# element36-io/hyperfridge-r0

Hardware: AMD Instinct MI355X
Metric: segments/sec (po2=20) proving camt53 guest, 1/2/4/8 MI355X (higher is better)
Workload: dtype u32

## Files before the change

### __graft_entry__.py

```python
import hashlib
import os
import subprocess
import sys

ROOT = os.path.dirname(os.path.abspath(__file__))
HIPCC = os.environ.get("HIPCC", "/opt/rocm/bin/hipcc")
CIRCUITS = ("tiny", "small", "bench", "recursion", "trace", "image")
PRECOMPILED = ("small", "bench", "recursion", "trace", "image")


def _run(cmd, **kw):
    subprocess.check_call(cmd, cwd=ROOT, **kw)


def _stale(target, sources):
    if not os.path.exists(target):
        return True
    t = os.path.getmtime(target)
    return any(os.path.getmtime(s) > t for s in sources)


def circuit_blob_path(name):
    return os.path.join(ROOT, "circuits", name + ".r0c")


def code_object_path(name):
    return os.path.join(ROOT, "circuits", name + ".evalcheck.hsaco")


def check_code_object_path(name):
    return os.path.join(ROOT, "circuits", name + ".checkwitness.hsaco")


def term_names_path(name):
    return os.path.join(ROOT, "circuits", name + ".terms.txt")


NAMED = ("trace", "image")


def build():
    jobs = str(min(8, os.cpu_count() or 1))
    _run(["make", "-s", "-j", jobs, "-C", os.path.join("hyperfridge-r0_amd", "csrc")])
    _run(["make", "-s", "-C", "oracle"])
    gen = os.path.join(ROOT, "tools", "gen_circuit.py")
    for name in CIRCUITS:
        if _stale(circuit_blob_path(name), [gen, os.path.join(ROOT, "tools", "trace_circuit.py"), os.path.join(ROOT, "tools", "sponge_component.py"), os.path.join(ROOT, "tools", "image_circuit.py")]):
            _run([sys.executable, gen, name, circuit_blob_path(name)])
    for name in NAMED:
        if _stale(term_names_path(name), [circuit_blob_path(name)]):
            _run([sys.executable, gen, "--names", name, term_names_path(name)])
    sys.path.insert(0, ROOT)
    import numpy as np

    import hyperfridge_r0_amd as r0
    r0.lib()
    guest = os.path.join(ROOT, "circuits", "guest_camt53.elf")
    if _stale(guest, [os.path.join(ROOT, "tools", n) for n in ("guest_camt53.py", "guest_rsa.py", "rvasm.py")]):
        _run([sys.executable, os.path.join(ROOT, "tools", "guest_camt53.py"), guest], stdout=subprocess.DEVNULL)
    pending = []
    for name in PRECOMPILED:
        blob = np.fromfile(circuit_blob_path(name), dtype=np.uint32)
        for emit, target, suffix in ((r0.emit_eval_check_source, code_object_path(name), ".evalcheck.hip"),
                                     (r0.emit_check_witness_source, check_code_object_path(name), ".checkwitness.hip")):
            src = emit(blob)
            src_path = os.path.join(ROOT, "circuits", name + suffix)
            digest = hashlib.sha256(src.encode()).hexdigest()
            stamp = target + ".sha256"
            if os.path.exists(target) and os.path.exists(stamp) and open(stamp).read() == digest:
                continue
            with open(src_path, "w") as f:
                f.write(src)
            cmd = [HIPCC, "--genco", "--offload-arch=gfx950", "-O3", "-o", target, src_path]
            pending.append((name, stamp, digest, cmd, subprocess.Popen(cmd, cwd=ROOT)))
    for name, stamp, digest, cmd, proc in pending:
        if proc.wait() != 0:
            raise subprocess.CalledProcessError(proc.returncode, cmd)
        with open(stamp, "w") as f:
            f.write(digest)
    return None


def ensure_built():
    needed = [os.path.join(ROOT, "hyperfridge-r0_amd", "libr0hip.so"), os.path.join(ROOT, "hyperfridge-r0_amd", "r0h_prove"),
              os.path.join(ROOT, "hyperfridge-r0_amd", "r0h_verify"), os.path.join(ROOT, "hyperfridge-r0_amd", "r0h_preprocess"),
              os.path.join(ROOT, "oracle", "liborc.so"), os.path.join(ROOT, "circuits", "guest_camt53.elf")] + [circuit_blob_path(n) for n in CIRCUITS] + [code_object_path(n) for n in PRECOMPILED] + [
                  check_code_object_path(n) for n in PRECOMPILED] + [term_names_path(n) for n in NAMED]
    if not all(os.path.exists(p) for p in needed):
        build()


def smoke():
    ensure_built()
    sys.path.insert(0, ROOT)
    sys.path.insert(0, os.path.join(ROOT, "tests"))
    import numpy as np

    import hyperfridge_r0_amd as r0
    import orc_binding
    hal = r0.Hal(0)
    blob = np.fromfile(circuit_blob_path("small"), dtype=np.uint32)
    co = code_object_path("small")
    circuit = hal.load_circuit(blob, co if os.path.exists(co) else None)
    po2 = 10
    code, data, glob = hal.witgen(circuit, po2, seed=42)
    seal = hal.prove_segment(circuit, po2, code, data, glob)
    orc = orc_binding.load()
    oc = orc.circuit(blob)
    root = hal.code_root(circuit, po2)
    rc, why = oc.verify(seal, code_root=root)
    assert rc == 0, "oracle verifier rejected the GPU seal: " + why
    want = oc.prove(po2, code.to_host(), data.to_host(), glob)
    assert np.array_equal(seal, want), "GPU seal differs from the oracle's"
    print("smoke ok: seal of %d words verified (bound to the control root) and identical to the oracle; phases (ms): %s" % (
        seal.size, ", ".join("%s=%.2f" % p for p in hal.last_profile())))
    sys.path.insert(0, os.path.join(ROOT, "tools"))
    from bench_session import elf_of
    from test_rv32im import _guest
    tblob = np.fromfile(circuit_blob_path("trace"), dtype=np.uint32)
    tc = hal.load_circuit(tblob, code_object_path("trace"))
    elf, words = elf_of(_guest(300), 0x400), [7, 0x01020304]
    iblob = np.fromfile(circuit_blob_path("image"), dtype=np.uint32)
    ic = hal.load_circuit(iblob, code_object_path("image"))
    hal.set_image_circuit(ic)
    receipt, image_id, cycles = hal.prove_elf(tc, elf, words, segment_po2=16)
    hal.set_image_circuit(None)
    seals = receipt.seals()
    size = r0.verify_seal(tblob, seals[-1][1])[2]
    troot = hal.code_root(tc, size)
    verdict = receipt.verify(tblob, {size: troot}, None, elf=elf)
    assert verdict[:2] == (0, "ok"), "the receipt of the proved run does not verify with its ELF: %r" % (verdict,)
    verdict = receipt.verify_image(tblob, {size: troot}, iblob, image_id)
    assert verdict[:2] == (0, "ok"), "the receipt does not verify with the image id alone: %r" % (verdict,)
    toc = orc.circuit(tblob)
    assert toc.verify(seals[-1][1], code_root=troot) == (0, "ok"), "oracle verifier rejected the trace-circuit seal"
    vm = r0.Vm()
    vm.load_elf(elf)
    vm.set_input(words)
    assert vm.run(segment_po2=16, keep_trace=True, boundary_rows=True) == (0, 0)
    k = len(seals) - 1
    wdata, _ = vm.trace_witness(k, size, claim_globals=vm.claims()[k].globals())
    want = toc.prove(size, toc.witgen(size, 0)[0], wdata, seals[-1][1][:r0.TRACE_GLOBALS])
    assert np.array_equal(want, seals[-1][1]), "the device's trace-circuit seal differs from the oracle's"
    print("smoke ok: prove(env, elf) of %d cycles in %d segment(s) with the trace circuit: receipt verified with the ELF and with the image id alone, last seal identical to the oracle's" % (cycles, len(seals)))
    ic.free()
    tc.free()
    hal.close()
    return None


if __name__ == "__main__":
    build()
    if len(sys.argv) > 1 and sys.argv[1] == "smoke":
        smoke()
```

### hyperfridge-r0_amd/__init__.py

```python
import ctypes
import sys
import os

import numpy as np

P = 2013265921
INV_RATE = 4
QUERIES = 50
FRI_FOLD = 16
CHECK_SIZE = 16
GROUP_ACCUM, GROUP_CODE, GROUP_DATA = 0, 1, 2

_HERE = os.path.dirname(os.path.abspath(__file__))
LIB_PATH = os.path.join(_HERE, "libr0hip.so")


class R0HipError(RuntimeError):
    pass


_c = ctypes
_vp, _u32, _u64, _sz, _cp = _c.c_void_p, _c.c_uint32, _c.c_uint64, _c.c_size_t, _c.c_char_p
_pp = _c.POINTER(_c.c_void_p)

# ... 42 lines not shown
    "r0h_circuit_emit_hip_check": [_vp, _sz, _c.POINTER(_c.c_char_p)],
    "r0h_circuit_load_check": [_vp, _cp],
    "r0h_check_witness": [_vp, _vp, _u32, _vp, _vp, _vp, _vp, _vp, _vp, _sz, _c.POINTER(_sz)],
    "r0h_ctx_set_check_witness": [_vp, _c.c_int],
    "r0h_circuit_free": [_vp],
    "r0h_witgen": [_vp, _vp, _u32, _u64, _vp, _vp, _vp],
    "r0h_witgen_public": [_vp, _vp, _u32, _u64, _vp, _vp, _vp],
    "r0h_seal_digest": [_vp, _sz, _vp],
    "r0h_ctx_set_session_resident_limit": [_vp, _u64],
    "r0h_proof_shrink": [_vp, _vp],
    "r0h_sponge_trace": [_vp, _sz, _u32, _vp],
    "r0h_image_po2": [_vp, _sz, _vp],
    "r0h_image_witness": [_vp, _sz, _u32, _vp, _vp],
    "r0h_prove_image": [_vp, _vp, _vp, _sz, _vp, _vp, _sz, _vp],
    "r0h_accum": [_vp, _vp, _u32, _vp, _vp, _vp, _vp],
    "r0h_eval_check": [_vp, _vp, _u32, _vp, _vp, _vp, _vp, _vp, _vp, _vp],
    "r0h_prove_segment": [_vp, _vp, _u32, _vp, _vp, _vp, _vp, _sz, _c.POINTER(_sz)],
    "r0h_proof_begin": [_vp, _vp, _u32, _vp, _vp, _vp, _vp, _pp],
    "r0h_proof_finish": [_vp, _vp, _vp, _sz, _c.POINTER(_sz)],
    "r0h_proof_abort": [_vp],
    "r0h_verify_seal": [_vp, _sz, _vp, _vp, _vp, _sz, _c.POINTER(_c.c_int), _c.POINTER(_u32)],
    "r0h_verify_seal_bound": [_vp, _sz, _vp, _vp, _vp, _sz, _vp, _c.POINTER(_c.c_int), _c.POINTER(_u32), _vp],
    "r0h_code_root": [_vp, _vp, _u32, _u32, _vp],
    "r0h_code_commit_new": [_vp, _vp, _u32, _u32, _pp],
    "r0h_code_commit_free": [_vp],
    "r0h_code_commit_root": [_vp, _vp],
    "r0h_prove_segment_committed": [_vp, _vp, _u32, _vp, _vp, _vp, _vp, _sz, _c.POINTER(_sz)],
    "r0h_proof_begin_committed": [_vp, _vp, _u32, _vp, _vp, _vp, _vp, _pp],
    "r0h_serde_encode_str": [_vp, _sz, _vp, _sz, _c.POINTER(_sz)],
    "r0h_serde_decode_str": [_vp, _sz, _c.POINTER(_sz), _c.POINTER(_sz), _c.POINTER(_sz)],
    "r0h_journal_commitment_span": [_vp, _sz, _c.POINTER(_sz), _c.POINTER(_sz)],
    "r0h_env_new": [_pp],
    "r0h_env_write_str": [_vp, _vp, _sz],
    "r0h_env_write_u8_seq": [_vp, _vp, _sz],
    "r0h_env_words": [_vp, _pp, _c.POINTER(_sz)],
    "r0h_env_free": [_vp],
    "r0h_receipt_parse": [_vp, _sz, _pp],
    "r0h_receipt_new": [_c.c_int, _vp, _sz, _pp],
    "r0h_receipt_add_segment": [_vp, _vp, _sz, _u32],
    "r0h_receipt_free": [_vp],
    "r0h_receipt_add_segment_claim": [_vp, _vp, _sz, _u32, _vp, _vp],
    "r0h_receipt_segment_claim": [_vp, _sz, _vp, _c.POINTER(_c.c_int)],
    "r0h_receipt_verify": [_vp, _vp, _sz, _vp, _sz, _vp, _c.POINTER(_c.c_int), _c.POINTER(_sz), _c.POINTER(_c.c_int)],
    "r0h_receipt_verify_elf": [_vp, _vp, _sz, _vp, _sz, _vp, _sz, _c.POINTER(_c.c_int), _c.POINTER(_sz), _c.POINTER(_c.c_int)],
    "r0h_receipt_verify_image": [_vp, _vp, _sz, _vp, _sz, _vp, _sz, _vp, _vp, _c.POINTER(_c.c_int), _c.POINTER(_sz), _c.POINTER(_c.c_int)],
    "r0h_receipt_set_image_proof": [_vp, _vp, _sz],
    "r0h_receipt_image_proof": [_vp, _c.POINTER(_vp), _c.POINTER(_sz)],
    "r0h_ctx_set_image_circuit": [_vp, _vp],
    "r0h_sha256": [_vp, _sz, _vp],
    "r0h_image_id_from_hex": [_cp, _vp],
    "r0h_image_id_to_hex": [_vp, _vp],
    "r0h_tagged_struct": [_cp, _vp, _sz, _vp, _sz, _vp],
    "r0h_system_state_digest": [_vp, _vp],
    "r0h_output_digest": [_vp, _sz, _vp, _vp],
    "r0h_claim_digest": [_vp, _vp],
    "r0h_claim_globals": [_vp, _vp],
    "r0h_receipt_journal": [_vp, _pp, _c.POINTER(_sz)],
    "r0h_receipt_segment": [_vp, _sz, _pp, _c.POINTER(_sz), _c.POINTER(_u32)],
    "r0h_receipt_to_json": [_vp, _pp],
    "r0h_ebics_parse": [_vp, _sz, _pp],
    "r0h_ebics_free": [_vp],
    "r0h_ebics_part": [_vp, _c.c_int, _pp, _c.POINTER(_sz)],
    "r0h_ebics_check_digest": [_vp, _c.POINTER(_c.c_int)],
    "r0h_ebics_verify_bank_signature": [_vp, _vp, _sz, _c.POINTER(_c.c_int)],
    "r0h_ebics_check_transaction_key": [_vp, _vp, _sz, _vp, _sz, _vp, _c.POINTER(_c.c_int)],
    "r0h_ebics_verify_witness": [_vp, _vp, _sz, _vp, _sz, _c.POINTER(_c.c_int)],
    "r0h_ebics_decrypt_transaction_key": [_vp, _vp, _sz, _vp, _sz, _c.POINTER(_sz), _vp, _c.POINTER(_c.c_int)],
    "r0h_ebics_witness_sign": [_vp, _vp, _sz, _pp],
    "r0h_ebics_decrypt_order_data": [_vp, _vp],
    "r0h_ebics_document": [_vp, _sz, _pp, _pp, _c.POINTER(_sz)],
    "r0h_rsa_public_key_decimal": [_vp, _sz, _pp, _pp],
    "r0h_ebics_env_inputs": [_vp, _vp, _sz, _vp, _sz, _vp, _sz, _cp, _cp, _vp, _sz, _vp, _sz, _cp, _pp],
    "r0h_aes128_block": [_vp, _vp, _c.c_int, _vp],
    "r0h_zlib_inflate": [_vp, _sz, _pp, _c.POINTER(_sz)],
    "r0h_vm_new": [_pp],
    "r0h_vm_free": [_vp],
    "r0h_vm_load": [_vp, _u32, _vp, _sz],
    "r0h_vm_load_elf": [_vp, _vp, _sz],
    "r0h_vm_set_input": [_vp, _vp, _sz],
    "r0h_vm_set_pc": [_vp, _u32],
    "r0h_vm_set_reg": [_vp, _u32, _u32],
    "r0h_vm_read": [_vp, _u32, _vp, _sz],
    "r0h_vm_run": [_vp, _vp, _c.POINTER(_c.c_int), _c.POINTER(_u32)],
    "r0h_vm_segment_info": [_vp, _sz, _vp],
    "r0h_vm_preflight": [_vp, _sz, _pp, _c.POINTER(_sz)],
    "r0h_vm_trace_witness": [_vp, _sz, _u32, _vp, _vp],
    "r0h_vm_run_segment": [_vp, _vp, _c.POINTER(_c.c_int), _c.POINTER(_c.c_int), _c.POINTER(_u32)],
    "r0h_vm_release_trace": [_vp, _sz],
    "r0h_vm_boundary": [_vp, _sz, _pp, _c.POINTER(_sz)],
    "r0h_trace_witgen": [_vp, _vp, _sz, _vp, _sz, _u32, _vp, _vp, _vp],
    "r0h_logup_multiplicities": [_vp, _vp, _u32, _vp, _vp],
    "r0h_logup_multiplicities_host": [_vp, _sz, _u32, _vp, _vp],
    "r0h_logup_totals": [_vp, _vp, _u32, _vp, _vp, _vp],
    "r0h_accum_public": [_vp, _vp, _u32, _vp, _vp, _vp, _vp, _vp],
    "r0h_prefix_sums": [_vp, _vp, _u32],
    "r0h_proof_data_root": [_vp, _vp],
    "r0h_proof_late": [_vp, _vp, _vp],
    "r0h_proof_globals": [_vp, _vp],
    "r0h_code_commit_columns": [_vp, _pp],
    "r0h_verify_seal_roots": [_vp, _sz, _vp, _sz, _vp, _c.POINTER(_c.c_int), _c.POINTER(_u32), _vp],
    "r0h_session_begin": [_vp, _vp, _vp, _sz, _vp, _sz, _u32, _u64, _u32, _u32, _pp],
    "r0h_session_records": [_vp, _vp, _vp, _sz, _c.POINTER(_sz)],
    "r0h_session_finish": [_vp, _vp, _sz, _pp, _vp, _c.POINTER(_u64)],
    "r0h_session_free": [_vp],
    "r0h_session_challenge": [_vp, _sz, _vp],
    "r0h_last_session_stats": [_vp, _vp],
    "r0h_vm_journal": [_vp, _pp, _c.POINTER(_sz)],
    "r0h_vm_segment_claim": [_vp, _sz, _vp],
    "r0h_compute_image_id": [_vp, _sz, _vp],
    "r0h_camt53_guest_input": [_vp, _vp, _sz, _vp, _sz, _vp, _sz, _vp, _sz, _vp, _sz, _c.c_char_p, _c.c_char_p, _u32, _pp, _c.POINTER(_sz)],
    "r0h_control_root_host": [_vp, _sz, _vp, _vp, _u32, _vp],
    "r0h_prove_elf": [_vp, _vp, _vp, _sz, _vp, _sz, _u32, _u64, _pp, _vp, _c.POINTER(_u64)],
    "r0h_prove_elf_part": [_vp, _vp, _vp, _sz, _vp, _sz, _u32, _u64, _u32, _u32, _pp, _vp, _c.POINTER(_u64)],
    "r0h_receipt_merge": [_pp, _sz, _pp],
    "r0h_recursor_new": [_vp, _vp, _sz, _cp, _u32, _vp, _sz, _vp, _sz, _pp],
    "r0h_recursor_free": [_vp],
    "r0h_recursor_control_root": [_vp, _vp],
    "r0h_lift": [_vp, _vp, _sz, _vp, _pp],
    "r0h_join": [_vp, _vp, _vp, _pp],
    "r0h_node_new": [_vp, _sz, _vp, _pp],
    "r0h_node_free": [_vp],
    "r0h_node_seal": [_vp, _pp, _c.POINTER(_sz)],
    "r0h_node_claim": [_vp, _vp],
    "r0h_node_verify": [_vp, _sz, _vp, _vp, _c.POINTER(_c.c_int)],
    "r0h_kernel_timing": [_vp, _c.c_int],
    "r0h_kernel_stats": [_vp, _vp, _sz],
    "r0h_last_profile": [_vp, _c.POINTER(_c.POINTER(_cp)), _c.POINTER(_c.POINTER(_c.c_float)), _c.POINTER(_u32)],
}
_PLAIN = {
    "r0h_free_error": ([_vp], None),
    "r0h_version": ([], _cp),
    "r0h_ctx_hashfn": ([_vp], _cp),
    "r0h_receipt_kind": ([_vp], _c.c_int),
    "r0h_receipt_n_segments": ([_vp], _sz),
    "r0h_ebics_n_documents": ([_vp], _sz),
    "r0h_vm_n_segments": ([_vp], _sz),
    "r0h_session_n_segments": ([_vp], _sz),
    "r0h_vm_cycles": ([_vp], _u64),
    "r0h_vm_reg": ([_vp, _u32], _u32),
    "r0h_vm_pc": ([_vp], _u32),
    "r0h_verify_reason": ([_c.c_int], _cp),
    "r0h_trace_column_name": ([_u32], _cp),
    "r0h_receipt_verify_reason": ([_c.c_int], _cp),
    "r0h_buf_device_ptr": ([_vp], _vp),
    "r0h_buf_bytes": ([_vp], _sz),
    "r0h_circuit_group_size": ([_vp, _u32], _u32),
    "r0h_circuit_n_global": ([_vp], _u32),
    "r0h_proof_resident_bytes": ([_vp], _sz),
    "r0h_circuit_n_mix": ([_vp], _u32),
    "r0h_circuit_n_taps": ([_vp], _u32),
    "r0h_circuit_n_terms": ([_vp], _u32),
}
EXPORTED_SYMBOLS = sorted(list(_SIGNATURES) + list(_PLAIN))

_lib = None


def _torch_runtime_first():
    import sys
    if os.environ.get("R0H_NO_TORCH") == "1":
        return
    try:
        if "torch" not in sys.modules:
            import importlib.util
            if importlib.util.find_spec("torch") is None:
                return
        import torch
        if getattr(torch.version, "hip", None):
            torch.cuda.is_available()
    except Exception:
        pass


def lib():
    global _lib
    if _lib is None:
        _torch_runtime_first()
        if not os.path.exists(LIB_PATH):
            raise R0HipError("%s is missing: run `python -c 'import __graft_entry__ as g; g.build()'` (hipcc, gfx950). "
                             "There is no CPU fallback." % LIB_PATH)
        h = ctypes.CDLL(LIB_PATH)
        for name, args in _SIGNATURES.items():
            fn = getattr(h, name)
            fn.argtypes = args
            fn.restype = _vp
        for name, (args, res) in _PLAIN.items():
            fn = getattr(h, name)
            fn.argtypes = args
            fn.restype = res
        _lib = h
    return _lib


def _check(err):
    if err:
        msg = ctypes.cast(err, ctypes.c_char_p).value.decode("utf-8", "replace")
        lib().r0h_free_error(err)
        raise R0HipError(msg)


def _u32arr(a):
    a = np.ascontiguousarray(a, dtype=np.uint32)
    return a, a.ctypes.data_as(_vp)


class Buf:

    def __init__(self, hal, handle, words):
        self.hal, self.handle, self.words = hal, handle, words

    def to_host(self, offset_words=0, words=None):
        words = self.words - offset_words if words is None else words
        out = np.empty(words, dtype=np.uint32)
        _check(lib().r0h_buf_d2h(self.hal.ctx, self.handle, offset_words * 4, out.ctypes.data_as(_vp), words * 4))
        return out

    def upload(self, array, offset_words=0):
        a, p = _u32arr(array)
        _check(lib().r0h_buf_h2d(self.hal.ctx, self.handle, offset_words * 4, p, a.size * 4))

    def slice(self, offset_words, words):
        h = _vp()
        _check(lib().r0h_buf_slice(self.handle, offset_words * 4, words * 4, ctypes.byref(h)))
        return Buf(self.hal, h, words)

    def device_ptr(self):
        return lib().r0h_buf_device_ptr(self.handle)

    def free(self):
        if self.handle:
            _check(lib().r0h_buf_free(self.handle))
            self.handle = None

    def __del__(self):
        try:
            self.free()
        except Exception:
            pass


class Circuit:
    def __init__(self, hal, handle, blob):
        self.hal, self.handle, self.blob = hal, handle, blob
        L = lib()
        self.group_size = [L.r0h_circuit_group_size(handle, g) for g in range(3)]
        self.n_global = L.r0h_circuit_n_global(handle)
        self.n_mix = L.r0h_circuit_n_mix(handle)
        self.n_taps = L.r0h_circuit_n_taps(handle)
        self.n_terms = L.r0h_circuit_n_terms(handle)

    def load_check(self, code_object_path=None):
        _check(lib().r0h_circuit_load_check(self.handle, code_object_path.encode() if code_object_path else None))

    def free(self):
        if self.handle:
            _check(lib().r0h_circuit_free(self.handle))
            self.handle = None

    def __del__(self):
        try:
            self.free()
        except Exception:
            pass


class CodeCommit:

    def __init__(self, handle, po2):
        self.handle, self.po2 = handle, po2

    def root(self):
        out = np.zeros(8, dtype=np.uint32)
        _check(lib().r0h_code_commit_root(self.handle, out.ctypes.data_as(_vp)))
        return out

    def free(self):
        if self.handle:
            _check(lib().r0h_code_commit_free(self.handle))
            self.handle = None

    def __del__(self):
        try:
            self.free()
        except Exception:
            pass


def emit_eval_check_source(blob):
    a, p = _u32arr(blob)
    out = ctypes.c_char_p()
    _check(lib().r0h_circuit_emit_hip(p, a.size, ctypes.byref(out)))
    src = out.value.decode()
    lib().r0h_free_error(ctypes.cast(out, _vp))
    return src


def emit_check_witness_source(blob):
    a, p = _u32arr(blob)
    out = ctypes.c_char_p()
    _check(lib().r0h_circuit_emit_hip_check(p, a.size, ctypes.byref(out)))
    src = out.value.decode()
    lib().r0h_free_error(ctypes.cast(out, _vp))
    return src


class Violation(ctypes.Structure):
    _fields_ = [("term", _u32), ("rows", _u32), ("first_row", _u32), ("reserved", _u32)]


def verify_seal(blob, seal, poseidon2_consts=None, code_root=None, hashfn="poseidon2"):
    b, pb = _u32arr(blob)
    s_, ps = _u32arr(seal)
    if hashfn != "poseidon2":
        if poseidon2_consts is not None:
            raise R0HipError("verify_seal: Poseidon2 tables make no sense with hashfn=%r" % (hashfn,))
        verdict, po2 = _c.c_int(-1), _u32(0)
        proot = None
        if code_root is not None:
            root, proot = _u32arr(code_root)
            if root.size != 8:
                raise R0HipError("verify_seal: a code root is 8 words")
        _check(lib().r0h_verify_seal_hashfn(pb, b.size, str(hashfn).encode(), ps, s_.size, proot, ctypes.byref(verdict), ctypes.byref(po2), None))
        return verdict.value, lib().r0h_verify_reason(verdict.value).decode(), po2.value
    prc = pdg = None
    if poseidon2_consts is not None:
        rc, prc = _u32arr(poseidon2_consts[0])
        dg, pdg = _u32arr(poseidon2_consts[1])
        if rc.size != 29 * 24 or dg.size != 24:
            raise R0HipError("verify_seal: Poseidon2 tables must hold 29*24 and 24 words")
    verdict, po2 = _c.c_int(-1), _u32(0)
    proot = None
    if code_root is not None:
        root, proot = _u32arr(code_root)
        if root.size != 8:
            raise R0HipError("verify_seal: a code root is 8 words")
    _check(lib().r0h_verify_seal_bound(pb, b.size, prc, pdg, ps, s_.size, proot, ctypes.byref(verdict), ctypes.byref(po2), None))
    return verdict.value, lib().r0h_verify_reason(verdict.value).decode(), po2.value


def seal_code_root(blob, seal):
    b, pb = _u32arr(blob)
    s_, ps = _u32arr(seal)
    verdict, po2 = _c.c_int(-1), _u32(0)
    out = np.zeros(8, dtype=np.uint32)
    _check(lib().r0h_verify_seal_bound(pb, b.size, None, None, ps, s_.size, None, ctypes.byref(verdict), ctypes.byref(po2), out.ctypes.data_as(_vp)))
    return out


def serde_encode_str(text):
    raw = text.encode("utf-8") if isinstance(text, str) else bytes(text)
    n = _sz(0)
    _check(lib().r0h_serde_encode_str(raw, len(raw), None, 0, ctypes.byref(n)))
    out = (ctypes.c_uint8 * n.value)()
    _check(lib().r0h_serde_encode_str(raw, len(raw), out, n.value, ctypes.byref(n)))
    return bytes(out)


def serde_decode_str(data):
    data = bytes(data)
    off, ln, used = _sz(0), _sz(0), _sz(0)
    _check(lib().r0h_serde_decode_str(data, len(data), ctypes.byref(off), ctypes.byref(ln), ctypes.byref(used)))
    return data[off.value:off.value + ln.value], used.value


def env_input_words(items):
    h = _vp()
    _check(lib().r0h_env_new(ctypes.byref(h)))
    try:
        for it in items:
            if isinstance(it, str):
                raw = it.encode("utf-8")
                _check(lib().r0h_env_write_str(h, raw, len(raw)))
            else:
                raw = bytes(it)
                _check(lib().r0h_env_write_u8_seq(h, raw, len(raw)))
        p, n = _vp(), _sz(0)
        _check(lib().r0h_env_words(h, ctypes.byref(p), ctypes.byref(n)))
        return np.frombuffer(ctypes.string_at(p, n.value * 4), dtype=np.uint32).copy()
    finally:
        lib().r0h_env_free(h)


def journal_commitment(data):
    data = bytes(data)
    off, ln = _sz(0), _sz(0)
    _check(lib().r0h_journal_commitment_span(data, len(data), ctypes.byref(off), ctypes.byref(ln)))
    return data[off.value:off.value + ln.value]


def seal_digest(seal):
    a, pa = _u32arr(seal)
    out = np.zeros(8, dtype=np.uint32)
    _check(lib().r0h_seal_digest(pa, a.size, out.ctypes.data_as(_vp)))
    return out


SPONGE_DATA_COLUMNS = 65
IMAGE_COLUMNS, IMAGE_GLOBALS, IMAGE_GAMMA, IMAGE_SUM = 69, 28, 8, 24


def image_po2(elf):
    buf = (ctypes.c_uint8 * len(elf)).from_buffer_copy(elf)
    out = _u32(0)
    _check(lib().r0h_image_po2(buf, len(elf), ctypes.byref(out)))
    return out.value


def image_witness(elf, po2=None):
    po2 = image_po2(elf) if po2 is None else po2
    buf = (ctypes.c_uint8 * len(elf)).from_buffer_copy(elf)
    data, glob = np.zeros((IMAGE_COLUMNS, 1 << po2), dtype=np.uint32), np.zeros(IMAGE_GLOBALS, dtype=np.uint32)
    _check(lib().r0h_image_witness(buf, len(elf), po2, data.ctypes.data_as(_vp), glob.ctypes.data_as(_vp)))
    return data, glob


def sponge_trace(words, po2):
    a, pa = _u32arr(words)
    out = np.zeros((SPONGE_DATA_COLUMNS, 1 << po2), dtype=np.uint32)
    _check(lib().r0h_sponge_trace(pa, a.size, po2, out.ctypes.data_as(_vp)))
    return out


class Ebics:
    AUTHENTICATED, SIGNED_INFO, SIGNATURE_VALUE, ORDER_DATA, DIGEST_VALUE, SIGNATURE_BIN, TRANSACTION_KEY_BIN, ORDER_DATA_BIN, PAYLOAD_ZIP = range(9)

    def __init__(self, xml):
        raw = xml.encode("utf-8") if isinstance(xml, str) else bytes(xml)
        self.handle = _vp()
        _check(lib().r0h_ebics_parse(raw, len(raw), ctypes.byref(self.handle)))

    def part(self, which):
        p, n = _vp(), _sz(0)
        _check(lib().r0h_ebics_part(self.handle, which, ctypes.byref(p), ctypes.byref(n)))
        return ctypes.string_at(p, n.value) if n.value else b""

    def camt53_guest_input(self, pub_bank_pem, pub_client_pem, pub_witness_pem, tx_key_block, witness_hex, iban, host_info, form=1):
        pems = [p.encode() if isinstance(p, str) else bytes(p) for p in (pub_bank_pem, pub_client_pem, pub_witness_pem)]
        block = bytes(tx_key_block)
        hx = witness_hex.encode() if isinstance(witness_hex, str) else bytes(witness_hex)
        words, n = _vp(), _sz(0)
        _check(lib().r0h_camt53_guest_input(self.handle, pems[0], len(pems[0]), pems[1], len(pems[1]), pems[2], len(pems[2]), block, len(block), hx, len(hx),
                                            iban.encode(), host_info.encode(), form, ctypes.byref(words), ctypes.byref(n)))
        try:
            return np.frombuffer(ctypes.string_at(words, 4 * n.value), dtype=np.uint32).copy()
        finally:
            lib().r0h_free_error(words)

    def _flag(self, fn, *args):
        ok = _c.c_int(-1)
        _check(fn(self.handle, *args, ctypes.byref(ok)))
        return bool(ok.value)

    def check_digest(self):
# ... 609 lines not shown
    def batch_expand_into_evaluate_ntt(self, out, inp, count, in_po2, expand_bits):
        _check(lib().r0h_batch_expand_into_evaluate_ntt(self.ctx, out.handle, inp.handle, count, in_po2, expand_bits))

    def batch_bit_reverse(self, io, count, po2):
        _check(lib().r0h_batch_bit_reverse(self.ctx, io.handle, count, po2))

    def zk_shift(self, io, count, po2):
        _check(lib().r0h_zk_shift(self.ctx, io.handle, count, po2))

    def batch_interpolate_ntt_zk_shift(self, io, count, po2):
        _check(lib().r0h_batch_interpolate_ntt_zk_shift(self.ctx, io.handle, count, po2))

    def poseidon2_set_consts(self, rc, diag_m1):
        a, pa = _u32arr(rc)
        b, pb = _u32arr(diag_m1)
        assert a.size == 24 * 29 and b.size == 24
        _check(lib().r0h_poseidon2_set_consts(self.ctx, pa, pb))

    def hash_rows(self, digests, matrix, rows, cols):
        _check(lib().r0h_hash_rows(self.ctx, digests.handle, matrix.handle, rows, cols))

    def hash_fold(self, nodes, output_size):
        _check(lib().r0h_hash_fold(self.ctx, nodes.handle, output_size))

    def merkle_build(self, nodes, matrix, rows, cols):
        _check(lib().r0h_merkle_build(self.ctx, nodes.handle, matrix.handle, rows, cols))

    def batch_evaluate_any(self, coeffs, po2, which, xs, out):
        w, pw = _u32arr(which)
        x, px = _u32arr(xs)
        assert x.size == 4 * w.size
        _check(lib().r0h_batch_evaluate_any(self.ctx, coeffs.handle, po2, pw, px, w.size, out.handle))

    def mix_poly_coeffs(self, combos, mix_start, mix, inp, combo_of, po2):
        ms, pms = _u32arr(mix_start)
        m, pm = _u32arr(mix)
        co, pco = _u32arr(combo_of)
        _check(lib().r0h_mix_poly_coeffs(self.ctx, combos.handle, pms, pm, inp.handle, pco, co.size, po2))

    def eltwise_add_elem(self, out, a, b, n):
        _check(lib().r0h_eltwise_add_elem(self.ctx, out.handle, a.handle, b.handle, n))

    def eltwise_copy_elem(self, out, inp, n):
        _check(lib().r0h_eltwise_copy_elem(self.ctx, out.handle, inp.handle, n))

    def eltwise_sum_extelem(self, out, inp, count, n):
        _check(lib().r0h_eltwise_sum_extelem(self.ctx, out.handle, inp.handle, count, n))

    def eltwise_zeroize_elem(self, io, n):
        _check(lib().r0h_eltwise_zeroize_elem(self.ctx, io.handle, n))

    def gather_sample(self, dst, src, idx, size, stride):
        _check(lib().r0h_gather_sample(self.ctx, dst.handle, src.handle, idx, size, stride))

    def scatter(self, into, index, offsets, values, n_index):
        _check(lib().r0h_scatter(self.ctx, into.handle, index.handle, offsets.handle, values.handle, n_index))

    def batch_evaluate_any_buf(self, coeffs, po2, which_buf, xs_buf, n_eval, out):
        _check(lib().r0h_batch_evaluate_any_buf(self.ctx, coeffs.handle, po2, which_buf.handle, xs_buf.handle, n_eval, out.handle))

    def mix_poly_coeffs_buf(self, combos, mix_start, mix, inp, combo_buf, input_count, po2):
        ms, pms = _u32arr(mix_start)
        m, pm = _u32arr(mix)
        _check(lib().r0h_mix_poly_coeffs_buf(self.ctx, combos.handle, pms, pm, inp.handle, combo_buf.handle, input_count, po2))

    def scatter_slices(self, into, index, offsets, values):
        i, pi = _u32arr(index)
        o, po = _u32arr(offsets)
        v, pv = _u32arr(values)
        assert o.size == v.size
        _check(lib().r0h_scatter_slices(self.ctx, into.handle, pi, i.size, po, pv, o.size))

    def hash_fold_io(self, io, input_size, output_size):
        _check(lib().r0h_hash_fold_io(self.ctx, io.handle, input_size, output_size))

    def fri_fold(self, out, inp, mix, n_out):
        m, pm = _u32arr(mix)
        _check(lib().r0h_fri_fold(self.ctx, out.handle, inp.handle, pm, n_out))

    def prefix_products(self, io, n):
        _check(lib().r0h_prefix_products(self.ctx, io.handle, n))

    def poly_divide(self, poly, n, z):
        zz, pz = _u32arr(z)
        rem = np.zeros(4, dtype=np.uint32)
        _check(lib().r0h_poly_divide(self.ctx, poly.handle, n, pz, rem.ctypes.data_as(_vp)))
        return rem

    def load_circuit(self, blob, code_object_path=None):
        a, p = _u32arr(blob)
        h = _vp()
        path = code_object_path.encode() if code_object_path else None
        _check(lib().r0h_circuit_load(self.ctx, p, a.size, path, ctypes.byref(h)))
        return Circuit(self, h, a)

    def witgen(self, circuit, po2, seed, globals_in=None):
        n = 1 << po2
        code = self.alloc(circuit.group_size[GROUP_CODE] * n)
        data = self.alloc(circuit.group_size[GROUP_DATA] * n)
        if globals_in is not None:
            g, pg = _u32arr(globals_in)
            if g.size != circuit.n_global:
                raise R0HipError("witgen: %d public inputs given, the circuit has %d" % (g.size, circuit.n_global))
            _check(lib().r0h_witgen_public(self.ctx, circuit.handle, po2, seed, pg, code.handle, data.handle))
            return code, data, g.copy()
        glob = np.zeros(max(circuit.n_global, 1), dtype=np.uint32)
        _check(lib().r0h_witgen(self.ctx, circuit.handle, po2, seed, code.handle, data.handle, glob.ctypes.data_as(_vp)))
        return code, data, glob[:circuit.n_global]

    def trace_witgen(self, rows, bounds, po2, claim_globals=None, into=None, number=1, closing=True, idle_pc=0, circuit=None):
        rows = np.ascontiguousarray(rows, dtype=np.uint32).reshape(-1, 18)
        bounds = np.ascontiguousarray(bounds, dtype=np.uint32).reshape(-1, 8)
        data = into if into is not None else self.alloc(TRACE_COLUMNS << po2)
        glob = np.zeros(TRACE_GLOBALS, dtype=np.uint32)
        seg = TraceSegment(number, 1 if closing else 0, idle_pc, 0)
        try:
            _check(lib().r0h_trace_witgen(self.ctx, rows.ctypes.data_as(_vp), rows.shape[0], bounds.ctypes.data_as(_vp), bounds.shape[0], po2, ctypes.byref(seg),
                                          data.handle, glob.ctypes.data_as(_vp)))
            if circuit is not None:
                _check(lib().r0h_logup_multiplicities(self.ctx, circuit.handle, po2, data.handle, glob.ctypes.data_as(_vp)))
        except R0HipError:
            if into is None:
                data.free()
            raise
        if claim_globals is not None:
            glob[:8] = claim_globals
        return data, glob

    def witgen_into(self, circuit, po2, seed, code, data):
        glob = np.zeros(max(circuit.n_global, 1), dtype=np.uint32)
        _check(lib().r0h_witgen(self.ctx, circuit.handle, po2, seed, code.handle, data.handle, glob.ctypes.data_as(_vp)))
        return glob[:circuit.n_global]

    def accum(self, circuit, po2, code, data, mix):
        n = 1 << po2
        m, pm = _u32arr(mix)
        out = self.alloc(circuit.group_size[GROUP_ACCUM] * n)
        _check(lib().r0h_accum(self.ctx, circuit.handle, po2, code.handle, data.handle, pm, out.handle))
        return out

    def accum_public(self, circuit, po2, code, data, glob, mix):
        n = 1 << po2
        g, pg = _u32arr(glob)
        m, pm = _u32arr(mix)
        out = self.alloc(circuit.group_size[GROUP_ACCUM] * n)
        _check(lib().r0h_accum_public(self.ctx, circuit.handle, po2, code.handle, data.handle, pg, pm, out.handle))
        return out

    def logup_totals(self, circuit, po2, code, data, glob):
        g = np.ascontiguousarray(glob, dtype=np.uint32).copy()
        _check(lib().r0h_logup_totals(self.ctx, circuit.handle, po2, code.handle, data.handle, g.ctypes.data_as(_vp)))
        return g

    def logup_multiplicities(self, circuit, po2, data, glob):
        g = np.ascontiguousarray(glob if len(glob) else [0], dtype=np.uint32)
        _check(lib().r0h_logup_multiplicities(self.ctx, circuit.handle, po2, data.handle, g.ctypes.data_as(_vp)))

    def prefix_sums(self, io, n):
        _check(lib().r0h_prefix_sums(self.ctx, io.handle, n))

    def eval_check(self, circuit, po2, eval_accum, eval_code, eval_data, glob, mix, poly_mix):
        g, pg = _u32arr(glob)
        m, pm = _u32arr(mix)
        q, pq = _u32arr(poly_mix)
        check = self.alloc(16 << po2)
        _check(lib().r0h_eval_check(self.ctx, circuit.handle, po2, eval_accum.handle, eval_code.handle, eval_data.handle,
                                    pg, pm, pq, check.handle))
        return check

    def check_witness(self, circuit, po2, code, data, glob, accum=None, mix=None, capacity=None):
        g, pg = _u32arr(glob if len(glob) else [0])
        m, pm = _u32arr(mix if mix is not None and len(mix) else [0])
        cap = circuit.n_terms if capacity is None else int(capacity)
        out = (Violation * max(cap, 1))()
        n = _sz(0)
        _check(lib().r0h_check_witness(self.ctx, circuit.handle, po2, accum.handle if accum is not None else None, code.handle, data.handle,
                                       pg, pm if mix is not None else None, out, cap, ctypes.byref(n)))
        if n.value > cap:
            raise R0HipError("check_witness: %d terms are violated, room for %d" % (n.value, cap))
        return [(out[i].term, out[i].rows, out[i].first_row) for i in range(n.value)]

    def set_check_witness(self, on=True):
        _check(lib().r0h_ctx_set_check_witness(self.ctx, 1 if on else 0))

    def prove_segment(self, circuit, po2, code, data, glob, seal_capacity_words=1 << 20):
        g, pg = _u32arr(glob)
        seal = np.empty(seal_capacity_words, dtype=np.uint32)
        n = _sz(0)
        fn = lib().r0h_prove_segment_committed if isinstance(code, CodeCommit) else lib().r0h_prove_segment
        _check(fn(self.ctx, circuit.handle, po2, code.handle, data.handle, pg, seal.ctypes.data_as(_vp), seal.size, ctypes.byref(n)))
        return seal[:n.value].copy()

    def code_commit(self, circuit, po2, code=None):
        own = None
        if code is None:
            code, own, _ = self.witgen(circuit, po2, seed=0)
        h = _vp()
        try:
            _check(lib().r0h_code_commit_new(self.ctx, code.handle, circuit.group_size[GROUP_CODE], po2, ctypes.byref(h)))
        finally:
            if own is not None:
                own.free()
                code.free()
        return CodeCommit(h, po2)

    def code_root(self, circuit, po2, code=None):
        own = None
        if code is None:
            code, own, _ = self.witgen(circuit, po2, seed=0)
        out = np.zeros(8, dtype=np.uint32)
        try:
            _check(lib().r0h_code_root(self.ctx, code.handle, circuit.group_size[GROUP_CODE], po2, out.ctypes.data_as(_vp)))
        finally:
            if own is not None:
                own.free()
                code.free()
        return out

    def prove_elf(self, circuit, elf, input_words, segment_po2=20, max_cycles=0, part=0, parts=1):
        elf = bytes(elf)
        w, pw = _u32arr(input_words if len(input_words) else [0])
        h, image_id, cycles = _vp(), (ctypes.c_uint8 * 32)(), _u64(0)
        _check(lib().r0h_prove_elf_part(self.ctx, circuit.handle, elf, len(elf), pw, len(input_words), segment_po2, max_cycles, part, parts, ctypes.byref(h),
                                        image_id, ctypes.byref(cycles)))
        return Receipt(h), bytes(image_id), cycles.value

    def session_begin(self, circuit, elf, input_words, segment_po2=20, max_cycles=0, part=0, parts=1):
        elf = bytes(elf)
        w, pw = _u32arr(input_words if len(input_words) else [0])
        h = _vp()
        _check(lib().r0h_session_begin(self.ctx, circuit.handle, elf, len(elf), pw, len(input_words), segment_po2, max_cycles, part, parts, ctypes.byref(h)))
        return Session(h)

    def set_session_resident_limit(self, n_bytes):
        _check(lib().r0h_ctx_set_session_resident_limit(self.ctx, n_bytes))

    def set_image_circuit(self, image_circuit):
        _check(lib().r0h_ctx_set_image_circuit(self.ctx, image_circuit.handle if image_circuit is not None else None))
        self._image_circuit = image_circuit

    def prove_image(self, image_circuit, elf, challenge):
        buf = (ctypes.c_uint8 * len(elf)).from_buffer_copy(elf)
        ch, pch = _u32arr(challenge)
        assert ch.size == 16
        seal = np.empty(1 << 18, dtype=np.uint32)
        n = _sz(0)
        _check(lib().r0h_prove_image(self.ctx, image_circuit.handle, buf, len(elf), pch, seal.ctypes.data_as(_vp), seal.size, ctypes.byref(n)))
        return seal[:n.value].copy()

    def last_session_stats(self):
        st = SessionStats()
        _check(lib().r0h_last_session_stats(self.ctx, ctypes.byref(st)))
        return {name: getattr(st, name) for name, _ in SessionStats._fields_}

    def proof_begin(self, circuit, po2, code, data, glob):
        g, pg = _u32arr(glob)
        mix = np.zeros(max(circuit.n_mix, 1), dtype=np.uint32)
        h = _vp()
        fn = lib().r0h_proof_begin_committed if isinstance(code, CodeCommit) else lib().r0h_proof_begin
        _check(fn(self.ctx, circuit.handle, po2, code.handle, data.handle, pg, mix.ctypes.data_as(_vp), ctypes.byref(h)))
        return h, mix[:circuit.n_mix]

    def proof_finish(self, proof, accum, seal_capacity_words=1 << 20):
        seal = np.empty(seal_capacity_words, dtype=np.uint32)
        n = _sz(0)
        _check(lib().r0h_proof_finish(proof, accum.handle, seal.ctypes.data_as(_vp), seal.size, ctypes.byref(n)))
        return seal[:n.value].copy()

    def proof_abort(self, proof):
        _check(lib().r0h_proof_abort(proof))

    def kernel_timing(self, enable=True):
        _check(lib().r0h_kernel_timing(self.ctx, 1 if enable else 0))

    def kernel_stats(self):
        import json
        buf = ctypes.create_string_buffer(1 << 16)
        _check(lib().r0h_kernel_stats(self.ctx, buf, len(buf)))
        return json.loads(buf.value.decode())

    def last_profile(self):
        names = _c.POINTER(_cp)()
        ms = _c.POINTER(_c.c_float)()
        n = _u32(0)
        _check(lib().r0h_last_profile(self.ctx, ctypes.byref(names), ctypes.byref(ms), ctypes.byref(n)))
        return [(names[i].decode(), float(ms[i])) for i in range(n.value)]
```

### hyperfridge-r0_amd/csrc/circuit.hip

```cpp
#include <hip/hiprtc.h>

#include <map>
#include <memory>
#include <sstream>

#include "../../include/r0hip_circuit.h"
#include "circuit.hpp"

namespace r0h {

const char* parse_blob(r0h_circuit* c, const uint32_t* w, size_t n_words) {
  R0H_REQUIRE(n_words >= 3 && w[0] == R0H_BLOB_MAGIC && w[1] == 1, "circuit blob: bad magic or version");
  size_t pos = 3;
  bool seen[16] = {false};
  for (uint32_t s = 0; s < w[2]; s++) {
    R0H_REQUIRE(pos + 2 <= n_words, "circuit blob: truncated section header");
    uint32_t tag = w[pos], len = w[pos + 1];
    const uint32_t* p = w + pos + 2;
    R0H_REQUIRE(pos + 2 + len <= n_words, "circuit blob: section %u overruns the blob", tag);
    if (tag < 16) seen[tag] = true;
    switch (tag) {
      case R0H_SEC_GROUPS:
        R0H_REQUIRE(len >= 3, "circuit blob: GROUPS too short");
        memcpy(c->group_size, p, 12);
// ... 428 lines not shown
      }
      if (!done[s.b]) stack.push_back({s.b, 0});
      if (!done[s.a]) stack.push_back({s.a, 0});
      continue;
    }
    stack.pop_back();
    done[v] = true;
    os << "  const u32 v" << v << " = ";
    if (!f.muls.empty()) {
      std::ostringstream sum;
      sum << "fred64(";
      for (size_t k = 0; k < f.muls.size(); k++) {
        const Step& ms = c->steps[c->fp_step[f.muls[k]]];
        sum << (k ? " + " : "") << "(u64)v" << ms.a << " * v" << ms.b;
      }
      sum << ")";
      std::string expr = sum.str();
      for (uint32_t y : f.rest) expr = "fadd(" + expr + ", v" + std::to_string(y) + ")";
      os << expr << ";\n";
      continue;
    }
    switch (s.op) {
      case R0H_OP_CONST: os << enc(s.a) << "u"; break;
      case R0H_OP_GET: {
        const Tap& t = c->taps[s.a];
        os << "TAP(g" << t.group << ", " << t.offset << "u, " << t.back << "u)";
        break;
      }
      case R0H_OP_GET_GLOBAL: os << (s.a == 0 ? "glob[" : "mix[") << s.b << "]"; break;
      case R0H_OP_ADD:
        if (lazy[v]) os << "v" << s.a << " + v" << s.b;
        else os << "fadd(v" << s.a << ", v" << s.b << ")";
        break;
      case R0H_OP_SUB: os << "fsub(v" << s.a << ", v" << s.b << ")"; break;
      case R0H_OP_MUL: os << "fmul(v" << s.a << ", v" << s.b << ")"; break;
      default: break;
    }
    os << ";\n";
  }
}

static uint32_t tunable(const char* name, uint32_t dflt) {
  const char* v = getenv(name);
  return v && *v ? (uint32_t)strtoul(v, nullptr, 10) : dflt;
}

static void emit_accumulate(const Plan& pl, uint32_t term, uint32_t position, std::ostringstream& os) {
  if (position >= 4 && position % 2 == 0) os << "  T0 = dfix(T0); T1 = dfix(T1); T2 = dfix(T2); T3 = dfix(T3);\n";
  for (int q = 0; q < 4; q++)
    os << "  T" << q << (position ? " += " : " = ") << "(u64)mixpow[" << 4 * (size_t)pl.terms[term].pow + q << "] * w" << term << ";\n";
}

static std::string emit_source(const r0h_circuit* c) {
  const Plan& pl = c->plan;
  const std::vector<bool> lazy = lazy_additions(c);
  const std::vector<Fuse> fuse = plan_fusion(c, lazy);
  const uint32_t scope_terms = tunable("R0H_EC_SCOPE", 0), waves = tunable("R0H_EC_WAVES", 0);
  std::ostringstream os;
  os << PRELUDE;
  os << "// terms: " << pl.terms.size() << ", powers of poly_mix: " << pl.n_pow << ", kernels: " << pl.cut.size() - 1 << "\n";
  for (size_t k = 0; k + 1 < pl.cut.size(); k++) {
    os << "extern \"C\" __global__ __launch_bounds__(256";
    if (waves) os << ", " << waves;
    os << ") void eval_check_" << k
       << "(u32* __restrict__ check, const u32* __restrict__ g0, const u32* __restrict__ g1, const u32* __restrict__ g2,\n"
          "    const u32* __restrict__ glob, const u32* __restrict__ mix, const u32* __restrict__ mixpow,\n"
          "    const u32* __restrict__ inv_van, u32 po2, u32 accumulate) {\n"
          "  const u32 domain = 4u << po2, mask = domain - 1u;\n"
          "  const u32 i = blockIdx.x * 256u + threadIdx.x;\n"
          "  u64 T0 = 0, T1 = 0, T2 = 0, T3 = 0;\n";
    std::vector<bool> done(c->fp_step.size(), false);
    uint32_t in_scope = 0;
    os << "  {\n";
    for (uint32_t t = pl.cut[k]; t < pl.cut[k + 1]; t++) {
      if (scope_terms && in_scope == scope_terms) {
        os << "  }\n  __builtin_amdgcn_sched_barrier(0);\n  {\n";
        std::fill(done.begin(), done.end(), false);
        in_scope = 0;
      }
      const Term& tm = pl.terms[t];
      emit_var(c, tm.v, done, lazy, fuse, os);
      for (uint32_t g : tm.conds) emit_var(c, g, done, lazy, fuse, os);
      std::ostringstream val;
      for (size_t g = 0; g < tm.conds.size(); g++) val << "fmul(v" << tm.conds[g] << ", ";
      val << "v" << tm.v;
      for (size_t g = 0; g < tm.conds.size(); g++) val << ")";
      os << "  const u32 w" << t << " = " << val.str() << ";\n";
      emit_accumulate(pl, t, t - pl.cut[k], os);
      in_scope++;
    }
    os << "  }\n";
    os << "  u32 t0 = dfinish(T0), t1 = dfinish(T1), t2 = dfinish(T2), t3 = dfinish(T3);\n";
    os << "  const u32 iv = inv_van[i & 3u];\n"
          "  t0 = fmul(t0, iv); t1 = fmul(t1, iv); t2 = fmul(t2, iv); t3 = fmul(t3, iv);\n"
          "  if (accumulate) {\n"
          "    t0 = fadd(t0, check[i]); t1 = fadd(t1, check[(size_t)domain + i]);\n"
          "    t2 = fadd(t2, check[2 * (size_t)domain + i]); t3 = fadd(t3, check[3 * (size_t)domain + i]);\n"
          "  }\n"
          "  check[i] = t0; check[(size_t)domain + i] = t1; check[2 * (size_t)domain + i] = t2; check[3 * (size_t)domain + i] = t3;\n"
          "}\n\n";
  }
  return os.str();
}

static const char* CHECK_PRELUDE = R"SRC(// the witness checker: rows of the trace, not the coset
#undef TAP
#define TAP(g, col, back) g[(size_t)(col) * domain + ((i - (back)) & mask)]
// table[2 t] += rows of this wave where term t does not vanish, table[2 t + 1] = min(.., the first of them): lanes are consecutive rows
__device__ __forceinline__ void tally(u32* __restrict__ table, u32 t, u32 w, u32 i) {
  const u64 bad = __ballot(w != 0u);
  if (bad && (threadIdx.x & 63u) == 0u) {
    atomicAdd(table + 2u * t, (u32)__popcll(bad));
    atomicMin(table + 2u * t + 1u, i + (u32)__ffsll((long long)bad) - 1u);
  }
}
)SRC";

static std::string emit_check_source(const r0h_circuit* c) {
  const Plan& pl = c->plan;
  const std::vector<bool> lazy = lazy_additions(c);
  const std::vector<Fuse> fuse(c->fp_step.size());
  std::ostringstream os;
  os << PRELUDE << CHECK_PRELUDE;
  os << "// terms: " << pl.terms.size() << ", kernels: " << pl.cut.size() - 1 << "\n";
  for (size_t k = 0; k + 1 < pl.cut.size(); k++) {
    os << "extern \"C\" __global__ __launch_bounds__(256) void check_witness_" << k
       << "(u32* __restrict__ table, const u32* __restrict__ g0, const u32* __restrict__ g1, const u32* __restrict__ g2,\n"
          "    const u32* __restrict__ glob, const u32* __restrict__ mix, u32 po2, u32 with_accum) {\n"
          "  const u32 domain = 1u << po2, mask = domain - 1u;\n"
          "  const u32 i = blockIdx.x * blockDim.x + threadIdx.x;\n";
    std::vector<bool> done(c->fp_step.size(), false);
    bool any_late = false;
    for (uint32_t t = pl.cut[k]; t < pl.cut[k + 1]; t++) any_late = any_late || pl.late[t];
    for (int late = 0; late < (any_late ? 2 : 1); late++) {
      if (late) os << "  if (with_accum) {\n";
      for (uint32_t t = pl.cut[k]; t < pl.cut[k + 1]; t++) {
        if (pl.late[t] != (late != 0)) continue;
        const Term& tm = pl.terms[t];
        emit_var(c, tm.v, done, lazy, fuse, os);
        for (uint32_t g : tm.conds) emit_var(c, g, done, lazy, fuse, os);
        std::ostringstream val;
        for (size_t g = 0; g < tm.conds.size(); g++) val << "fmul(v" << tm.conds[g] << ", ";
        val << "v" << tm.v;
        for (size_t g = 0; g < tm.conds.size(); g++) val << ")";
        os << "  tally(table, " << t << "u, " << val.str() << ", i);\n";
      }
      if (late) os << "  }\n";
    }
    os << "}\n\n";
  }
  return os.str();
}

static const char* compile_in_process(const std::string& src, std::vector<char>& code) {
  hiprtcProgram prog;
  hiprtcResult r = hiprtcCreateProgram(&prog, src.c_str(), "eval_check.hip", 0, nullptr, nullptr);
  R0H_REQUIRE(r == HIPRTC_SUCCESS, "hiprtcCreateProgram: %s", hiprtcGetErrorString(r));
  const char* opts[] = {"--offload-arch=gfx950", "-O3"};
  r = hiprtcCompileProgram(prog, 2, opts);
  if (r != HIPRTC_SUCCESS) {
    size_t n = 0;
    hiprtcGetProgramLogSize(prog, &n);
    std::string log(n, 0);
    if (n) hiprtcGetProgramLog(prog, &log[0]);
    hiprtcDestroyProgram(&prog);
    return make_error("hiprtcCompileProgram: %s\n%.2000s", hiprtcGetErrorString(r), log.c_str());
  }
  size_t n = 0;
  hiprtcGetCodeSize(prog, &n);
  code.resize(n);
  hiprtcGetCode(prog, code.data());
  hiprtcDestroyProgram(&prog);
  return nullptr;
}

__global__ void witgen_fixed_kernel(uint32_t* __restrict__ buf, const uint32_t* __restrict__ kinds ,
                                    uint32_t po2, uint64_t seed_mixed, const uint32_t* __restrict__ periodic , uint32_t period) {
  const uint32_t r = blockIdx.x * blockDim.x + threadIdx.x, col = blockIdx.y, kind = kinds[2 * col];
  if (kind > 6) return;
  buf[((size_t)col << po2) + r] = fixed_cell(kind, kinds[2 * col + 1], r, 1u << po2, seed_mixed, periodic, period);
}
__global__ void witgen_derived_kernel(uint32_t* __restrict__ dst, const uint32_t* __restrict__ a, const uint32_t* __restrict__ b,
                                      const uint32_t* __restrict__ c, const uint32_t* __restrict__ e, uint32_t ba, uint32_t bb,
                                      uint32_t bc, uint32_t be, uint32_t kind, uint32_t po2) {
  const uint32_t r = blockIdx.x * blockDim.x + threadIdx.x, mask = (1u << po2) - 1;
  uint32_t prod = mul(a[(r - ba) & mask], b[(r - bb) & mask]);
  if (kind == 2) prod = mul(prod, c[(r - bc) & mask]);
  dst[r] = add(prod, e[(r - be) & mask]);
}
__global__ void accum_term_kernel(uint32_t* __restrict__ term, const uint32_t* __restrict__ a, const uint32_t* __restrict__ b, Fp4 m0, Fp4 m1) {
  const uint32_t r = blockIdx.x * blockDim.x + threadIdx.x;
  Fp4 t = m0 + scale(m1, b[r]);
  t.e[0] = add(t.e[0], a[r]);
  *(uint4*)(term + 4 * (size_t)r) = make_uint4(t.e[0], t.e[1], t.e[2], t.e[3]);
}
struct FpCols { const uint32_t* col[3][4]; uint32_t n_f; };
__global__ void accum_fp_term_kernel(uint32_t* __restrict__ term, FpCols cols, Fp4 alpha, Fp4 b1, Fp4 b2, Fp4 b3) {
  const uint32_t r = blockIdx.x * blockDim.x + threadIdx.x;
  Fp4 prod = fp4_one();
  for (uint32_t f = 0; f < cols.n_f; f++) {
    Fp4 t = alpha - scale(b1, cols.col[f][1][r]) - scale(b2, cols.col[f][2][r]) - scale(b3, cols.col[f][3][r]);
    t.e[0] = sub(t.e[0], cols.col[f][0][r]);
    prod = f ? prod * t : t;
  }
  *(uint4*)(term + 4 * (size_t)r) = make_uint4(prod.e[0], prod.e[1], prod.e[2], prod.e[3]);
}
__global__ void check_table_init_kernel(uint32_t* __restrict__ table, uint32_t n_terms) {
  const uint32_t t = blockIdx.x * blockDim.x + threadIdx.x;
  if (t < n_terms) { table[2 * t] = 0u; table[2 * t + 1] = 0xffffffffu; }
}
__global__ void accum_unpack_kernel(uint32_t* __restrict__ cols, const uint32_t* __restrict__ term, uint32_t po2) {
  const uint32_t r = blockIdx.x * blockDim.x + threadIdx.x;
  uint4 v = *(const uint4*)(term + 4 * (size_t)r);
  cols[r] = v.x; cols[((size_t)1 << po2) + r] = v.y; cols[((size_t)2 << po2) + r] = v.z; cols[((size_t)3 << po2) + r] = v.w;
}

}

using namespace r0h;

extern "C" {

const char* r0h_circuit_emit_hip(const uint32_t* blob, size_t n_words, char** source_out) {
  R0H_GUARD_BEGIN
  R0H_REQUIRE(blob && source_out, "r0h_circuit_emit_hip: NULL argument");
  r0h_circuit c;
  R0H_TRY(parse_blob(&c, blob, n_words));
  make_plan(&c);
  std::string src = emit_source(&c);
  char* out = (char*)malloc(src.size() + 1);
  R0H_REQUIRE(out, "r0h_circuit_emit_hip: out of memory");
  memcpy(out, src.c_str(), src.size() + 1);
  *source_out = out;
  return nullptr;
  R0H_GUARD_END
}

static const char* read_code_object(const char* caller, const char* path, std::vector<char>& code) {
  FILE* f = fopen(path, "rb");
  R0H_REQUIRE(f, "%s: cannot open code object %s", caller, path);
  fseek(f, 0, SEEK_END);
  long sz = ftell(f);
  fseek(f, 0, SEEK_SET);
  code.resize(sz > 0 ? (size_t)sz : 0);
  size_t got = fread(code.data(), 1, code.size(), f);
  fclose(f);
  R0H_REQUIRE(got == code.size() && !code.empty(), "%s: short read of %s", caller, path);
  return nullptr;
}

struct CircuitUnload {
  void operator()(r0h_circuit* circuit) const {
    if (circuit->module) (void)hipModuleUnload(circuit->module);
    if (circuit->check_module) (void)hipModuleUnload(circuit->check_module);
    delete circuit;
  }
};

const char* r0h_circuit_load(r0h_ctx* ctx, const uint32_t* blob, size_t n_words, const char* code_object_path, r0h_circuit** out) {
  R0H_GUARD_BEGIN
  R0H_REQUIRE(ctx && blob && out, "r0h_circuit_load: NULL argument");
  std::unique_ptr<r0h_circuit, CircuitUnload> c(new r0h_circuit());
  c->ctx = ctx;
  R0H_TRY(parse_blob(c.get(), blob, n_words));
  make_plan(c.get());
  R0H_TRY_HIP(hipSetDevice(ctx->device));
  std::vector<char> code;
  if (code_object_path) {
    R0H_TRY(read_code_object("r0h_circuit_load", code_object_path, code));
  } else {
    R0H_TRY(compile_in_process(emit_source(c.get()), code));
  }
  hipError_t e = hipModuleLoadData(&c->module, code.data());
  R0H_REQUIRE(e == hipSuccess, "r0h_circuit_load: hipModuleLoadData: %s", hipGetErrorString(e));
  for (size_t k = 0;; k++) {
    char name[64];
    snprintf(name, sizeof name, "eval_check_%zu", k);
    hipFunction_t fn;
    if (hipModuleGetFunction(&fn, c->module, name) != hipSuccess) break;
    c->kernels.push_back(fn);
  }
  (void)hipGetLastError();
  R0H_REQUIRE(!c->kernels.empty() || c->plan.terms.empty(), "r0h_circuit_load: the code object has no eval_check_0 (built from another source?)");
  ctx_retain(ctx);
  *out = c.release();
  return nullptr;
  R0H_GUARD_END
}

const char* r0h_circuit_free(r0h_circuit* c) {
  if (!c) return nullptr;
  r0h_ctx* ctx = c->ctx;
  (void)hipSetDevice(ctx->device);
  (void)hipStreamSynchronize(ctx->stream);
  CircuitUnload()(c);
  ctx_release(ctx);
  return nullptr;
}

uint32_t r0h_circuit_group_size(const r0h_circuit* c, uint32_t group) { return c && group < 3 ? c->group_size[group] : 0; }
uint32_t r0h_circuit_n_global(const r0h_circuit* c) { return c ? c->n_global : 0; }
uint32_t r0h_circuit_n_mix(const r0h_circuit* c) { return c ? c->n_mix : 0; }
uint32_t r0h_circuit_n_taps(const r0h_circuit* c) { return c ? (uint32_t)c->taps.size() : 0; }
uint32_t r0h_circuit_n_terms(const r0h_circuit* c) { return c ? (uint32_t)c->plan.terms.size() : 0; }

const char* r0h_circuit_emit_hip_check(const uint32_t* blob, size_t n_words, char** source_out) {
  R0H_GUARD_BEGIN
  R0H_REQUIRE(blob && source_out, "r0h_circuit_emit_hip_check: NULL argument");
  r0h_circuit c;
  R0H_TRY(parse_blob(&c, blob, n_words));
  make_plan(&c);
  std::string src = emit_check_source(&c);
  char* out = (char*)malloc(src.size() + 1);
  R0H_REQUIRE(out, "r0h_circuit_emit_hip_check: out of memory");
  memcpy(out, src.c_str(), src.size() + 1);
  *source_out = out;
  return nullptr;
  R0H_GUARD_END
}

static const char* check_module_load(const r0h_circuit* c, const char* caller, const char* code_object_path) {
  if (c->check_module) return nullptr;
  R0H_TRY_HIP(hipSetDevice(c->ctx->device));
  std::vector<char> code;
  if (code_object_path) R0H_TRY(read_code_object(caller, code_object_path, code));
  else R0H_TRY(compile_in_process(emit_check_source(c), code));
  hipModule_t module = nullptr;
  hipError_t e = hipModuleLoadData(&module, code.data());
  R0H_REQUIRE(e == hipSuccess, "%s: hipModuleLoadData: %s", caller, hipGetErrorString(e));
  std::vector<hipFunction_t> kernels;
  for (size_t k = 0; k + 1 < c->plan.cut.size(); k++) {
    char name[64];
    snprintf(name, sizeof name, "check_witness_%zu", k);
    hipFunction_t fn;
    if (hipModuleGetFunction(&fn, module, name) != hipSuccess) {
      (void)hipGetLastError();
      (void)hipModuleUnload(module);
      return make_error("%s: the code object has no %s (built from another source?)", caller, name);
    }
    kernels.push_back(fn);
  }
  c->check_module = module;
  c->check_kernels.swap(kernels);
  return nullptr;
}

const char* r0h_circuit_load_check(r0h_circuit* c, const char* code_object_path) {
  R0H_GUARD_BEGIN
  R0H_REQUIRE(c, "r0h_circuit_load_check: NULL argument");
  std::lock_guard<std::mutex> lk(c->check_mu);
  R0H_REQUIRE(!c->check_module, "r0h_circuit_load_check: the circuit's checker is loaded already");
  return check_module_load(c, "r0h_circuit_load_check", code_object_path);
  R0H_GUARD_END
}

}
namespace r0h {
const char* sponge_plant(r0h_ctx* ctx, const r0h_circuit* c, uint32_t po2, const uint32_t* words, size_t n_words, r0h_buf* data) {
  R0H_REQUIRE(ctx && c && data && c->has_sponge && (words || !n_words), "sponge_plant: NULL argument, or a circuit without the sponge component");
  const size_t n = (size_t)1 << po2, n_perm = n_words ? (n_words + P2_RATE - 1) / P2_RATE : 1, rows = n_perm * R0H_SPONGE_PERIOD;
  R0H_REQUIRE(rows < n, "the in-circuit sponge over %zu words takes %zu rows: the recursion trace has 2^%u", n_words, rows, po2);
  R0H_REQUIRE(((size_t)c->group_size[R0H_GROUP_DATA] << po2) * 4 <= data->bytes, "sponge_plant: DATA buffer too small for 2^%u rows", po2);
  for (size_t i = 0; i < n_words; i++) R0H_REQUIRE(words[i] < P, "sponge_plant: word %zu is not a canonical field element", i);
  std::vector<uint32_t> cols((size_t)R0H_SPONGE_DATA_COLUMNS * rows);
  size_t used = 0;
  p2_sponge_rows_host(p2_default(), words, n_words, cols.data(), rows, &used);
  uint32_t* first = u32(data) + ((size_t)c->sponge_data << po2);
  R0H_TRY_HIP(hipMemsetAsync(first, 0, (size_t)R0H_SPONGE_DATA_COLUMNS * n * 4, ctx->stream));
  R0H_TRY_HIP(hipMemcpy2DAsync(first, n * 4, cols.data(), rows * 4, rows * 4, R0H_SPONGE_DATA_COLUMNS, hipMemcpyHostToDevice, ctx->stream));
  R0H_TRY_HIP(hipStreamSynchronize(ctx->stream));
  return nullptr;
}
}
namespace r0h {
static const char* witgen_fixed(r0h_ctx* ctx, const r0h_circuit* c, uint32_t po2, std::vector<uint32_t>& kinds, uint64_t seed_mixed, r0h_buf* buf) {
  const uint32_t n = 1u << po2, threads = n < 256 ? n : 256, cols = (uint32_t)(kinds.size() / 2);
  const size_t table_at = kinds.size();
  for (uint32_t v : c->periodic) kinds.push_back(enc(v));
  R0H_TRY(ensure_scratch(ctx, kinds.size() * 4));
  R0H_TRY(stage_h2d(ctx, ctx->scratch, kinds.data(), kinds.size() * 4));
  const uint32_t* dk = (const uint32_t*)ctx->scratch;
  hipLaunchKernelGGL(witgen_fixed_kernel, dim3(n / threads, cols), dim3(threads), 0, ctx->stream, u32(buf), dk, po2, seed_mixed, dk + table_at, c->period);
  return launch_ok("r0h_witgen");
}
const char* witgen_code(r0h_ctx* ctx, const r0h_circuit* c, uint32_t po2, r0h_buf* code) {
  R0H_REQUIRE(ctx && c && code, "r0h_witgen: NULL argument");
  R0H_REQUIRE(c->has_column_program, "r0h_witgen: this circuit carries no synthetic column program (WITGEN/ACCUM sections); supply the witness");
  R0H_REQUIRE(po2 >= 4 && po2 <= R0H_MAX_PO2, "r0h_witgen: po2 %u outside [4, %u]", po2, R0H_MAX_PO2);
  const uint32_t nc = (uint32_t)c->code_cols.size();
  R0H_REQUIRE(((size_t)nc << po2) * 4 <= code->bytes, "r0h_witgen: buffers too small for 2^%u rows", po2);
  std::vector<uint32_t> kinds(2 * (size_t)nc);
  for (uint32_t k = 0; k < nc; k++) { kinds[2 * k] = c->code_cols[k].kind; kinds[2 * k + 1] = code_col_arg(c->code_cols[k], k); }
  return witgen_fixed(ctx, c, po2, kinds, splitmix64(CODE_SEED), code);
}
const char* code_commit_of(r0h_ctx* ctx, const r0h_circuit* c, uint32_t po2, r0h_code_commit** out) {
  DevBuf code;
  R0H_TRY(code.alloc(ctx, ((size_t)c->group_size[R0H_GROUP_CODE] << po2) * 4));
  R0H_TRY(witgen_code(ctx, c, po2, code.get()));
  return r0h_code_commit_new(ctx, code.get(), c->group_size[R0H_GROUP_CODE], po2, out);
}
}
extern "C" {

static const char* witgen_impl(r0h_ctx* ctx, const r0h_circuit* c, uint32_t po2, uint64_t seed, const uint32_t* global_in, r0h_buf* code,
                               r0h_buf* data, uint32_t* global_out) {
  R0H_GUARD_BEGIN
  R0H_REQUIRE(ctx && c && code && data, "r0h_witgen: NULL argument");
  R0H_REQUIRE(c->has_column_program, "r0h_witgen: this circuit carries no synthetic column program (WITGEN/ACCUM sections); supply the witness");
  R0H_REQUIRE(po2 >= 4 && po2 <= R0H_MAX_PO2, "r0h_witgen: po2 %u outside [4, %u]", po2, R0H_MAX_PO2);
  const uint32_t n = 1u << po2, threads = n < 256 ? n : 256, nc = (uint32_t)c->code_cols.size(), nd = (uint32_t)c->data_cols.size();
  R0H_REQUIRE(((size_t)nc << po2) * 4 <= code->bytes && ((size_t)nd << po2) * 4 <= data->bytes, "r0h_witgen: buffers too small for 2^%u rows", po2);
  R0H_TRY(witgen_code(ctx, c, po2, code));
  std::vector<uint32_t> kinds(2 * (size_t)nd);
  for (uint32_t k = 0; k < nd; k++) { kinds[2 * k] = c->data_cols[k].kind == 0 ? 3u : 99u; kinds[2 * k + 1] = (2u << 16) | k; }
  R0H_TRY(witgen_fixed(ctx, c, po2, kinds, splitmix64(seed), data));
  if (c->has_sponge) {
    R0H_TRY(sponge_plant(ctx, c, po2, nullptr, 0, data));
    if (!global_in) {
      uint32_t digest[8];
      p2_hash_elems_host(p2_default(), nullptr, 0, digest);
      for (uint32_t j = 0; j < 8; j++) R0H_TRY(stage_h2d(ctx, u32(data) + ((size_t)c->global_cols[c->sponge_global + j] << po2), digest + j, 4));
    }
  }
  if (global_in) {
    for (uint32_t k = 0; k < c->n_global; k++) {
      R0H_REQUIRE(global_in[k] < P, "r0h_witgen_public: global %u is not a canonical field word", k);
      R0H_TRY(stage_h2d(ctx, u32(data) + ((size_t)c->global_cols[k] << po2), global_in + k, 4));
    }
  }
  for (uint32_t k = 0; k < nd; k++) {
    const DataCol& d = c->data_cols[k];
    if (d.kind == 0) continue;
    auto col = [&](uint32_t r) { return ((r >> 28) == R0H_GROUP_CODE ? u32(code) : u32(data)) + ((size_t)(r & 0xfffffu) << po2); };
    auto back = [](uint32_t r) { return (r >> 20) & 0xffu; };
    uint32_t rc = d.kind == 2 ? d.c : d.a;
    hipLaunchKernelGGL(witgen_derived_kernel, dim3(n / threads), dim3(threads), 0, ctx->stream, u32(data) + ((size_t)k << po2), col(d.a), col(d.b),
                       col(rc), col(d.e), back(d.a), back(d.b), back(rc), back(d.e), d.kind, po2);
  }
  R0H_TRY(launch_ok("r0h_witgen"));
  if (global_out) {
    for (uint32_t k = 0; k < c->n_global; k++)
      R0H_TRY_HIP(hipMemcpyAsync(global_out + k, u32(data) + ((size_t)c->global_cols[k] << po2), 4, hipMemcpyDeviceToHost, ctx->stream));
  }
  R0H_TRY_HIP(hipStreamSynchronize(ctx->stream));
  return nullptr;
  R0H_GUARD_END
}

const char* r0h_witgen(r0h_ctx* ctx, const r0h_circuit* c, uint32_t po2, uint64_t seed, r0h_buf* code, r0h_buf* data, uint32_t* global_out) {
  return witgen_impl(ctx, c, po2, seed, nullptr, code, data, global_out);
}

const char* r0h_witgen_public(r0h_ctx* ctx, const r0h_circuit* c, uint32_t po2, uint64_t seed, const uint32_t* global_in, r0h_buf* code, r0h_buf* data) {
  R0H_REQUIRE(global_in || r0h_circuit_n_global(c) == 0, "r0h_witgen_public: global_in is NULL");
  return witgen_impl(ctx, c, po2, seed, global_in, code, data, nullptr);
}

const char* r0h_accum(r0h_ctx* ctx, const r0h_circuit* c, uint32_t po2, const r0h_buf* code, const r0h_buf* data, const uint32_t* mix, r0h_buf* accum) {
  R0H_GUARD_BEGIN
  (void)code;
  R0H_REQUIRE(ctx && c && data && accum && (mix || c->n_mix == 0), "r0h_accum: NULL argument");
  R0H_REQUIRE(c->has_column_program, "r0h_accum: this circuit carries no synthetic column program (WITGEN/ACCUM sections)");
  R0H_REQUIRE(po2 >= 4 && po2 <= R0H_MAX_PO2, "r0h_accum: po2 %u outside [4, %u]", po2, R0H_MAX_PO2);
  const uint32_t n = 1u << po2, threads = n < 256 ? n : 256;
  R0H_REQUIRE(((size_t)c->data_cols.size() << po2) * 4 <= data->bytes && ((size_t)c->group_size[R0H_GROUP_ACCUM] << po2) * 4 <= accum->bytes,
              "r0h_accum: buffers too small for 2^%u rows", po2);
  for (uint32_t i = 0; i < c->n_mix; i++) R0H_REQUIRE(mix[i] < P, "r0h_accum: mix[%u] not canonical", i);
  R0H_REQUIRE(c->logup.accs.empty(), "r0h_accum: this circuit accumulates a log-derivative argument that reads public inputs: use r0h_accum_public");
  DevBuf term;
  R0H_TRY(term.alloc(ctx, (size_t)n * 16));
  for (uint32_t j = 0; j < c->acc_fp.size(); j++) {
    const AccFp& a = c->acc_fp[j];
    FpCols cols;
    cols.n_f = a.n_f;
    for (uint32_t f = 0; f < 3; f++)
      for (uint32_t q = 0; q < 4; q++) cols.col[f][q] = u32(data) + ((size_t)a.col[f][q] << po2);
    auto m = [&](uint32_t k) { return Fp4{{mix[4 * k], mix[4 * k + 1], mix[4 * k + 2], mix[4 * k + 3]}}; };
    hipLaunchKernelGGL(accum_fp_term_kernel, dim3(n / threads), dim3(threads), 0, ctx->stream, u32(term.get()), cols, m(0), m(1), m(2), m(3));
    R0H_TRY(r0h_prefix_products(ctx, term.get(), n));
    hipLaunchKernelGGL(accum_unpack_kernel, dim3(n / threads), dim3(threads), 0, ctx->stream, u32(accum) + ((size_t)(4 * j) << po2), u32(term.get()), po2);
  }
  for (uint32_t j = 0; j < c->acc_cols.size(); j++) {
    Fp4 m0{{mix[8 * j], mix[8 * j + 1], mix[8 * j + 2], mix[8 * j + 3]}}, m1{{mix[8 * j + 4], mix[8 * j + 5], mix[8 * j + 6], mix[8 * j + 7]}};
    hipLaunchKernelGGL(accum_term_kernel, dim3(n / threads), dim3(threads), 0, ctx->stream, u32(term.get()), u32(data) + ((size_t)c->acc_cols[j].a << po2),
                       u32(data) + ((size_t)c->acc_cols[j].b << po2), m0, m1);
    R0H_TRY(r0h_prefix_products(ctx, term.get(), n));
    hipLaunchKernelGGL(accum_unpack_kernel, dim3(n / threads), dim3(threads), 0, ctx->stream, u32(accum) + ((size_t)(4 * j) << po2), u32(term.get()), po2);
  }
  return launch_ok("r0h_accum");
  R0H_GUARD_END
}

const char* r0h_accum_public(r0h_ctx* ctx, const r0h_circuit* c, uint32_t po2, const r0h_buf* code, const r0h_buf* data, const uint32_t* global, const uint32_t* mix, r0h_buf* accum) {
  R0H_REQUIRE(ctx && c, "r0h_accum_public: NULL argument");
  if (c->logup.accs.empty()) return r0h_accum(ctx, c, po2, code, data, mix, accum);
  return logup_accum(ctx, c, po2, code, data, global, mix, accum);
}

const char* r0h_eval_check(r0h_ctx* ctx, const r0h_circuit* c, uint32_t po2, const r0h_buf* eval_accum, const r0h_buf* eval_code,
                           const r0h_buf* eval_data, const uint32_t* global, const uint32_t* mix, const uint32_t poly_mix[4], r0h_buf* check) {
  R0H_GUARD_BEGIN
  R0H_REQUIRE(ctx && c && eval_accum && eval_code && eval_data && check && poly_mix, "r0h_eval_check: NULL argument");
  R0H_REQUIRE((global || !c->n_global) && (mix || !c->n_mix), "r0h_eval_check: NULL globals");
  R0H_REQUIRE(po2 >= 6 && po2 <= R0H_MAX_PO2, "r0h_eval_check: po2 %u outside [6, %u]", po2, R0H_MAX_PO2);
  for (int q = 0; q < 4; q++) R0H_REQUIRE(poly_mix[q] < P, "r0h_eval_check: poly_mix words must be canonical (< p)");
  const size_t domain = (size_t)4 << po2;
  const r0h_buf* g[3] = {eval_accum, eval_code, eval_data};
  for (int k = 0; k < 3; k++) R0H_REQUIRE(domain * c->group_size[k] * 4 <= g[k]->bytes, "r0h_eval_check: group %d buffer too small", k);
  R0H_REQUIRE(domain * 16 <= check->bytes, "r0h_eval_check: check buffer too small");
  std::vector<uint32_t> params(c->n_global + c->n_mix + 4 * (size_t)c->plan.n_pow + 4);
// ... 103 lines not shown
```

### hyperfridge-r0_amd/csrc/circuit.hpp

```cpp
#pragma once
#include <mutex>

#include "../../include/r0hip_circuit.h"
#include "internal.hpp"

namespace r0h {

struct Tap { uint32_t group, offset, back; };
struct Reg { uint32_t group, offset, first_tap, size, combo; };
struct Step { uint32_t op, a, b, c; };
struct CodeCol { uint32_t kind, param; };
struct DataCol { uint32_t kind, a, b, c, e; };
struct AccCol { uint32_t first, a, b; };
struct AccFp { uint32_t n_f; uint32_t col[3][4]; };
struct Term { uint32_t pow, v; std::vector<uint32_t> conds; };
struct LfTerm { uint32_t coef, global, col; };
struct Lf { std::vector<LfTerm> terms; };
struct LogupPart { uint32_t ch_kind, ch_idx; Lf lf; };
struct LogupFraction { uint32_t table; Lf num; std::vector<LogupPart> parts; };
struct LogupAcc { uint32_t final_global; std::vector<LogupFraction> fr; };
struct LogupTable { uint32_t data_col, kind; };
struct Logup {
  std::vector<LogupTable> tables;
  std::vector<LogupAcc> accs;
  uint32_t n_chain = 0;
};

R0H_HD uint64_t splitmix64(uint64_t x) {
  x += 0x9E3779B97F4A7C15ull;
  x = (x ^ (x >> 30)) * 0xBF58476D1CE4E5B9ull;
  x = (x ^ (x >> 27)) * 0x94D049BB133111EBull;
  return x ^ (x >> 31);
}
R0H_HD uint32_t synth_word(uint64_t seed_mixed, uint32_t stream, uint32_t row) {
  uint64_t h = splitmix64(seed_mixed ^ (((uint64_t)stream << 32) | row));
  return (uint32_t)(((h >> 32) * (uint64_t)P) >> 32);
}
constexpr uint64_t CODE_SEED = 0xC0DEull;
inline uint32_t code_col_arg(const CodeCol& cc, uint32_t col) { return cc.kind == 6 ? cc.param : (1u << 16) | col; }
R0H_HD uint32_t fixed_cell(uint32_t kind, uint32_t arg, uint32_t r, uint32_t n, uint64_t seed_mixed, const uint32_t* periodic, uint32_t period) {
  if (kind == 0) return r == 0 ? ONE : 0u;
  if (kind == 1) return r == n - 1 ? ONE : 0u;
  if (kind == 2) return enc(r);
  if (kind == 3) return synth_word(seed_mixed, arg, r);
  if (kind == 4) return r < 65536u ? enc(r) : 0u;
  if (kind == 5) return enc(R0H_TAG_AND + (r < 65536u ? r + 65536u * ((r & 255u) & (r >> 8)) : 0u));
  if (kind == 6) return r < (n / period) * period ? periodic[arg * period + r % period] : 0u;
  return 0u;
}

struct Plan {
  std::vector<Term> terms;
  std::vector<uint32_t> cut;
  uint32_t n_pow = 0;
  std::vector<bool> late;
};

}

struct r0h_circuit {
  r0h_ctx* ctx = nullptr;
  uint32_t group_size[3] = {0, 0, 0};
  std::vector<r0h::Tap> taps;
  std::vector<r0h::Reg> regs;
  std::vector<uint32_t> combo_begin, combo_backs;
  uint32_t group_tap_begin[4] = {0, 0, 0, 0};
  uint32_t n_global = 0, n_mix = 0;
  std::vector<uint32_t> global_cols;
  std::vector<r0h::Step> steps;
  uint32_t ret = 0;
  std::vector<uint32_t> fp_step, mix_step;
  std::vector<r0h::CodeCol> code_cols;
  std::vector<r0h::DataCol> data_cols;
  std::vector<r0h::AccCol> acc_cols;
  std::vector<r0h::AccFp> acc_fp;
  r0h::Logup logup;
  uint32_t period = 0;
  std::vector<uint32_t> periodic;
  bool has_sponge = false;
  uint32_t sponge_code = 0, sponge_data = 0, sponge_global = 0;
  uint32_t n_late = 0;
  bool has_column_program = false;
  std::vector<uint32_t> blob;
  uint8_t info[16] = {'R', '0', 'H', 'I', 'P', '_', 'S', 'Y', 'N', 'T', 'H', ':', 'v', '1', '_', '_'};
  r0h::Plan plan;
  hipModule_t module = nullptr;
  std::vector<hipFunction_t> kernels;
  mutable std::mutex check_mu;
  mutable hipModule_t check_module = nullptr;
  mutable std::vector<hipFunction_t> check_kernels;
};

namespace r0h {
const char* parse_blob(r0h_circuit* c, const uint32_t* blob, size_t n_words);
const char* sponge_plant(r0h_ctx* ctx, const r0h_circuit* c, uint32_t po2, const uint32_t* words, size_t n_words, r0h_buf* data);
const char* require_witness(const char* caller, r0h_ctx* ctx, const r0h_circuit* c, uint32_t po2, const r0h_buf* accum, const r0h_buf* code, const r0h_buf* data,
                            const uint32_t* global, const uint32_t* mix);
const char* logup_accum(r0h_ctx* ctx, const r0h_circuit* c, uint32_t po2, const r0h_buf* code, const r0h_buf* data, const uint32_t* global, const uint32_t* mix, r0h_buf* accum);
}
```

### hyperfridge-r0_amd/csrc/image.cpp

```cpp
#include <string.h>

#include <algorithm>
#include <memory>
#include <vector>

#include "../../include/r0hip_circuit.h"
#include "circuit.hpp"
#include "receipt_types.hpp"

using namespace r0h;

namespace r0h {
bool is_image_circuit(const r0h_circuit& c) {
  return !memcmp(c.info, "R0HIP_IMAGE:v1__", 16) && c.n_global == R0H_IMAGE_GLOBALS && c.n_late == R0H_IMAGE_LATE_GLOBALS && c.has_sponge &&
         c.group_size[R0H_GROUP_DATA] == R0H_IMAGE_COLUMNS && c.sponge_data == 0 && c.sponge_global == 0;
}
const char* image_witness(const std::vector<std::pair<uint32_t, uint32_t>>& image, uint32_t po2, uint32_t* data, uint32_t digest[8]) {
  std::vector<uint32_t> stream;
  image_stream(image, stream);
  const size_t n = (size_t)1 << po2, n_blocks = stream.size() / 16;
  R0H_REQUIRE(n_blocks * R0H_SPONGE_PERIOD < n, "the image's %zu words take %zu rows: the image trace has 2^%u", image.size(), n_blocks * R0H_SPONGE_PERIOD, po2);
  memset(data, 0, (size_t)R0H_IMAGE_COLUMNS * n * 4);
  size_t used = 0;
  p2_sponge_rows_host(p2_default(), stream.data(), stream.size(), data, n, &used);
  for (size_t q = 0; q < n_blocks; q++) {
    const size_t there = std::min<size_t>(4, image.size() - std::min<size_t>(image.size(), 4 * q));
    for (size_t j = 0; j < there; j++) data[(R0H_SPONGE_DATA_COLUMNS + j) * n + q * R0H_SPONGE_PERIOD] = ONE;
  }
  if (digest) p2_hash_elems_host(p2_default(), stream.data(), stream.size(), digest);
  return nullptr;
}
}

extern "C" {

const char* r0h_image_po2(const uint8_t* elf, size_t elf_len, uint32_t* po2_out) {
  R0H_GUARD_BEGIN
  R0H_REQUIRE(elf && po2_out, "r0h_image_po2: NULL argument");
  std::vector<std::pair<uint32_t, uint32_t>> image;
  uint32_t entry;
  uint8_t id[32];
  R0H_TRY(elf_image(elf, elf_len, image, &entry, id));
  const size_t rows = (image.empty() ? 1 : (image.size() + 3) / 4) * R0H_SPONGE_PERIOD;
  uint32_t po2 = 9;
  while (((size_t)1 << po2) <= rows) po2++;
  R0H_REQUIRE(po2 <= R0H_MAX_PO2, "r0h_image_po2: an image of %zu words does not fit a trace", image.size());
  *po2_out = po2;
  return nullptr;
  R0H_GUARD_END
}

const char* r0h_image_witness(const uint8_t* elf, size_t elf_len, uint32_t po2, uint32_t* data_out, uint32_t globals_out[R0H_IMAGE_GLOBALS]) {
  R0H_GUARD_BEGIN
  R0H_REQUIRE(elf && data_out && globals_out, "r0h_image_witness: NULL argument");
  R0H_REQUIRE(po2 >= 6 && po2 <= R0H_MAX_PO2, "r0h_image_witness: po2 %u outside [6, %u]", po2, R0H_MAX_PO2);
  std::vector<std::pair<uint32_t, uint32_t>> image;
  uint32_t entry;
  uint8_t id[32];
  R0H_TRY(elf_image(elf, elf_len, image, &entry, id));
  memset(globals_out, 0, R0H_IMAGE_GLOBALS * 4);
  return image_witness(image, po2, data_out, globals_out);
  R0H_GUARD_END
}

const char* r0h_ctx_set_image_circuit(r0h_ctx* ctx, const r0h_circuit* image_circuit) {
  R0H_GUARD_BEGIN
  R0H_REQUIRE(ctx, "r0h_ctx_set_image_circuit: ctx is NULL");
  if (image_circuit) {
    R0H_REQUIRE(is_image_circuit(*image_circuit), "r0h_ctx_set_image_circuit: the circuit is not the image circuit (circuits/image.r0c) this library was built for");
    R0H_REQUIRE(image_circuit->ctx == ctx, "r0h_ctx_set_image_circuit: the circuit was loaded on another context");
  }
  ctx->image_circuit = image_circuit;
  return nullptr;
  R0H_GUARD_END
}

const char* r0h_prove_image(r0h_ctx* ctx, const r0h_circuit* c, const uint8_t* elf, size_t elf_len, const uint32_t challenge[16], uint32_t* seal_out,
                            size_t seal_capacity_words, size_t* seal_words_out) {
  R0H_GUARD_BEGIN
  R0H_REQUIRE(ctx && c && elf && challenge && seal_words_out, "r0h_prove_image: NULL argument");
  R0H_TRY(require_poseidon2(ctx, "r0h_prove_image"));
  R0H_REQUIRE(is_image_circuit(*c), "r0h_prove_image: the circuit is not the image circuit (circuits/image.r0c) this library was built for");
  for (int i = 0; i < 16; i++) R0H_REQUIRE(challenge[i] < P, "r0h_prove_image: challenge word %d is not a canonical field word", i);
  R0H_TRY_HIP(hipSetDevice(ctx->device));
  std::vector<std::pair<uint32_t, uint32_t>> image;
  uint32_t entry, po2 = 9;
  uint8_t id[32];
  R0H_TRY(elf_image(elf, elf_len, image, &entry, id));
  std::vector<uint32_t> stream, global(R0H_IMAGE_GLOBALS, 0);
  image_stream(image, stream);
  const size_t n_blocks = stream.size() / 16, rows = n_blocks * R0H_SPONGE_PERIOD;
  while (((size_t)1 << po2) <= rows) po2++;
  R0H_REQUIRE(po2 <= R0H_MAX_PO2, "r0h_prove_image: an image of %zu words does not fit a trace", image.size());
  const size_t n = (size_t)1 << po2;
  p2_hash_elems_host(p2_default(), stream.data(), stream.size(), global.data());
  memcpy(&global[R0H_IMAGE_GAMMA], challenge, 64);
  DevBuf code, data;
  const size_t data_bytes = (size_t)R0H_IMAGE_COLUMNS * n * 4;
  R0H_TRY(code.alloc(ctx, (size_t)c->group_size[R0H_GROUP_CODE] * n * 4));
  R0H_TRY(data.alloc(ctx, data_bytes));
  R0H_TRY(witgen_code(ctx, c, po2, code.get()));
  R0H_TRY(sponge_plant(ctx, c, po2, stream.data(), stream.size(), data.get()));
  std::vector<uint32_t> flags(4 * n_blocks, 0u);
  for (size_t k = 0; k < image.size(); k++) flags[(k % 4) * n_blocks + k / 4] = ONE;
  uint32_t* first_flag = (uint32_t*)data->ptr + (size_t)R0H_SPONGE_DATA_COLUMNS * n;
  R0H_TRY_HIP(hipMemsetAsync(first_flag, 0, 4 * n * 4, ctx->stream));
  for (size_t j = 0; j < 4; j++)
    R0H_TRY_HIP(hipMemcpy2DAsync(first_flag + j * n, (size_t)R0H_SPONGE_PERIOD * 4, flags.data() + j * n_blocks, 4, 4, n_blocks, hipMemcpyHostToDevice, ctx->stream));
  R0H_TRY(r0h_logup_totals(ctx, c, po2, code.get(), data.get(), global.data()));
  return r0h_prove_segment(ctx, c, po2, code.get(), data.get(), global.data(), seal_out, seal_capacity_words, seal_words_out);
  R0H_GUARD_END
}

}
```

### hyperfridge-r0_amd/csrc/logup.hip

```cpp
#include <algorithm>
#include <map>

#include "../../include/r0hip_circuit.h"
#include "circuit.hpp"

namespace r0h {

namespace {
struct Tape {
  std::vector<uint32_t> words;
  std::vector<const uint32_t*> cols;
  std::vector<Fp4> ch;
  std::vector<uint32_t> acc_begin;
};

const char* build_tape(const r0h_circuit* c, uint32_t po2, const r0h_buf* code, const r0h_buf* data, const uint32_t* global, const uint32_t* mix, Tape* t, bool lookups_only = false) {
  std::map<uint32_t, uint32_t> col_index;
  std::map<uint64_t, uint32_t> ch_index;
  t->ch.push_back(fp4_one());
  auto form = [&](const Lf& lf) -> const char* {
    t->words.push_back((uint32_t)lf.terms.size());
    for (const LfTerm& term : lf.terms) {
      uint32_t coef = enc(term.coef);
      if (term.global) {
        R0H_REQUIRE(global, "log-derivative accumulation: a form reads a public input and none were given");
        coef = mul(coef, global[term.global - 1]);
      }
      uint32_t col = 0;
      if (term.col) {
        const uint32_t ref = term.col - 1;
        auto it = col_index.find(ref);
        if (it == col_index.end()) {
          const r0h_buf* src = (ref >> 28) == R0H_GROUP_CODE ? code : data;
          R0H_REQUIRE(src, "log-derivative accumulation: a form reads the %s group and none was given", (ref >> 28) == R0H_GROUP_CODE ? "CODE" : "DATA");
          it = col_index.emplace(ref, (uint32_t)t->cols.size()).first;
          t->cols.push_back(u32(src) + ((size_t)(ref & 0xfffffu) << po2));
        }
        col = it->second + 1;
      }
      t->words.push_back(coef);
      t->words.push_back(col);
    }
    return nullptr;
  };
  for (const LogupAcc& a : c->logup.accs) {
    t->acc_begin.push_back((uint32_t)t->words.size());
    for (const LogupFraction& f : a.fr) {
      if (lookups_only && !f.table) continue;
      t->words.push_back(f.table);
      R0H_TRY(form(f.num));
      t->words.push_back((uint32_t)f.parts.size());
      for (const LogupPart& q : f.parts) {
        uint32_t idx = 0;
        if (q.ch_kind) {
          const uint64_t key = (uint64_t)q.ch_kind << 32 | q.ch_idx;
          auto it = ch_index.find(key);
          if (it == ch_index.end()) {
            const uint32_t* src = q.ch_kind == 1 ? mix + 4 * (size_t)q.ch_idx : global + q.ch_idx;
            R0H_REQUIRE(q.ch_kind == 1 ? mix != nullptr : global != nullptr, "log-derivative accumulation: a challenge is read from %s and none were given", q.ch_kind == 1 ? "the mix" : "the public inputs");
            it = ch_index.emplace(key, (uint32_t)t->ch.size()).first;
            t->ch.push_back(Fp4{{src[0], src[1], src[2], src[3]}});
          }
          idx = it->second;
        }
        t->words.push_back(idx);
        R0H_TRY(form(q.lf));
      }
    }
  }
  t->acc_begin.push_back((uint32_t)t->words.size());
  return nullptr;
}

struct DeviceTape {
  DevBuf buf;
  const uint32_t* words = nullptr;
  const uint32_t* const* cols = nullptr;
  const Fp4* ch = nullptr;
};
const char* upload_tape(r0h_ctx* ctx, const Tape& t, DeviceTape* d) {
  const size_t w_bytes = (t.words.size() * 4 + 15) & ~(size_t)15, c_bytes = (t.cols.size() * sizeof(void*) + 15) & ~(size_t)15, h_bytes = t.ch.size() * 16;
  R0H_TRY(d->buf.alloc(ctx, w_bytes + c_bytes + h_bytes));
  char* base = (char*)d->buf->ptr;
  R0H_TRY(stage_h2d(ctx, base, t.words.data(), t.words.size() * 4));
  R0H_TRY(stage_h2d(ctx, base + w_bytes, t.cols.data(), t.cols.size() * sizeof(void*)));
  R0H_TRY(stage_h2d(ctx, base + w_bytes + c_bytes, t.ch.data(), h_bytes));
  d->words = (const uint32_t*)base;
  d->cols = (const uint32_t* const*)(base + w_bytes);
  d->ch = (const Fp4*)(base + w_bytes + c_bytes);
  return nullptr;
}

__device__ __forceinline__ uint32_t eval_form(const uint32_t* __restrict__ tape, uint32_t& at, const uint32_t* const* __restrict__ cols, uint32_t r) {
  const uint32_t n = tape[at++];
  uint32_t acc = 0;
  for (uint32_t k = 0; k < n; k++) {
    const uint32_t coef = tape[at], col = tape[at + 1];
    at += 2;
    acc = add(acc, col ? mul(coef, cols[col - 1][r]) : coef);
  }
  return acc;
}

constexpr uint32_t HOT = 4096;

__global__ __launch_bounds__(256) void logup_count_kernel(uint32_t* __restrict__ hist , uint32_t* __restrict__ err, const uint32_t* __restrict__ tape,
                                                          uint32_t tape_end, const uint32_t* const* __restrict__ cols, uint32_t n, uint32_t n_tables) {
  __shared__ uint32_t hot[2][HOT];
  for (uint32_t i = threadIdx.x; i < 2 * HOT; i += 256) (&hot[0][0])[i] = 0;
  __syncthreads();
  const uint32_t r = blockIdx.x * 256u + threadIdx.x;
  uint32_t gated[2] = {0, 0};
  if (r < n) {
    uint32_t at = 0;
    while (at < tape_end) {
      const uint32_t table = tape[at++];
      const uint32_t num = eval_form(tape, at, cols, r);
      const uint32_t n_parts = tape[at++];
      uint32_t value = 0;
      for (uint32_t q = 0; q < n_parts; q++) {
        at++;
        const uint32_t v = eval_form(tape, at, cols, r);
        if (q == 1) value = v;
      }
      if (!table || table > n_tables) continue;
      if (num != ONE) {
        if (num) atomicOr(err, 1u);
        else gated[table - 1]++;
        continue;
      }
      uint32_t v = dec(neg(value));
      if (table == R0H_TABLE_AND) {
        v -= R0H_TAG_AND;
        if (v >> 24 || ((v & 255u) & ((v >> 8) & 255u)) != v >> 16) { atomicOr(err, 2u); continue; }
        v &= 0xffffu;
      } else if (v >> 16) {
        atomicOr(err, 2u);
        continue;
      }
      if (!v) continue;
      if (v < HOT) atomicAdd(&hot[table - 1][v], 1u);
      else atomicAdd(&hist[(size_t)(table - 1) * 65536 + v], 1u);
    }
  }
  if (gated[0]) atomicAdd(&hot[0][0], gated[0]);
  if (gated[1]) atomicAdd(&hot[1][0], gated[1]);
  __syncthreads();
  for (uint32_t i = threadIdx.x; i < 2 * HOT; i += 256) {
    const uint32_t cnt = (&hot[0][0])[i];
    if (cnt) atomicAdd(&hist[(size_t)(i / HOT) * 65536 + (i % HOT)], cnt);
  }
}
__global__ void logup_mult_kernel(uint32_t* __restrict__ column, const uint32_t* __restrict__ hist, uint32_t total, uint32_t n) {
  __shared__ uint32_t part[256];
  const uint32_t r = blockIdx.x * 256u + threadIdx.x;
  if (blockIdx.x == 0) {
    uint32_t s = 0;
    for (uint32_t i = threadIdx.x; i < 65536u; i += 256) s += hist[i];
    part[threadIdx.x] = s;
    __syncthreads();
    for (uint32_t k = 128; k; k >>= 1) {
      if (threadIdx.x < k) part[threadIdx.x] += part[threadIdx.x + k];
      __syncthreads();
    }
  }
  if (r >= n) return;
  uint32_t v = r < 65536u ? hist[r] : 0u;
  if (r == 0) v = total - part[0];
  column[r] = enc(v);
}

__global__ __launch_bounds__(256) void logup_term_kernel(uint32_t* __restrict__ accum, uint32_t* __restrict__ row_total, uint32_t* __restrict__ own_terms,
                                                         const uint32_t* __restrict__ tape, const uint32_t* const* __restrict__ cols, const Fp4* __restrict__ ch,
                                                         uint32_t a0, uint32_t a1, uint32_t n_chain, uint32_t po2) {
  const uint32_t r = blockIdx.x * 256u + threadIdx.x, n = 1u << po2;
  if (r >= n) return;
  uint32_t at = 0;
  Fp4 run = fp4_zero();
  for (uint32_t j = a0; j < a1; j++) {
    Fp4 d[4];
    uint32_t num[4];
    for (uint32_t f = 0; f < 4; f++) {
      at++;
      num[f] = eval_form(tape, at, cols, r);
      const uint32_t n_parts = tape[at++];
      Fp4 den = fp4_zero();
      for (uint32_t q = 0; q < n_parts; q++) {
        const uint32_t ci = tape[at++];
        const uint32_t v = eval_form(tape, at, cols, r);
        if (ci == 0) den.e[0] = add(den.e[0], v);
        else den = den + scale(ch[ci], v);
      }
      d[f] = den;
    }
    const Fp4 d01 = d[0] * d[1], d23 = d[2] * d[3];
    const Fp4 top = (scale(d[1], num[0]) + scale(d[0], num[1])) * d23 + (scale(d[3], num[2]) + scale(d[2], num[3])) * d01;
    const Fp4 term = top * fp4_inv(d01 * d23);
    if (j < n_chain) {
      run = run + term;
      for (uint32_t i = 0; i < 4; i++) accum[((size_t)(4 * j + i) << po2) + r] = run.e[i];
    } else {
      *(uint4*)(own_terms + 4 * ((size_t)(j - n_chain) * n + r)) = make_uint4(term.e[0], term.e[1], term.e[2], term.e[3]);
    }
  }
  if (a0 < n_chain) *(uint4*)(row_total + 4 * (size_t)r) = make_uint4(run.e[0], run.e[1], run.e[2], run.e[3]);
}
__global__ void logup_chain_kernel(uint32_t* __restrict__ accum, const uint32_t* __restrict__ scanned, uint32_t n_cols, uint32_t po2) {
  const uint32_t r = blockIdx.x * 256u + threadIdx.x, col = blockIdx.y;
  if (r == 0 || r >= (1u << po2) || col >= n_cols) return;
  uint32_t* cell = accum + ((size_t)col << po2) + r;
  *cell = add(*cell, scanned[4 * (size_t)(r - 1) + (col & 3u)]);
}
__global__ void logup_unpack_kernel(uint32_t* __restrict__ cols, const uint32_t* __restrict__ scanned, uint32_t po2) {
  const uint32_t r = blockIdx.x * 256u + threadIdx.x;
  if (r >= (1u << po2)) return;
  const uint4 v = *(const uint4*)(scanned + 4 * (size_t)r);
  cols[r] = v.x; cols[((size_t)1 << po2) + r] = v.y; cols[((size_t)2 << po2) + r] = v.z; cols[((size_t)3 << po2) + r] = v.w;
}
}

static const char* own_accumulators(r0h_ctx* ctx, const r0h_circuit* c, uint32_t po2, const Tape& t, const DeviceTape& d, r0h_buf* accum, uint32_t* totals_out) {
  const uint32_t n = 1u << po2, n_chain = c->logup.n_chain, n_acc = (uint32_t)c->logup.accs.size(), n_own = n_acc - n_chain;
  if (!n_own) return nullptr;
  DevBuf terms;
  R0H_TRY(terms.alloc(ctx, (size_t)n_own * n * 16));
  hipLaunchKernelGGL(logup_term_kernel, dim3((n + 255) / 256), dim3(256), 0, ctx->stream, accum ? u32(accum) : nullptr, (uint32_t*)nullptr, u32(terms.get()),
                     d.words + t.acc_begin[n_chain], d.cols, d.ch, n_chain, n_acc, n_chain, po2);
  R0H_TRY(launch_ok("logup_term_kernel"));
  for (uint32_t k = 0; k < n_own; k++) {
    r0h_buf view = buf_view(terms.get(), (size_t)k * n * 16, (size_t)n * 16);
    R0H_TRY(r0h_prefix_sums(ctx, &view, n));
    if (accum) {
      hipLaunchKernelGGL(logup_unpack_kernel, dim3((n + 255) / 256), dim3(256), 0, ctx->stream, u32(accum) + ((size_t)(4 * (n_chain + k)) << po2), (const uint32_t*)view.ptr, po2);
      R0H_TRY(launch_ok("logup_unpack_kernel"));
    }
    if (totals_out) R0H_TRY(r0h_buf_d2h(ctx, &view, (size_t)(n - 1) * 16, totals_out + 4 * k, 16));
  }
  return nullptr;
}

const char* logup_accum(r0h_ctx* ctx, const r0h_circuit* c, uint32_t po2, const r0h_buf* code, const r0h_buf* data, const uint32_t* global, const uint32_t* mix, r0h_buf* accum) {
  R0H_GUARD_BEGIN
  R0H_REQUIRE(ctx && c && data && accum, "r0h_accum: NULL argument");
  R0H_REQUIRE(po2 >= 4 && po2 <= R0H_MAX_PO2, "r0h_accum: po2 %u outside [4, %u]", po2, R0H_MAX_PO2);
  const uint32_t n = 1u << po2, n_chain = c->logup.n_chain;
  R0H_REQUIRE(((size_t)c->group_size[R0H_GROUP_DATA] << po2) * 4 <= data->bytes && ((size_t)c->group_size[R0H_GROUP_ACCUM] << po2) * 4 <= accum->bytes &&
                  (!code || ((size_t)c->group_size[R0H_GROUP_CODE] << po2) * 4 <= code->bytes),
              "r0h_accum: buffers too small for 2^%u rows", po2);
  for (uint32_t i = 0; i < c->n_mix; i++) R0H_REQUIRE(mix && mix[i] < P, "r0h_accum: mix[%u] missing or not canonical", i);
  for (uint32_t i = 0; i < c->n_global; i++) R0H_REQUIRE(!global || global[i] < P, "r0h_accum: global[%u] not canonical", i);
  Tape t;
  R0H_TRY(build_tape(c, po2, code, data, global, mix, &t));
  DeviceTape d;
  R0H_TRY(upload_tape(ctx, t, &d));
  KScope ks(ctx, "logup_accum", ((double)t.cols.size() + 2.0 * c->group_size[R0H_GROUP_ACCUM]) * n * 4);
  DevBuf totals;
  R0H_TRY(totals.alloc(ctx, (size_t)n * 16));
  hipLaunchKernelGGL(logup_term_kernel, dim3((n + 255) / 256), dim3(256), 0, ctx->stream, u32(accum), u32(totals.get()), (uint32_t*)nullptr, d.words, d.cols, d.ch, 0u, n_chain, n_chain, po2);
  R0H_TRY(launch_ok("logup_term_kernel"));
  R0H_TRY(r0h_prefix_sums(ctx, totals.get(), n));
  hipLaunchKernelGGL(logup_chain_kernel, dim3((n + 255) / 256, 4 * n_chain), dim3(256), 0, ctx->stream, u32(accum), u32(totals.get()), 4 * n_chain, po2);
  R0H_TRY(launch_ok("logup_chain_kernel"));
  R0H_TRY(own_accumulators(ctx, c, po2, t, d, accum, nullptr));
  R0H_TRY_HIP(hipStreamSynchronize(ctx->stream));
  return nullptr;
  R0H_GUARD_END
}

}

using namespace r0h;

extern "C" {

const char* r0h_logup_multiplicities(r0h_ctx* ctx, const r0h_circuit* c, uint32_t po2, r0h_buf* data, const uint32_t* global) {
  R0H_GUARD_BEGIN
  R0H_REQUIRE(ctx && c && data, "r0h_logup_multiplicities: NULL argument");
  if (c->logup.tables.empty()) return nullptr;
  R0H_REQUIRE(po2 >= 16 && po2 <= R0H_MAX_PO2, "r0h_logup_multiplicities: the tables have 2^16 rows: po2 %u outside [16, %u]", po2, R0H_MAX_PO2);
  R0H_REQUIRE(((size_t)c->group_size[R0H_GROUP_DATA] << po2) * 4 <= data->bytes, "r0h_logup_multiplicities: the DATA buffer is too small for 2^%u rows", po2);
  R0H_REQUIRE(c->logup.tables.size() <= 2, "r0h_logup_multiplicities: at most two tables");
  const uint32_t n = 1u << po2, n_tables = (uint32_t)c->logup.tables.size();
  Tape t;
  std::vector<uint32_t> dummy_mix(c->n_mix, 0), dummy_global(c->n_global, 0);
  R0H_TRY(build_tape(c, po2, nullptr, data, global ? global : dummy_global.data(), dummy_mix.data(), &t, true));
  DeviceTape d;
  R0H_TRY(upload_tape(ctx, t, &d));
  std::vector<uint64_t> slots(n_tables, 0);
  for (uint32_t j = 0; j < c->logup.n_chain; j++)
    for (const LogupFraction& f : c->logup.accs[j].fr)
      if (f.table && f.table <= n_tables) slots[f.table - 1] += n;
  for (uint32_t k = 0; k < n_tables; k++)
    R0H_REQUIRE(slots[k] <= P - 1, "r0h_logup_multiplicities: table %u has %llu lookup slots at 2^%u rows: more than p - 1", k, (unsigned long long)slots[k], po2);
  DevBuf hist;
  const size_t hist_words = (size_t)n_tables * 65536;
  R0H_TRY(hist.alloc(ctx, hist_words * 4 + 16));
  R0H_TRY_HIP(hipMemsetAsync(hist->ptr, 0, hist_words * 4 + 16, ctx->stream));
  KScope ks(ctx, "logup_multiplicities", (double)t.cols.size() * n * 4);
  hipLaunchKernelGGL(logup_count_kernel, dim3((n + 255) / 256), dim3(256), 0, ctx->stream, u32(hist.get()), u32(hist.get()) + hist_words, d.words, (uint32_t)t.words.size(), d.cols, n, n_tables);
  R0H_TRY(launch_ok("logup_count_kernel"));
  for (uint32_t k = 0; k < n_tables; k++) {
    const LogupTable& tb = c->logup.tables[k];
    hipLaunchKernelGGL(logup_mult_kernel, dim3((n + 255) / 256), dim3(256), 0, ctx->stream, u32(data) + ((size_t)tb.data_col << po2), u32(hist.get()) + (size_t)k * 65536,
                       (uint32_t)slots[k], n);
    R0H_TRY(launch_ok("logup_mult_kernel"));
  }
  R0H_TRY_HIP(hipStreamSynchronize(ctx->stream));
  uint32_t err = 0;
  R0H_TRY(r0h_buf_d2h(ctx, hist.get(), hist_words * 4, &err, 4));
  R0H_REQUIRE(!(err & 1u), "r0h_logup_multiplicities: a lookup's numerator is neither 0 nor 1");
  R0H_REQUIRE(!(err & 2u), "r0h_logup_multiplicities: a row whose numerator is 1 looks up a value that is not in its table");
  return nullptr;
  R0H_GUARD_END
}

const char* r0h_logup_totals(r0h_ctx* ctx, const r0h_circuit* c, uint32_t po2, const r0h_buf* code, const r0h_buf* data, uint32_t* global_io) {
  R0H_GUARD_BEGIN
  R0H_REQUIRE(ctx && c && data && global_io, "r0h_logup_totals: NULL argument");
  R0H_REQUIRE(po2 >= 4 && po2 <= R0H_MAX_PO2, "r0h_logup_totals: po2 %u outside [4, %u]", po2, R0H_MAX_PO2);
  const uint32_t n_chain = c->logup.n_chain, n_acc = (uint32_t)c->logup.accs.size();
  if (n_acc == n_chain) return nullptr;
  for (uint32_t j = n_chain; j < n_acc; j++)
    for (const LogupFraction& f : c->logup.accs[j].fr)
      for (const LogupPart& q : f.parts) R0H_REQUIRE(q.ch_kind != 1, "r0h_logup_totals: accumulator %u takes a challenge from the mix", j);
  Tape t;
  std::vector<uint32_t> dummy_mix(c->n_mix, 0);
  R0H_TRY(build_tape(c, po2, code ? code : data, data, global_io, dummy_mix.data(), &t));
  DeviceTape d;
  R0H_TRY(upload_tape(ctx, t, &d));
  std::vector<uint32_t> totals(4 * (size_t)(n_acc - n_chain));
  R0H_TRY(own_accumulators(ctx, c, po2, t, d, nullptr, totals.data()));
  for (uint32_t j = n_chain; j < n_acc; j++) memcpy(global_io + c->logup.accs[j].final_global, totals.data() + 4 * (size_t)(j - n_chain), 16);
  return nullptr;
  R0H_GUARD_END
}

}
```

### hyperfridge-r0_amd/csrc/prover.hip

```cpp
#include <memory>

#include "seal_layout.hpp"

namespace r0h {

struct CircuitView {
  uint32_t group_size[3];
  uint32_t n_taps, n_regs, n_combos, n_global, n_mix;
  std::vector<uint32_t> tap_offset, tap_back, reg_group, reg_offset, reg_first, reg_size, reg_combo;
  const uint32_t* combo_begin; const uint32_t* combo_backs;
  uint32_t group_tap_begin[4];
  const uint32_t* blob; size_t blob_words;
};
static void circuit_view(const r0h_circuit* c, CircuitView* v) {
  memcpy(v->group_size, c->group_size, sizeof v->group_size);
  v->n_taps = (uint32_t)c->taps.size(); v->n_regs = (uint32_t)c->regs.size(); v->n_combos = (uint32_t)c->combo_begin.size() - 1;
  v->n_global = c->n_global; v->n_mix = c->n_mix;
  for (const Tap& t : c->taps) { v->tap_offset.push_back(t.offset); v->tap_back.push_back(t.back); }
  for (const Reg& r : c->regs) {
    v->reg_group.push_back(r.group); v->reg_offset.push_back(r.offset); v->reg_first.push_back(r.first_tap);
    v->reg_size.push_back(r.size); v->reg_combo.push_back(r.combo);
  }
  v->combo_begin = c->combo_begin.data(); v->combo_backs = c->combo_backs.data();
  memcpy(v->group_tap_begin, c->group_tap_begin, sizeof v->group_tap_begin);
// ... 306 lines not shown

  phase(ctx, "mix_combos");
  const Fp4 mixv = io.rng.ext();
  const uint32_t n_combos = cv.n_combos;
  r0h_buf* combos = nullptr;
  R0H_TRY(sc.alloc(ctx, (size_t)(n_combos + 1) * n * 16, &combos));
  R0H_TRY(r0h_buf_zero(ctx, combos));
  Fp4 cur = fp4_one();
  for (int g = 0; g < 3; g++) {
    uint32_t gs = cv.group_size[g];
    std::vector<uint32_t> combo_of(gs);
    for (uint32_t r = 0; r < cv.n_regs; r++)
      if (cv.reg_group[r] == (uint32_t)g) combo_of[cv.reg_offset[r]] = cv.reg_combo[r];
    R0H_TRY(r0h_mix_poly_coeffs(ctx, combos, cur.e, mixv.e, grp[g]->coeffs, combo_of.data(), gs, po2));
    cur = cur * fp4_pow(mixv, gs);
  }
  {
    uint32_t combo_of[R0H_CHECK_SIZE];
    for (int i = 0; i < R0H_CHECK_SIZE; i++) combo_of[i] = n_combos;
    R0H_TRY(r0h_mix_poly_coeffs(ctx, combos, cur.e, mixv.e, g_check.coeffs, combo_of, R0H_CHECK_SIZE, po2));
  }
  R0H_TRY(bit_reverse_ext(ctx, combos, n_combos + 1, po2));
  {
    std::vector<Fp4> head((size_t)(n_combos + 1) * 64, fp4_zero());
    std::vector<uint32_t> head_len(n_combos + 1, 0);
    cur = fp4_one();
    for (uint32_t r = 0; r < cv.n_regs; r++) {
      R0H_REQUIRE(cv.reg_size[r] <= 64, "prove_segment: register with more than 64 taps");
      for (uint32_t i = 0; i < cv.reg_size[r]; i++) {
        Fp4& h = head[(size_t)cv.reg_combo[r] * 64 + i];
        h = h + cur * coeff_u[cv.reg_first[r] + i];
      }
      if (cv.reg_size[r] > head_len[cv.reg_combo[r]]) head_len[cv.reg_combo[r]] = cv.reg_size[r];
      cur = cur * mixv;
    }
    for (uint32_t i = 0; i < R0H_CHECK_SIZE; i++) {
      head[(size_t)n_combos * 64] = head[(size_t)n_combos * 64] + cur * coeff_u[cv.n_taps + i];
      cur = cur * mixv;
    }
    head_len[n_combos] = 1;
    std::vector<uint32_t> fix;
    for (uint32_t k = 0; k <= n_combos; k++)
      for (uint32_t i = 0; i < head_len[k]; i++)
        for (uint32_t q = 0; q < 4; q++) {
          fix.push_back((uint32_t)((((size_t)k << po2) + i) * 4 + q));
          fix.push_back(head[(size_t)k * 64 + i].e[q]);
        }
    R0H_REQUIRE(((size_t)(n_combos + 1) << po2) * 4 < ((size_t)1 << 32), "prove_segment: combos buffer exceeds 32-bit word indexing");
    r0h_buf* d_fix = nullptr;
    R0H_TRY(sc.alloc(ctx, fix.size() * 4, &d_fix));
    R0H_TRY(stage_h2d(ctx, d_fix->ptr, fix.data(), fix.size() * 4));
    uint32_t nf = (uint32_t)(fix.size() / 2);
    hipLaunchKernelGGL(sub_head_kernel, dim3((nf + 255) / 256), dim3(256), 0, ctx->stream, u32(combos), u32(d_fix), nf);
    R0H_TRY(launch_ok("sub_head_kernel"));
    sc.release(d_fix);
  }
  phase(ctx, "deep_divide");
  {
    std::vector<uint32_t> job_poly, job_pt;
    for (uint32_t k = 0; k <= n_combos; k++) {
      if (k < n_combos) {
        for (uint32_t b = cv.combo_begin[k]; b < cv.combo_begin[k + 1]; b++) {
          const Fp4 pt = scale(z, fpow(back_one, cv.combo_backs[b]));
          job_poly.push_back(k);
          job_pt.insert(job_pt.end(), pt.e, pt.e + 4);
        }
      } else {
        job_poly.push_back(k);
        job_pt.insert(job_pt.end(), z4.e, z4.e + 4);
      }
    }
    std::vector<uint32_t> rem(4 * job_poly.size());
    R0H_TRY(poly_divide_batch(ctx, combos, (uint32_t)n, job_poly.data(), job_pt.data(), (uint32_t)job_poly.size(), rem.data()));
    for (size_t j = 0; j < job_poly.size(); j++)
      R0H_REQUIRE(!(rem[4 * j] | rem[4 * j + 1] | rem[4 * j + 2] | rem[4 * j + 3]),
                  "prove_segment: DEEP quotient of combo %u has a non-zero remainder (witness violates the taps?)", job_poly[j]);
  }
  r0h_buf* fri_coeffs = nullptr;
  R0H_TRY(sc.alloc(ctx, n * 16, &fri_coeffs));
  R0H_TRY(r0h_eltwise_sum_extelem(ctx, fri_coeffs, combos, n_combos + 1, (uint32_t)n));
  R0H_TRY(r0h_batch_bit_reverse(ctx, fri_coeffs, 4, po2));
  sc.release(combos);

  phase(ctx, "fri_commit");
  struct Round { Tree tree; r0h_buf* evaluated; };
  std::vector<Round> rounds;
  const FriSchedule fri(n);
  for (const FriRound& fr : fri.rounds) {
    Round rd{Tree(fr.rows, R0H_FRI_FOLD * 4), nullptr};
    R0H_TRY(sc.alloc(ctx, fr.domain * 16, &rd.evaluated));
    R0H_TRY(r0h_batch_expand_into_evaluate_ntt(ctx, rd.evaluated, fri_coeffs, 4, log2u(fr.degree), 2));
    R0H_TRY(tree_build(ctx, sc, rd.tree, rd.evaluated));
    R0H_TRY(tree_commit(ctx, rd.tree, io));
    Fp4 fold_mix = io.rng.ext();
    r0h_buf* folded = nullptr;
    R0H_TRY(sc.alloc(ctx, fr.degree / R0H_FRI_FOLD * 16, &folded));
    R0H_TRY(r0h_fri_fold(ctx, folded, fri_coeffs, fold_mix.e, (uint32_t)(fr.degree / R0H_FRI_FOLD)));
    sc.release(fri_coeffs);
    fri_coeffs = folded;
    rounds.push_back(rd);
  }
  R0H_TRY(r0h_batch_bit_reverse(ctx, fri_coeffs, 4, log2u(fri.final_degree)));
  {
    std::vector<uint32_t> fc(4 * fri.final_degree);
    R0H_TRY(r0h_buf_d2h(ctx, fri_coeffs, 0, fc.data(), fc.size() * 4));
    io.write(fc.data(), fc.size());
    io.commit_elems(fc.data(), fc.size());
  }

  phase(ctx, "queries");
  {
    const uint32_t nq = R0H_QUERIES, n_trees = 4 + (uint32_t)rounds.size();
    std::vector<uint32_t> idx((size_t)n_trees * nq);
    for (uint32_t q = 0; q < nq; q++) {
      size_t pos = io.rng.bits(log2u(domain)) % domain;
      for (uint32_t t = 0; t < 4; t++) idx[(size_t)t * nq + q] = (uint32_t)pos;
      for (size_t r = 0; r < rounds.size(); r++) {
        pos = pos % rounds[r].tree.mp.rows;
        idx[(size_t)(4 + r) * nq + q] = (uint32_t)pos;
      }
    }
    r0h_buf* d_idx = nullptr;
    R0H_TRY(sc.alloc(ctx, idx.size() * 4, &d_idx));
    R0H_TRY(stage_h2d(ctx, d_idx->ptr, idx.data(), idx.size() * 4));
    std::vector<const Tree*> trees = {&g_accum.tree, &g_code.tree, &g_data.tree, &g_check.tree};
    for (Round& rd : rounds) trees.push_back(&rd.tree);
    std::vector<std::vector<uint32_t>> opened(n_trees);
    for (uint32_t t = 0; t < n_trees; t++) {
      r0h_buf view = buf_view(d_idx, (size_t)t * nq * 4, (size_t)nq * 4);
      R0H_TRY(tree_open(ctx, sc, *trees[t], &view, nq, opened[t]));
    }
    for (uint32_t q = 0; q < nq; q++)
      for (uint32_t t = 0; t < n_trees; t++) {
        size_t w = trees[t]->mp.opening_words();
        io.write(opened[t].data() + (size_t)q * w, w);
      }
  }
  phase(ctx, "end");
  R0H_TRY_HIP(hipStreamSynchronize(ctx->stream));
  Profile& pf = ctx->prof;
  pf.ms.assign(pf.names.size(), 0.f);
  for (size_t i = 0; i + 1 < pf.names.size(); i++) hipEventElapsedTime(&pf.ms[i], pf.events[i], pf.events[i + 1]);
  seal.swap(io.proof);
  return nullptr;
}

}

using namespace r0h;

extern "C" {

static const char* prove_segment_impl(r0h_ctx* ctx, const r0h_circuit* c, uint32_t po2, const r0h_buf* code, const r0h_code_commit* cc,
                                      const r0h_buf* data, const uint32_t* global, uint32_t* seal_out, size_t seal_cap, size_t* seal_words_out) {
  R0H_GUARD_BEGIN
  R0H_REQUIRE(ctx && c && (code || cc) && data && seal_words_out, "r0h_prove_segment: NULL argument");
  R0H_REQUIRE(global || r0h_circuit_n_global(c) == 0, "r0h_prove_segment: global is NULL");
  R0H_REQUIRE(po2 >= 9 && po2 <= R0H_MAX_PO2, "r0h_prove_segment: po2 %u outside [9, %u]", po2, R0H_MAX_PO2);
  R0H_REQUIRE(c->has_column_program, "r0h_prove_segment: the circuit has no accumulation program; drive the per-op entry points with your own accum step");
  R0H_TRY_HIP(hipSetDevice(ctx->device));
  std::vector<uint32_t> seal;
  {
    CircuitView cv;
    circuit_view(c, &cv);
    r0h_proof st(ctx, c, po2, cv);
    R0H_TRY(proof_begin(st, code, cc, data, global));
    if (c->n_late) R0H_TRY(proof_late(st, global + (cv.n_global - c->n_late)));
    r0h_buf* accum = nullptr;
    R0H_TRY(st.sc.alloc(ctx, ((size_t)cv.group_size[R0H_GROUP_ACCUM] << po2) * 4, &accum));
    const r0h_buf* code_cols = code;
    r0h_buf code_view;
    if (!code_cols && cc && cc->witness) { code_view = *cc->witness; code_cols = &code_view; }
    R0H_TRY(r0h_accum_public(ctx, c, po2, code_cols, data, st.global.data(), st.mix.data(), accum));
    R0H_TRY(proof_finish(st, accum, seal));
  }
  *seal_words_out = seal.size();
  R0H_REQUIRE(seal.size() <= seal_cap || !seal_out, "r0h_prove_segment: seal needs %zu words, capacity is %zu", seal.size(), seal_cap);
  if (seal_out) memcpy(seal_out, seal.data(), seal.size() * 4);
  return nullptr;
  R0H_GUARD_END
}

static const char* proof_begin_impl(r0h_ctx* ctx, const r0h_circuit* c, uint32_t po2, const r0h_buf* code, const r0h_code_commit* cc,
                                    const r0h_buf* data, const uint32_t* global, uint32_t* mix_out, r0h_proof** out) {
  R0H_GUARD_BEGIN
  R0H_REQUIRE(ctx && c && (code || cc) && data && out, "r0h_proof_begin: NULL argument");
  R0H_REQUIRE((global || r0h_circuit_n_global(c) == 0) && (mix_out || r0h_circuit_n_mix(c) == 0 || c->n_late), "r0h_proof_begin: NULL globals / mix_out");
  R0H_REQUIRE(po2 >= 9 && po2 <= R0H_MAX_PO2, "r0h_proof_begin: po2 %u outside [9, %u]", po2, R0H_MAX_PO2);
  R0H_TRY_HIP(hipSetDevice(ctx->device));
  CircuitView cv;
  circuit_view(c, &cv);
  r0h_proof* st = new r0h_proof(ctx, c, po2, cv);
  const char* err = proof_begin(*st, code, cc, data, global);
  if (err) { delete st; return err; }
  if (cv.n_mix && st->mix_drawn && mix_out) memcpy(mix_out, st->mix.data(), (size_t)cv.n_mix * 4);
  *out = st;
  return nullptr;
  R0H_GUARD_END
}

const char* r0h_prove_segment(r0h_ctx* ctx, const r0h_circuit* c, uint32_t po2, const r0h_buf* code, const r0h_buf* data,
                              const uint32_t* global, uint32_t* seal_out, size_t seal_cap, size_t* seal_words_out) {
  R0H_REQUIRE(code, "r0h_prove_segment: NULL argument");
  return prove_segment_impl(ctx, c, po2, code, nullptr, data, global, seal_out, seal_cap, seal_words_out);
}
const char* r0h_prove_segment_committed(r0h_ctx* ctx, const r0h_circuit* c, uint32_t po2, const r0h_code_commit* code, const r0h_buf* data,
                                        const uint32_t* global, uint32_t* seal_out, size_t seal_cap, size_t* seal_words_out) {
  R0H_REQUIRE(code, "r0h_prove_segment_committed: NULL argument");
  return prove_segment_impl(ctx, c, po2, nullptr, code, data, global, seal_out, seal_cap, seal_words_out);
}

const char* r0h_proof_begin(r0h_ctx* ctx, const r0h_circuit* c, uint32_t po2, const r0h_buf* code, const r0h_buf* data,
                            const uint32_t* global, uint32_t* mix_out, r0h_proof** out) {
  R0H_REQUIRE(code, "r0h_proof_begin: NULL argument");
  return proof_begin_impl(ctx, c, po2, code, nullptr, data, global, mix_out, out);
}
const char* r0h_proof_begin_committed(r0h_ctx* ctx, const r0h_circuit* c, uint32_t po2, const r0h_code_commit* code, const r0h_buf* data,
                                      const uint32_t* global, uint32_t* mix_out, r0h_proof** out) {
  R0H_REQUIRE(code, "r0h_proof_begin_committed: NULL argument");
  return proof_begin_impl(ctx, c, po2, nullptr, code, data, global, mix_out, out);
}

const char* r0h_code_commit_new(r0h_ctx* ctx, const r0h_buf* code, uint32_t count, uint32_t po2, r0h_code_commit** out) {
  R0H_GUARD_BEGIN
  R0H_REQUIRE(ctx && code && out, "r0h_code_commit_new: NULL argument");
  R0H_REQUIRE(count >= 1, "r0h_code_commit_new: the CODE group has no columns");
  R0H_REQUIRE(po2 >= 9 && po2 <= R0H_MAX_PO2, "r0h_code_commit_new: po2 %u outside [9, %u]", po2, R0H_MAX_PO2);
  R0H_TRY_HIP(hipSetDevice(ctx->device));
  std::unique_ptr<r0h_code_commit, const char* (*)(r0h_code_commit*)> cc(new r0h_code_commit(), r0h_code_commit_free);
  cc->ctx = ctx; cc->count = count; cc->po2 = po2; cc->hashfn = ctx->hashfn;
  ctx_retain(ctx);
  {
    Scope sc;
    Group g(count, (size_t)4 << po2);
    R0H_TRY(group_from_witness(ctx, sc, g, code, po2));
    WriteIop io(ctx->hashfn, &ctx->p2_host);
    R0H_TRY(tree_commit(ctx, g.tree, io));
    cc->top.swap(io.proof);
    R0H_TRY(r0h_buf_d2h(ctx, g.tree.nodes, 32, cc->root, 32));
    cc->coeffs = g.coeffs; cc->evaluated = g.evaluated; cc->nodes = g.tree.nodes;
    {
      const size_t bytes = ((size_t)count << po2) * 4;
      R0H_TRY(r0h_buf_alloc(ctx, bytes, &cc->witness));
      R0H_TRY_HIP(hipMemcpyAsync(cc->witness->ptr, code->ptr, bytes, hipMemcpyDeviceToDevice, ctx->stream));
      R0H_TRY_HIP(hipStreamSynchronize(ctx->stream));
    }
    sc.bufs.clear();
    for (r0h_buf* b : {cc->coeffs, cc->evaluated, cc->nodes}) { b->pooled = false; b->owned = true; }
  }
  *out = cc.release();
  return nullptr;
  R0H_GUARD_END
}
const char* r0h_code_commit_free(r0h_code_commit* cc) {
  if (!cc) return nullptr;
  if (cc->coeffs) r0h_buf_free(cc->coeffs);
  if (cc->evaluated) r0h_buf_free(cc->evaluated);
  if (cc->nodes) r0h_buf_free(cc->nodes);
  if (cc->witness) r0h_buf_free(cc->witness);
  r0h_ctx* ctx = cc->ctx;
  delete cc;
  if (ctx) ctx_release(ctx);
  return nullptr;
}
const char* r0h_code_commit_columns(const r0h_code_commit* cc, const r0h_buf** columns_out) {
  R0H_REQUIRE(cc && columns_out && cc->witness, "r0h_code_commit_columns: NULL argument");
  *columns_out = cc->witness;
  return nullptr;
}
const char* r0h_code_commit_root(const r0h_code_commit* cc, uint32_t root_out[8]) {
  R0H_REQUIRE(cc && root_out, "r0h_code_commit_root: NULL argument");
  memcpy(root_out, cc->root, 32);
  return nullptr;
}

const char* r0h_proof_finish(r0h_proof* proof, const r0h_buf* accum, uint32_t* seal_out, size_t seal_cap, size_t* seal_words_out) {
  R0H_GUARD_BEGIN
  R0H_REQUIRE(proof && accum && seal_words_out, "r0h_proof_finish: NULL argument");
  R0H_TRY_HIP(hipSetDevice(proof->ctx->device));
  std::vector<uint32_t> seal;
  const char* err = proof_finish(*proof, accum, seal);
  delete proof;
  if (err) return err;
  *seal_words_out = seal.size();
  R0H_REQUIRE(seal.size() <= seal_cap || !seal_out, "r0h_proof_finish: seal needs %zu words, capacity is %zu", seal.size(), seal_cap);
  if (seal_out) memcpy(seal_out, seal.data(), seal.size() * 4);
  return nullptr;
  R0H_GUARD_END
}

const char* r0h_proof_data_root(const r0h_proof* proof, uint32_t root_out[8]) {
  R0H_REQUIRE(proof && root_out, "r0h_proof_data_root: NULL argument");
  memcpy(root_out, proof->data_root, 32);
  return nullptr;
}
const char* r0h_proof_late(r0h_proof* proof, const uint32_t* late_globals, uint32_t* mix_out) {
  R0H_GUARD_BEGIN
  R0H_REQUIRE(proof && (mix_out || !proof->cv.n_mix), "r0h_proof_late: NULL argument");
  R0H_REQUIRE(proof->circ->n_late, "r0h_proof_late: this circuit has no late public inputs");
  R0H_TRY_HIP(hipSetDevice(proof->ctx->device));
  R0H_TRY(proof_late(*proof, late_globals));
  if (proof->cv.n_mix) memcpy(mix_out, proof->mix.data(), (size_t)proof->cv.n_mix * 4);
  return nullptr;
  R0H_GUARD_END
}
const char* r0h_proof_globals(const r0h_proof* proof, uint32_t* globals_out) {
  R0H_REQUIRE(proof && globals_out, "r0h_proof_globals: NULL argument");
  memcpy(globals_out, proof->global.data(), proof->global.size() * 4);
  return nullptr;
}

const char* r0h_proof_abort(r0h_proof* proof) {
  delete proof;
  return nullptr;
}
const char* r0h_proof_shrink(r0h_proof* proof, size_t* bytes_freed_out) {
  R0H_GUARD_BEGIN
  R0H_REQUIRE(proof, "r0h_proof_shrink: NULL argument");
  size_t freed = 0;
  if (proof->g_data.evaluated) {
    R0H_TRY_HIP(hipSetDevice(proof->ctx->device));
    R0H_TRY_HIP(hipStreamSynchronize(proof->ctx->stream));
    freed = proof->g_data.evaluated->bytes;
    proof->sc.release(proof->g_data.evaluated);
    proof->g_data.evaluated = nullptr;
    proof->g_data.tree.matrix = nullptr;
  }
  if (bytes_freed_out) *bytes_freed_out = freed;
  return nullptr;
  R0H_GUARD_END
}
size_t r0h_proof_resident_bytes(const r0h_proof* proof) {
  if (!proof) return 0;
  size_t total = 0;
  for (const r0h_buf* b : proof->sc.bufs) total += b->bytes;
  return total;
}

const char* r0h_code_root(r0h_ctx* ctx, const r0h_buf* code, uint32_t count, uint32_t po2, uint32_t root_out[8]) {
  R0H_GUARD_BEGIN
  R0H_REQUIRE(ctx && code && root_out, "r0h_code_root: NULL argument");
  R0H_REQUIRE(count >= 1, "r0h_code_root: the CODE group has no columns");
  R0H_REQUIRE(po2 >= 9 && po2 <= R0H_MAX_PO2, "r0h_code_root: po2 %u outside [9, %u]", po2, R0H_MAX_PO2);
  R0H_TRY_HIP(hipSetDevice(ctx->device));
  Scope sc;
  Group g(count, (size_t)4 << po2);
  R0H_TRY(group_from_witness(ctx, sc, g, code, po2));
  return r0h_buf_d2h(ctx, g.tree.nodes, 32, root_out, 32);
  R0H_GUARD_END
}

const char* r0h_last_profile(r0h_ctx* ctx, const char*** names_out, const float** ms_out, uint32_t* n_out) {
// ... 9 lines not shown
```

### hyperfridge-r0_amd/csrc/session.cpp

```cpp
#include <stdlib.h>
#include <string.h>

#include <algorithm>
#include <atomic>
#include <chrono>
#include <condition_variable>
#include <deque>
#include <map>
#include <memory>
#include <mutex>
#include <thread>
#include <utility>
#include <vector>

#include "circuit.hpp"
#include "receipt_types.hpp"

using namespace r0h;

namespace {
using Clock = std::chrono::steady_clock;
double seconds(Clock::time_point a, Clock::time_point b) { return std::chrono::duration<double>(b - a).count(); }

struct CodeCommits {
// ... 160 lines not shown
  const Run& join() {
    if (thread_.joinable()) thread_.join();
    run_.vm = vm_.get();
    return run_;
  }

 private:
  void execute() {
    r0h_vm* vm = vm_.get();
    const char* err = nullptr;
    try {
      size_t handed = 0;
      for (int finished = 0; !finished && !err;) {
        std::vector<std::unique_ptr<Produced>> back;
        {
          std::unique_lock<std::mutex> lk(mu_);
          while (!stop_ && queue_.size() >= queue_depth_) cv_.wait(lk);
          if (stop_) break;
          back.swap(returned_);
        }
        for (auto& b : back) vm_recycle_trace(vm, b->rows, b->bounds);
        const Clock::time_point t0 = Clock::now();
        err = r0h_vm_run_segment(vm, &lim_, &finished, &run_.exit_kind, &run_.exit_code);
        run_.executor_s += seconds(t0, Clock::now());
        if (err) break;
        for (; handed < r0h_vm_n_segments(vm) && !err; handed++) {
          std::unique_ptr<Produced> p(new Produced());
          const size_t i = handed;
          err = r0h_vm_segment_info(vm, i, &p->info);
          if (!err) err = r0h_vm_segment_claim(vm, i, &p->claim);
          if (err) break;
          p->index = i;
          if (i == 0) run_.first_pre = p->info.pre;
          if (trace_mode_) vm_take_trace(vm, i, p->rows, p->bounds);
          const bool own = i % parts_ == part_;
          std::unique_lock<std::mutex> lk(mu_);
          while (own && !stop_ && queue_.size() >= queue_depth_ + 2) cv_.wait(lk);
          if (!own || stop_) vm_recycle_trace(vm, p->rows, p->bounds);
          if (stop_) break;
          if (!own) continue;
          queue_.push_back(std::move(p));
          cv_.notify_all();
        }
      }
    } catch (const std::exception& ex) {
      err = make_error("exception in the executor: %s", ex.what());
    } catch (...) {
      err = make_error("unknown exception in the executor");
    }
    std::lock_guard<std::mutex> lk(mu_);
    producer_err_ = err;
    producer_done_ = true;
    cv_.notify_all();
  }

  RowBuffers& rows_;
  const r0h_vm_limits lim_;
  const bool trace_mode_;
  const uint32_t part_, parts_;
  std::unique_ptr<r0h_vm, VmFree> vm_;
  Run run_;
  std::mutex mu_;
  std::condition_variable cv_;
  std::deque<std::unique_ptr<Produced>> queue_;
  std::vector<std::unique_ptr<Produced>> returned_;
  bool producer_done_ = false, stop_ = false;
  size_t queue_depth_ = 2;
  const char* producer_err_ = nullptr;
  std::thread thread_;
};

template <class Fn, class OnError>
const char* run_lanes(const std::vector<r0h_ctx*>& lanes, Fn fn, OnError on_error) {
  std::atomic<const char*> first(nullptr);
  auto lane = [&](r0h_ctx* lctx) {
    const char* err = nullptr;
    try {
      err = fn(lctx);
    } catch (const std::exception& ex) {
      err = make_error("exception in a prover lane: %s", ex.what());
    } catch (...) {
      err = make_error("unknown exception in a prover lane");
    }
    if (!err) return;
    const char* none = nullptr;
    if (!first.compare_exchange_strong(none, err)) r0h_free_error(err);
    on_error();
  };
  std::vector<std::thread> workers;
  for (size_t k = 1; k < lanes.size(); k++) workers.emplace_back(lane, lanes[k]);
  lane(lanes[0]);
  for (std::thread& t : workers) t.join();
  return first;
}
}

namespace r0h {
void session_rows_free(r0h_ctx* ctx) {
  delete (RowPool*)ctx->session_rows;
  ctx->session_rows = nullptr;
}
}


constexpr uint32_t RECORD_WORDS = (R0H_TRACE_GLOBALS - R0H_TRACE_LATE_GLOBALS) + 8;
static_assert(RECORD_WORDS == R0H_SESSION_RECORD_WORDS, "R0H_SESSION_RECORD_WORDS out of step");

struct ProofAbort { void operator()(r0h_proof* p) const { r0h_proof_abort(p); } };

struct Pending {
  size_t index = 0;
  r0h_ctx* lctx = nullptr;
  DevBuf data;
  std::unique_ptr<r0h_proof, ProofAbort> proof;
  r0h_code_commit* cc = nullptr;
  uint32_t po2 = 0;
  std::vector<uint32_t> global;
  uint32_t root[8] = {0};
  r0h_receipt_claim claim;
  std::vector<uint32_t> seal;
  bool done = false;
};

struct r0h_session {
  r0h_ctx* ctx = nullptr;
  const r0h_circuit* c = nullptr;
  bool trace_mode = false;
  uint32_t part = 0, parts = 1;
  size_t n_segments = 0;
  std::mutex commit_mu, result_mu;
  std::vector<Pending> pending;
  CodeCommits commits;
  std::vector<uint8_t> journal;
  std::vector<uint8_t> elf;
  uint8_t image_id[32] = {0};
  uint64_t cycles = 0;
  r0h_session_stats stats = {0, 0, 0, 0, 0, 0, 0};
  uint64_t resident_limit = 0, resident_evaluations = 0;
  Clock::time_point t_begin;
  std::vector<r0h_ctx*> lane_ctx;
  ~r0h_session() {
    pending.clear();
    if (ctx) ctx_release(ctx);
  }
};

namespace {
const char* commit_segment(r0h_session* ses, RowBuffers& rows, const Produced& seg, DevBuf& data, std::vector<uint32_t>& global, Pending& pend) {
  const r0h_circuit* c = ses->c;
  const Clock::time_point t0 = Clock::now();
  rows.pin(seg.rows.data(), seg.rows.capacity() * sizeof(r0h_preflight_row));
  const r0h_trace_segment ts = {seg.info.index + 1, seg.info.closing, seg.info.pre.pc, 0};
  R0H_TRY(r0h_trace_witgen(pend.lctx, seg.rows.data(), seg.rows.size(), seg.bounds.data(), seg.bounds.size(), pend.po2, &ts, data.get(), global.data()));
  R0H_TRY(r0h_logup_multiplicities(pend.lctx, c, pend.po2, data.get(), global.data()));
  const Clock::time_point t1 = Clock::now();
  r0h_proof* proof = nullptr;
  R0H_TRY(r0h_proof_begin_committed(pend.lctx, c, pend.po2, pend.cc, data.get(), global.data(), nullptr, &proof));
  pend.proof.reset(proof);
  R0H_TRY(r0h_proof_data_root(proof, pend.root));
  {
    const uint64_t evaluations = ((uint64_t)c->group_size[R0H_GROUP_DATA] << pend.po2) * 16;
    std::unique_lock<std::mutex> lk(ses->result_mu);
    const bool lean = ses->resident_evaluations + evaluations > ses->resident_limit;
    if (lean) ses->stats.lean_segments++;
    else ses->resident_evaluations += evaluations;
    lk.unlock();
    if (lean) R0H_TRY(r0h_proof_shrink(proof, nullptr));
  }
  const Clock::time_point t2 = Clock::now();
  pend.global = global;
  pend.data = std::move(data);
  std::lock_guard<std::mutex> lk(ses->result_mu);
  ses->stats.witgen_ms += 1e3 * seconds(t0, t1);
  ses->stats.prove_ms += 1e3 * seconds(t1, t2);
  ses->pending.push_back(std::move(pend));
  return nullptr;
}

const char* prove_synthetic_segment(r0h_session* ses, const Produced& seg, DevBuf& data, std::vector<uint32_t>& global, std::vector<uint32_t>& seal, Pending& pend) {
  const r0h_circuit* c = ses->c;
  const Clock::time_point t0 = Clock::now();
  {
    DevBuf code;
    R0H_TRY(code.alloc(pend.lctx, ((size_t)c->group_size[R0H_GROUP_CODE] << pend.po2) * 4));
    R0H_TRY(r0h_witgen_public(pend.lctx, c, pend.po2, 0x5E55 + seg.index, global.data(), code.get(), data.get()));
  }
  const Clock::time_point t1 = Clock::now();
  size_t words = 0;
  seal.resize((size_t)1 << 20);
  R0H_TRY(r0h_prove_segment_committed(pend.lctx, c, pend.po2, pend.cc, data.get(), global.data(), seal.data(), seal.size(), &words));
  const Clock::time_point t2 = Clock::now();
  pend.seal.assign(seal.begin(), seal.begin() + words);
  pend.done = true;
  std::lock_guard<std::mutex> lk(ses->result_mu);
  ses->stats.witgen_ms += 1e3 * seconds(t0, t1);
  ses->stats.prove_ms += 1e3 * seconds(t1, t2);
  ses->stats.segments++;
  ses->pending.push_back(std::move(pend));
  return nullptr;
}

const char* take_segments(r0h_session* ses, Feed& feed, RowBuffers& rows, r0h_ctx* lctx) {
  const r0h_circuit* c = ses->c;
  std::vector<uint32_t> seal, global(c->n_global);
  for (;;) {
    Feed::Segment seg;
    R0H_TRY(feed.next(seg));
    if (!seg) return nullptr;
    const uint64_t rows_needed = ses->trace_mode ? seg->rows.size() + seg->bounds.size() : seg->info.user_cycles + seg->info.paging_cycles;
    DevBuf data;
    Pending pend;
    pend.index = seg->index;
    pend.lctx = lctx;
    pend.claim = seg->claim;
    pend.po2 = trace_size(rows_needed);
    if (ses->trace_mode && pend.po2 < R0H_TRACE_MIN_PO2) pend.po2 = R0H_TRACE_MIN_PO2;
    uint8_t cd[32];
    claim_digest(seg->claim, cd);
    std::fill(global.begin(), global.end(), 0u);
    claim_globals(cd, global.data());
    R0H_TRY(data.alloc(lctx, ((size_t)c->group_size[R0H_GROUP_DATA] << pend.po2) * 4));
    {
      std::lock_guard<std::mutex> lk(ses->commit_mu);
      R0H_TRY(ses->commits.get(lctx, c, pend.po2, &pend.cc));
    }
    R0H_TRY(ses->trace_mode ? commit_segment(ses, rows, *seg, data, global, pend) : prove_synthetic_segment(ses, *seg, data, global, seal, pend));
  }
}

uint32_t lane_count() {
  uint32_t n = 2;
  if (const char* v = getenv("R0H_SESSION_LANES")) n = (uint32_t)strtoul(v, nullptr, 10);
  return n < 1 ? 1 : n > 4 ? 4 : n;
}
}

extern "C" {

const char* r0h_last_session_stats(r0h_ctx* ctx, r0h_session_stats* out) {
  R0H_REQUIRE(ctx && out, "r0h_last_session_stats: NULL argument");
  *out = ctx->session;
  return nullptr;
}

const char* r0h_session_free(r0h_session* s) {
  delete s;
  return nullptr;
}

const char* r0h_session_begin(r0h_ctx* ctx, const r0h_circuit* c, const uint8_t* elf, size_t elf_len, const uint32_t* input_words, size_t n_input, uint32_t segment_po2,
                              uint64_t max_cycles, uint32_t part, uint32_t parts, r0h_session** session_out) {
  R0H_GUARD_BEGIN
  R0H_REQUIRE(ctx && c && elf && session_out && (input_words || !n_input), "r0h_prove_elf: NULL argument");
  R0H_TRY(require_poseidon2(ctx, "r0h_prove_elf / r0h_session_begin"));
  R0H_REQUIRE(parts >= 1 && part < parts, "r0h_prove_elf_part: part %u of %u", part, parts);
  const bool trace_mode = !memcmp(c->info, "R0HIP_TRACE:v5__", 16);
  R0H_REQUIRE(segment_po2 >= 9 && segment_po2 <= (trace_mode ? R0H_TRACE_MAX_PO2 : R0H_MAX_PO2), "r0h_prove_elf: segment_po2 %u outside [9, %u]", segment_po2,
              (unsigned)(trace_mode ? R0H_TRACE_MAX_PO2 : R0H_MAX_PO2));
  R0H_REQUIRE(c->has_column_program, "r0h_prove_elf: the circuit has no column program (CODE columns, accumulation)");
  R0H_REQUIRE(c->n_global >= 8, "r0h_prove_elf: the circuit exposes %u public inputs, a claim needs 8", c->n_global);
  if (trace_mode)
    R0H_REQUIRE(c->n_global == R0H_TRACE_GLOBALS && c->n_late == R0H_TRACE_LATE_GLOBALS && c->group_size[R0H_GROUP_DATA] == R0H_TRACE_COLUMNS,
                "r0h_prove_elf: this trace circuit is not the one the library was built for");
  else
    R0H_REQUIRE(c->n_late == 0, "r0h_prove_elf: a circuit with late public inputs other than the trace circuit");
  if (!max_cycles) max_cycles = R0H_DEFAULT_SESSION_LIMIT;
  std::unique_ptr<r0h_session> ses(new r0h_session());
  ses->ctx = ctx;
  ctx_retain(ctx);
  ses->c = c;
  ses->trace_mode = trace_mode;
  ses->part = part;
  ses->parts = parts;
  ses->t_begin = Clock::now();
  if (trace_mode && ctx->image_circuit && part == 0) ses->elf.assign(elf, elf + elf_len);
  ses->resident_limit = ctx->session_resident_limit;
  if (!ses->resident_limit) {
    size_t free_b = 0, total_b = 0;
    R0H_TRY_HIP(hipSetDevice(ctx->device));
    R0H_TRY_HIP(hipMemGetInfo(&free_b, &total_b));
    ses->resident_limit = total_b / 8;
  }
  r0h_vm_limits lim;
  memset(&lim, 0, sizeof lim);
  lim.segment_po2 = segment_po2;
  lim.max_cycles = max_cycles;
  lim.keep_trace = lim.boundary_rows = trace_mode ? 1 : 0;

  RowBuffers rows(trace_mode ? pool_of(ctx) : nullptr);
  Feed feed(rows, lim, part, parts);
  R0H_TRY(feed.start(elf, elf_len, input_words, n_input));

  ses->lane_ctx.assign(lane_count(), ctx);
  for (size_t k = 1; k < ses->lane_ctx.size(); k++) R0H_TRY(ctx_helper(ctx, k - 1, &ses->lane_ctx[k]));
  feed.set_lanes(ses->lane_ctx.size());
  R0H_TRY(run_lanes(ses->lane_ctx, [&](r0h_ctx* lctx) { return take_segments(ses.get(), feed, rows, lctx); }, [&] { feed.stop(); }));

  const Feed::Run& run = feed.join();
  R0H_REQUIRE(run.exit_kind != R0H_VM_LIMIT, "r0h_prove_elf: the guest did not halt within %llu cycles (session limit)", (unsigned long long)max_cycles);
  R0H_REQUIRE(run.exit_code == 0, "r0h_prove_elf: the guest exited with code %u", run.exit_code);
  ses->n_segments = r0h_vm_n_segments(run.vm);
  std::sort(ses->pending.begin(), ses->pending.end(), [](const Pending& a, const Pending& b) { return a.index < b.index; });
  size_t own = 0;
  for (size_t i = part; i < ses->n_segments; i += parts) own++;
  R0H_REQUIRE(ses->pending.size() == own, "r0h_prove_elf: %zu of this rank's %zu segments were committed", ses->pending.size(), own);
  ses->cycles = r0h_vm_cycles(run.vm);
  const uint8_t* journal; size_t journal_len;
  R0H_TRY(r0h_vm_journal(run.vm, &journal, &journal_len));
  ses->journal.assign(journal, journal + journal_len);
  system_state_digest(run.first_pre, ses->image_id);
  ses->stats.cycles = ses->cycles;
  ses->stats.executor_s = run.executor_s;
  *session_out = ses.release();
  return nullptr;
  R0H_GUARD_END
}

size_t r0h_session_n_segments(const r0h_session* s) { return s ? s->n_segments : 0; }

const char* r0h_session_records(const r0h_session* s, uint32_t* indices_out, uint32_t* records_out, size_t capacity, size_t* n_out) {
  R0H_REQUIRE(s && n_out, "r0h_session_records: NULL argument");
  *n_out = s->trace_mode ? s->pending.size() : 0;
  if (!s->trace_mode) return nullptr;
  R0H_REQUIRE(capacity >= s->pending.size() && indices_out && records_out, "r0h_session_records: room for %zu records wanted", s->pending.size());
  const uint32_t n_early = R0H_TRACE_GLOBALS - R0H_TRACE_LATE_GLOBALS;
  for (size_t k = 0; k < s->pending.size(); k++) {
    indices_out[k] = (uint32_t)s->pending[k].index;
    memcpy(records_out + k * RECORD_WORDS, s->pending[k].global.data(), n_early * 4);
    memcpy(records_out + k * RECORD_WORDS + n_early, s->pending[k].root, 32);
  }
  return nullptr;
}

namespace {
const char* finish_segment(r0h_session* s, Pending& p, const uint32_t challenge[16], std::vector<uint32_t>& mix, std::vector<uint32_t>& seal, size_t* words) {
  const r0h_circuit* c = s->c;
  DevBuf data = std::move(p.data);
  memcpy(p.global.data() + R0H_TRACE_GAMMA, challenge, 64);
  const r0h_buf* code_cols = nullptr;
  R0H_TRY(r0h_code_commit_columns(p.cc, &code_cols));
  R0H_TRY(r0h_logup_totals(p.lctx, c, p.po2, code_cols, data.get(), p.global.data()));
  R0H_TRY(r0h_proof_late(p.proof.get(), p.global.data() + (R0H_TRACE_GLOBALS - R0H_TRACE_LATE_GLOBALS), mix.data()));
  DevBuf accum;
  R0H_TRY(accum.alloc(p.lctx, ((size_t)c->group_size[R0H_GROUP_ACCUM] << p.po2) * 4));
  R0H_TRY(r0h_accum_public(p.lctx, c, p.po2, code_cols, data.get(), p.global.data(), mix.data(), accum.get()));
  return r0h_proof_finish(p.proof.release(), accum.get(), seal.data(), seal.size(), words);
}
}

const char* r0h_session_finish(r0h_session* s, const uint32_t* all_records, size_t n_records, r0h_receipt** receipt_out, uint8_t image_id_out[32], uint64_t* cycles_out) {
  R0H_GUARD_BEGIN
  R0H_REQUIRE(s && receipt_out, "r0h_session_finish: NULL argument");
  std::vector<uint32_t> image_seal;
  if (s->trace_mode) {
    R0H_REQUIRE(all_records && n_records == s->n_segments, "r0h_session_finish: the session has %zu segments, %zu records were given", s->n_segments, n_records);
    const uint32_t n_early = R0H_TRACE_GLOBALS - R0H_TRACE_LATE_GLOBALS;
    for (const Pending& p : s->pending)
      R0H_REQUIRE(!memcmp(all_records + p.index * RECORD_WORDS, p.global.data(), n_early * 4) && !memcmp(all_records + p.index * RECORD_WORDS + n_early, p.root, 32),
                  "r0h_session_finish: record %zu is not the one this rank committed", p.index);
    uint32_t challenge[16];
    session_challenge(all_records, n_records, challenge);
    std::atomic<bool> failed(false);
    auto lane = [&](r0h_ctx* lctx) -> const char* {
      std::vector<uint32_t> seal((size_t)1 << 20), mix(s->c->n_mix);
      size_t words = 0;
      if (lctx == s->ctx && !s->elf.empty() && s->ctx->image_circuit) {
        R0H_TRY(r0h_prove_image(s->ctx, s->ctx->image_circuit, s->elf.data(), s->elf.size(), challenge, seal.data(), seal.size(), &words));
        image_seal.assign(seal.begin(), seal.begin() + words);
      }
      for (Pending& p : s->pending) {
        if (p.lctx != lctx || p.done) continue;
        if (failed) return nullptr;
        const Clock::time_point t0 = Clock::now();
        R0H_TRY(finish_segment(s, p, challenge, mix, seal, &words));
        std::lock_guard<std::mutex> lk(s->result_mu);
        p.seal.assign(seal.begin(), seal.begin() + words);
        p.done = true;
        s->stats.prove_ms += 1e3 * seconds(t0, Clock::now());
        s->stats.segments++;
      }
      return nullptr;
    };
    R0H_TRY(run_lanes(s->lane_ctx, lane, [&] { failed = true; }));
  }
  r0h_receipt* rc = nullptr;
  R0H_TRY(r0h_receipt_new(R0H_RECEIPT_COMPOSITE, nullptr, 0, &rc));
  std::unique_ptr<r0h_receipt, const char* (*)(r0h_receipt*)> rc_guard(rc, r0h_receipt_free);
  for (Pending& p : s->pending) {
    R0H_REQUIRE(p.done, "r0h_prove_elf: segment %zu was never proved", p.index);
    R0H_TRY(r0h_receipt_add_segment_claim(rc, p.seal.data(), p.seal.size(), (uint32_t)p.index, &p.claim, nullptr));
  }
  rc->journal = s->journal;
  rc->image_seal = image_seal;
  if (image_id_out) memcpy(image_id_out, s->image_id, 32);
  if (cycles_out) *cycles_out = s->cycles;
  s->stats.wall_s = seconds(s->t_begin, Clock::now());
  s->ctx->session = s->stats;
  *receipt_out = rc_guard.release();
  return nullptr;
  R0H_GUARD_END
}

static const char* prove_session(r0h_ctx* ctx, const r0h_circuit* c, const uint8_t* elf, size_t elf_len, const uint32_t* input_words, size_t n_input, uint32_t segment_po2,
                                 uint64_t max_cycles, uint32_t part, uint32_t parts, r0h_receipt** receipt_out, uint8_t image_id_out[32], uint64_t* cycles_out) {
  r0h_session* s = nullptr;
  R0H_TRY(r0h_session_begin(ctx, c, elf, elf_len, input_words, n_input, segment_po2, max_cycles, part, parts, &s));
  std::unique_ptr<r0h_session> guard(s);
  std::vector<uint32_t> indices(s->pending.size() + 1), records((s->pending.size() + 1) * RECORD_WORDS);
  size_t n = 0;
  R0H_TRY(r0h_session_records(s, indices.data(), records.data(), s->pending.size(), &n));
  return r0h_session_finish(s, records.data(), n, receipt_out, image_id_out, cycles_out);
}

const char* r0h_prove_elf(r0h_ctx* ctx, const r0h_circuit* c, const uint8_t* elf, size_t elf_len, const uint32_t* input_words, size_t n_input, uint32_t segment_po2,
                          uint64_t max_cycles, r0h_receipt** receipt_out, uint8_t image_id_out[32], uint64_t* cycles_out) {
  R0H_GUARD_BEGIN
  R0H_REQUIRE(receipt_out, "r0h_prove_elf: NULL argument");
  return prove_session(ctx, c, elf, elf_len, input_words, n_input, segment_po2, max_cycles, 0, 1, receipt_out, image_id_out, cycles_out);
  R0H_GUARD_END
}

const char* r0h_prove_elf_part(r0h_ctx* ctx, const r0h_circuit* c, const uint8_t* elf, size_t elf_len, const uint32_t* input_words, size_t n_input, uint32_t segment_po2,
                               uint64_t max_cycles, uint32_t part, uint32_t parts, r0h_receipt** receipt_out, uint8_t image_id_out[32], uint64_t* cycles_out) {
  R0H_GUARD_BEGIN
  R0H_REQUIRE(receipt_out && c, "r0h_prove_elf_part: NULL argument");
  R0H_REQUIRE(parts == 1 || c->n_late == 0, "r0h_prove_elf_part: the segments of a trace-circuit session share one challenge: ranks use r0h_session_begin / r0h_session_records / r0h_session_finish");
  return prove_session(ctx, c, elf, elf_len, input_words, n_input, segment_po2, max_cycles, part, parts, receipt_out, image_id_out, cycles_out);
  R0H_GUARD_END
}

}
```

Measured before the change: 40.46.

## Generate circuit-specific logup kernels and reuse own-accumulator terms across phases

Adds a per-circuit generated HIP module for the log-derivative argument. It provides a multiplicity-counting kernel that bins into shared-memory histograms, a chain-term kernel, and an own-accumulator kernel, all replacing the generic tape interpreter. The session now launches the multiplicity count before the data commit and checks its verdict afterwards, so the count can overlap with commit work. The own-accumulator terms computed for the totals are kept and reused when building the accumulator columns, instead of being recomputed. The cost is more precompiled code objects and extra device memory held between the two phases.

Measured after the change: 40.63, median of 3. No clear change (+0.4%).

```diff
diff --git a/__graft_entry__.py b/__graft_entry__.py
--- a/__graft_entry__.py
+++ b/__graft_entry__.py
@@ -32,11 +32,16 @@
     return os.path.join(ROOT, "circuits", name + ".checkwitness.hsaco")
 
 
+def logup_code_object_path(name):
+    return os.path.join(ROOT, "circuits", name + ".logup.hsaco")
+
+
 def term_names_path(name):
     return os.path.join(ROOT, "circuits", name + ".terms.txt")
 
 
 NAMED = ("trace", "image")
+LOGUP = ("trace", "image")
 
 
 def build():
@@ -62,7 +67,10 @@
     for name in PRECOMPILED:
         blob = np.fromfile(circuit_blob_path(name), dtype=np.uint32)
         for emit, target, suffix in ((r0.emit_eval_check_source, code_object_path(name), ".evalcheck.hip"),
-                                     (r0.emit_check_witness_source, check_code_object_path(name), ".checkwitness.hip")):
+                                     (r0.emit_check_witness_source, check_code_object_path(name), ".checkwitness.hip"),
+                                     (r0.emit_logup_source, logup_code_object_path(name), ".logup.hip")):
+            if emit is r0.emit_logup_source and name not in LOGUP:
+                continue
             src = emit(blob)
             src_path = os.path.join(ROOT, "circuits", name + suffix)
             digest = hashlib.sha256(src.encode()).hexdigest()
@@ -85,7 +93,7 @@
     needed = [os.path.join(ROOT, "hyperfridge-r0_amd", "libr0hip.so"), os.path.join(ROOT, "hyperfridge-r0_amd", "r0h_prove"),
               os.path.join(ROOT, "hyperfridge-r0_amd", "r0h_verify"), os.path.join(ROOT, "hyperfridge-r0_amd", "r0h_preprocess"),
               os.path.join(ROOT, "oracle", "liborc.so"), os.path.join(ROOT, "circuits", "guest_camt53.elf")] + [circuit_blob_path(n) for n in CIRCUITS] + [code_object_path(n) for n in PRECOMPILED] + [
-                  check_code_object_path(n) for n in PRECOMPILED] + [term_names_path(n) for n in NAMED]
+                  check_code_object_path(n) for n in PRECOMPILED] + [logup_code_object_path(n) for n in LOGUP] + [term_names_path(n) for n in NAMED]
     if not all(os.path.exists(p) for p in needed):
         build()
 
diff --git a/hyperfridge-r0_amd/__init__.py b/hyperfridge-r0_amd/__init__.py
--- a/hyperfridge-r0_amd/__init__.py
+++ b/hyperfridge-r0_amd/__init__.py
@@ -218,6 +218,12 @@
     "r0h_circuit_n_terms": ([_vp], _u32),
 }
 EXPORTED_SYMBOLS = sorted(list(_SIGNATURES) + list(_PLAIN))
+_INTERNAL = {
+    "r0hi_circuit_emit_hip_logup": [_vp, _sz, _c.POINTER(_c.c_char_p)],
+    "r0hi_logup_totals_terms": [_vp, _vp, _u32, _vp, _vp, _vp, _pp],
+    "r0hi_accum_public_terms": [_vp, _vp, _u32, _vp, _vp, _vp, _vp, _vp, _vp],
+    "r0hi_logup_count_later": [_vp, _vp, _u32, _vp, _vp],
+}
 
 _lib = None
 
@@ -254,6 +260,12 @@
             fn = getattr(h, name)
             fn.argtypes = args
             fn.restype = res
+        for name, args in _INTERNAL.items():
+            fn = getattr(h, name)
+            fn.argtypes = args
+            fn.restype = _vp
+        h.r0hi_logup_terms_free.argtypes = [_vp]
+        h.r0hi_logup_terms_free.restype = None
         _lib = h
     return _lib
 
@@ -365,6 +377,15 @@
     a, p = _u32arr(blob)
     out = ctypes.c_char_p()
     _check(lib().r0h_circuit_emit_hip_check(p, a.size, ctypes.byref(out)))
+    src = out.value.decode()
+    lib().r0h_free_error(ctypes.cast(out, _vp))
+    return src
+
+
+def emit_logup_source(blob):
+    a, p = _u32arr(blob)
+    out = ctypes.c_char_p()
+    _check(lib().r0hi_circuit_emit_hip_logup(p, a.size, ctypes.byref(out)))
     src = out.value.decode()
     lib().r0h_free_error(ctypes.cast(out, _vp))
     return src
@@ -1280,6 +1301,26 @@
         _check(lib().r0h_logup_totals(self.ctx, circuit.handle, po2, code.handle, data.handle, g.ctypes.data_as(_vp)))
         return g
 
+    def logup_totals_with_terms(self, circuit, po2, code, data, glob):
+        g = np.ascontiguousarray(glob, dtype=np.uint32).copy()
+        h = _vp()
+        _check(lib().r0hi_logup_totals_terms(self.ctx, circuit.handle, po2, code.handle, data.handle, g.ctypes.data_as(_vp), ctypes.byref(h)))
+        return g, h
+
+    def accum_public_with_terms(self, circuit, po2, code, data, glob, mix, terms):
+        g, pg = _u32arr(glob)
+        m, pm = _u32arr(mix)
+        out = self.alloc(circuit.group_size[GROUP_ACCUM] * (1 << po2))
+        try:
+            _check(lib().r0hi_accum_public_terms(self.ctx, circuit.handle, po2, code.handle, data.handle, pg, pm, out.handle, terms))
+        except R0HipError:
+            out.free()
+            raise
+        return out
+
+    def free_logup_terms(self, terms):
+        lib().r0hi_logup_terms_free(terms)
+
     def logup_multiplicities(self, circuit, po2, data, glob):
         g = np.ascontiguousarray(glob if len(glob) else [0], dtype=np.uint32)
         _check(lib().r0h_logup_multiplicities(self.ctx, circuit.handle, po2, data.handle, g.ctypes.data_as(_vp)))
diff --git a/hyperfridge-r0_amd/csrc/circuit.hip b/hyperfridge-r0_amd/csrc/circuit.hip
--- a/hyperfridge-r0_amd/csrc/circuit.hip
+++ b/hyperfridge-r0_amd/csrc/circuit.hip
@@ -604,6 +604,207 @@
   return os.str();
 }
 
+static const char* LOGUP_PRELUDE = R"SRC(// the log-derivative argument: rows of the trace
+struct F4 { u32 e[4]; };
+__device__ __forceinline__ F4 f4add(F4 a, F4 b) { return F4{{fadd(a.e[0], b.e[0]), fadd(a.e[1], b.e[1]), fadd(a.e[2], b.e[2]), fadd(a.e[3], b.e[3])}}; }
+__device__ __forceinline__ F4 f4scale(F4 a, u32 s) { return F4{{fmul(a.e[0], s), fmul(a.e[1], s), fmul(a.e[2], s), fmul(a.e[3], s)}}; }
+// x^4 = 11: products summed in 64 bits (at most four: 4 p^2 < 2^64), one reduction per coefficient
+__device__ __forceinline__ F4 f4mul(F4 a, F4 b) {
+  const u32 c4 = fred64((u64)a.e[1] * b.e[3] + (u64)a.e[2] * b.e[2] + (u64)a.e[3] * b.e[1]);
+  const u32 c5 = fred64((u64)a.e[2] * b.e[3] + (u64)a.e[3] * b.e[2]);
+  const u32 c6 = fred64((u64)a.e[3] * b.e[3]);
+  F4 r;
+  r.e[0] = fred64((u64)a.e[0] * b.e[0] + (u64)FP_BETA * c4);
+  r.e[1] = fred64((u64)a.e[0] * b.e[1] + (u64)a.e[1] * b.e[0] + (u64)FP_BETA * c5);
+  r.e[2] = fred64((u64)a.e[0] * b.e[2] + (u64)a.e[1] * b.e[1] + (u64)a.e[2] * b.e[0] + (u64)FP_BETA * c6);
+  r.e[3] = fred64((u64)a.e[0] * b.e[3] + (u64)a.e[1] * b.e[2] + (u64)a.e[2] * b.e[1] + (u64)a.e[3] * b.e[0]);
+  return r;
+}
+__device__ __forceinline__ u32 fneg(u32 a) { return a ? FP_P - a : 0u; }
+__device__ __forceinline__ u32 finv(u32 a) {  // a^(p - 2)
+  u32 r = FP_ONE;
+#pragma unroll 1
+  for (u32 n = FP_P - 2u; n; n >>= 1) {
+    if (n & 1u) r = fmul(r, a);
+    a = fmul(a, a);
+  }
+  return r;
+}
+// through the tower Fp2[y]/(y^2 - x) over Fp[x]/(x^2 - 11): a = A + yB, 1/a = (A - yB)/(A^2 - x B^2)
+__device__ __forceinline__ F4 f4inv(F4 a) {
+  const u32 A0 = a.e[0], A1 = a.e[2], B0 = a.e[1], B1 = a.e[3];
+  const u32 A2_0 = fadd(fmul(A0, A0), fmul(FP_BETA, fmul(A1, A1))), A2_1 = fmul(fadd(A0, A0), A1);
+  const u32 B2_0 = fadd(fmul(B0, B0), fmul(FP_BETA, fmul(B1, B1))), B2_1 = fmul(fadd(B0, B0), B1);
+  const u32 D0 = fsub(A2_0, fmul(FP_BETA, B2_1)), D1 = fsub(A2_1, B2_0);
+  const u32 n = finv(fsub(fmul(D0, D0), fmul(FP_BETA, fmul(D1, D1))));
+  const u32 I0 = fmul(D0, n), I1 = fneg(fmul(D1, n));
+  F4 r;
+  r.e[0] = fadd(fmul(A0, I0), fmul(FP_BETA, fmul(A1, I1)));
+  r.e[2] = fadd(fmul(A0, I1), fmul(A1, I0));
+  r.e[1] = fneg(fadd(fmul(B0, I0), fmul(FP_BETA, fmul(B1, I1))));
+  r.e[3] = fneg(fadd(fmul(B0, I1), fmul(B1, I0)));
+  return r;
+}
+// n0/d0 + n1/d1 + n2/d2 + n3/d3 as one fraction: one inversion per accumulator and row
+__device__ __forceinline__ F4 logup_term(const u32* num, const F4* d) {
+  const F4 d01 = f4mul(d[0], d[1]), d23 = f4mul(d[2], d[3]);
+  const F4 top = f4add(f4mul(f4add(f4scale(d[1], num[0]), f4scale(d[0], num[1])), d23), f4mul(f4add(f4scale(d[3], num[2]), f4scale(d[2], num[3])), d01));
+  return f4mul(top, f4inv(f4mul(d01, d23)));
+}
+#define DATA(col) data[((size_t)(col) << po2) + r]
+#define CODE(col) code[((size_t)(col) << po2) + r]
+#define ACCUM(col) accum[((size_t)(col) << po2) + r]
+// One lookup of table T (1: the 16-bit range, 2: the byte AND, told by its tag) into the workgroup's bins.  Zero is not counted
+// (it is what the other entries leave); a slot gated off (numerator 0) is tallied in `gated`, a value binned in `binned`.  Bit 0 of
+// *err: a numerator that is neither 0 nor 1; bit 1: a numerator of 1 with a value outside the table.
+template <int T> __device__ __forceinline__ void logup_bin(u32 num, u32 value, u32* bins, u32* __restrict__ hist, u32* __restrict__ err, u32& gated, u32& binned) {
+  if (num != FP_ONE) {
+    if (num) atomicOr(err, 1u);
+    else gated++;
+    return;
+  }
+  u32 v = fmul(fneg(value), 1u);
+  if (T == 2) {
+    v -= LOGUP_TAG_AND;
+    if (v >> 24 || ((v & 255u) & ((v >> 8) & 255u)) != v >> 16) { atomicOr(err, 2u); return; }
+    v &= 0xffffu;
+  } else if (v >> 16) {
+    atomicOr(err, 2u);
+    return;
+  }
+  if (!v) return;
+  binned++;
+  if (v < LOGUP_HOT) atomicAdd(bins + (T - 1) * LOGUP_HOT + v, 1u);
+  else atomicAdd(hist + (T - 1) * 65536u + v, 1u);
+}
+)SRC";
+
+static void emit_form(const Lf& lf, std::ostringstream& os) {
+  if (lf.terms.empty()) { os << "0u"; return; }
+  for (size_t k = 0; k + 1 < lf.terms.size(); k++) os << "fadd(";
+  for (size_t k = 0; k < lf.terms.size(); k++) {
+    const LfTerm& t = lf.terms[k];
+    std::ostringstream coef;
+    if (t.global) coef << "fmul(" << enc(t.coef) << "u, pub.glob[" << t.global - 1 << "])";
+    else coef << enc(t.coef) << "u";
+    if (k) os << ", ";
+    if (t.col) os << "fmul(" << coef.str() << ", " << (((t.col - 1) >> 28) == R0H_GROUP_CODE ? "CODE(" : "DATA(") << ((t.col - 1) & 0xfffffu) << "))";
+    else os << coef.str();
+    if (k) os << ")";
+  }
+}
+static void emit_logup_term(const LogupAcc& a, std::ostringstream& os) {
+  os << "    u32 num[4];\n    F4 d[4];\n";
+  for (size_t f = 0; f < a.fr.size(); f++) {
+    os << "    num[" << f << "] = ";
+    emit_form(a.fr[f].num, os);
+    os << ";\n";
+    for (size_t q = 0; q < a.fr[f].parts.size(); q++) {
+      const LogupPart& part = a.fr[f].parts[q];
+      std::ostringstream v, ch;
+      emit_form(part.lf, v);
+      if (part.ch_kind) {
+        const char* src = part.ch_kind == 1 ? "pub.mix[" : "pub.glob[";
+        const uint32_t at = part.ch_kind == 1 ? 4 * part.ch_idx : part.ch_idx;
+        ch << "F4{{" << src << at << "], " << src << at + 1 << "], " << src << at + 2 << "], " << src << at + 3 << "]}}";
+      }
+      os << "    d[" << f << "]";
+      if (!q && !part.ch_kind) os << " = F4{{" << v.str() << ", 0u, 0u, 0u}};\n";
+      else if (!q) os << " = f4scale(" << ch.str() << ", " << v.str() << ");\n";
+      else if (!part.ch_kind) os << ".e[0] = fadd(d[" << f << "].e[0], " << v.str() << ");\n";
+      else os << " = f4add(d[" << f << "], f4scale(" << ch.str() << ", " << v.str() << "));\n";
+    }
+  }
+  os << "    const F4 t = logup_term(num, d);\n";
+}
+
+static std::string emit_logup_source(const r0h_circuit* c, std::string* suffix = nullptr) {
+  const Logup& lg = c->logup;
+  const uint32_t n_chain = lg.n_chain, n_acc = (uint32_t)lg.accs.size(), n_tables = (uint32_t)lg.tables.size();
+  std::ostringstream os;
+  os << PRELUDE;
+  os << "#define FP_ONE " << ONE << "u\n#define FP_BETA " << BETA_M << "u\n#define LOGUP_TAG_AND " << R0H_TAG_AND << "u\n#define LOGUP_HOT 4096u\n";
+  os << LOGUP_PRELUDE;
+  os << "// accumulators: " << n_acc << " (" << n_chain << " chain links), tables: " << n_tables << "\n";
+  os << "struct LogupPub { u32 glob[" << std::max(1u, c->n_global) << "]; u32 mix[" << std::max(1u, c->n_mix) << "]; };\n\n";
+  if (n_tables >= 1 && n_tables <= 2) {
+    os << "extern \"C\" __global__ __launch_bounds__(256) void logup_count@(u32* __restrict__ hist, u32* __restrict__ err, const u32* __restrict__ data,\n"
+          "    const LogupPub pub, u32 po2) {\n"
+          "  __shared__ u32 bins[" << n_tables << "u * LOGUP_HOT];\n"
+          "  __shared__ u32 counted[2];\n"
+          "  if (threadIdx.x < 2u) counted[threadIdx.x] = 0u;\n"
+          "  for (u32 i = threadIdx.x; i < " << n_tables << "u * LOGUP_HOT; i += 256u) bins[i] = 0u;\n"
+          "  __syncthreads();\n"
+          "  const u32 r = blockIdx.x * 256u + threadIdx.x;\n"
+          "  u32 gated0 = 0u, gated1 = 0u, binned0 = 0u, binned1 = 0u;\n"
+          "  if (r < (1u << po2)) {\n";
+    std::vector<const LogupFraction*> looks;
+    for (const LogupAcc& a : lg.accs)
+      for (const LogupFraction& f : a.fr)
+        if (f.table) looks.push_back(&f);
+    constexpr size_t LOGUP_GROUP = 32;
+    for (size_t g0 = 0; g0 < looks.size(); g0 += LOGUP_GROUP) {
+      const size_t g1 = std::min(looks.size(), g0 + LOGUP_GROUP);
+      if (g0) os << "    __builtin_amdgcn_sched_barrier(0);\n";
+      for (size_t k = g0; k < g1; k++) {
+        os << "    const u32 n" << k << " = ";
+        emit_form(looks[k]->num, os);
+        os << ", v" << k << " = ";
+        emit_form(looks[k]->parts[1].lf, os);
+        os << ";\n";
+      }
+      for (size_t k = g0; k < g1; k++) os << "    logup_bin<" << looks[k]->table << ">(n" << k << ", v" << k << ", bins, hist, err, gated" << looks[k]->table - 1 << ", binned" << looks[k]->table - 1 << ");\n";
+    }
+    os << "  }\n"
+          "  if (gated0) atomicAdd(bins, gated0);\n"
+          "  if (gated1) atomicAdd(bins + " << (n_tables - 1) << "u * LOGUP_HOT, gated1);\n"
+          "  if (gated0 + binned0) atomicAdd(counted, gated0 + binned0);\n"
+          "  if (gated1 + binned1) atomicAdd(counted + 1, gated1 + binned1);\n"
+          "  __syncthreads();\n"
+          "  if (threadIdx.x < 2u && counted[threadIdx.x]) atomicAdd(err + 1u + threadIdx.x, counted[threadIdx.x]);\n"
+          "  for (u32 i = threadIdx.x; i < " << n_tables << "u * LOGUP_HOT; i += 256u) {\n"
+          "    const u32 cnt = bins[i];\n"
+          "    if (cnt) atomicAdd(hist + (i / LOGUP_HOT) * 65536u + (i % LOGUP_HOT), cnt);\n"
+          "  }\n"
+          "}\n\n";
+  }
+  os << "extern \"C\" __global__ __launch_bounds__(256) void logup_terms_chain@(u32* __restrict__ accum, u32* __restrict__ row_total, const u32* __restrict__ code,\n"
+        "    const u32* __restrict__ data, const LogupPub pub, u32 po2) {\n"
+        "  const u32 r = blockIdx.x * 256u + threadIdx.x;\n"
+        "  if (r >= (1u << po2)) return;\n"
+        "  F4 run = F4{{0u, 0u, 0u, 0u}};\n";
+  for (uint32_t j = 0; j < n_chain; j++) {
+    if (j) os << "  __builtin_amdgcn_sched_barrier(0);\n";
+    os << "  {\n";
+    emit_logup_term(lg.accs[j], os);
+    os << "    run = f4add(run, t);\n";
+    for (uint32_t i = 0; i < 4; i++) os << "    ACCUM(" << 4 * j + i << ") = run.e[" << i << "];\n";
+    os << "  }\n";
+  }
+  os << "  *(uint4*)(row_total + 4 * (size_t)r) = make_uint4(run.e[0], run.e[1], run.e[2], run.e[3]);\n}\n\n";
+  if (n_acc > n_chain) {
+    os << "extern \"C\" __global__ __launch_bounds__(256) void logup_terms_own@(u32* __restrict__ own_terms, const u32* __restrict__ code, const u32* __restrict__ data,\n"
+          "    const LogupPub pub, u32 po2) {\n"
+          "  const u32 r = blockIdx.x * 256u + threadIdx.x;\n"
+          "  if (r >= (1u << po2)) return;\n";
+    for (uint32_t j = n_chain; j < n_acc; j++) {
+      if (j > n_chain) os << "  __builtin_amdgcn_sched_barrier(0);\n";
+      os << "  {\n";
+      emit_logup_term(lg.accs[j], os);
+      os << "    *(uint4*)(own_terms + 4 * (((size_t)" << j - n_chain << " << po2) + r)) = make_uint4(t.e[0], t.e[1], t.e[2], t.e[3]);\n  }\n";
+    }
+    os << "}\n";
+  }
+  std::string text = os.str();
+  uint64_t h = 0xcbf29ce484222325ull;
+  for (unsigned char ch : text) h = (h ^ ch) * 0x100000001b3ull;
+  char tail[24];
+  snprintf(tail, sizeof tail, "_%016llx", (unsigned long long)h);
+  for (size_t at = text.find('@'); at != std::string::npos; at = text.find('@', at)) text.replace(at, 1, tail);
+  if (suffix) *suffix = tail;
+  return text;
+}
+
 static const char* compile_in_process(const std::string& src, std::vector<char>& code) {
   hiprtcProgram prog;
   hiprtcResult r = hiprtcCreateProgram(&prog, src.c_str(), "eval_check.hip", 0, nullptr, nullptr);
@@ -705,6 +906,7 @@
   void operator()(r0h_circuit* circuit) const {
     if (circuit->module) (void)hipModuleUnload(circuit->module);
     if (circuit->check_module) (void)hipModuleUnload(circuit->check_module);
+    if (circuit->logup_module) (void)hipModuleUnload(circuit->logup_module);
     delete circuit;
   }
 };
@@ -720,6 +922,7 @@
   std::vector<char> code;
   if (code_object_path) {
     R0H_TRY(read_code_object("r0h_circuit_load", code_object_path, code));
+    c->code_object_path = code_object_path;
   } else {
     R0H_TRY(compile_in_process(emit_source(c.get()), code));
   }
@@ -806,8 +1009,97 @@
   R0H_GUARD_END
 }
 
+const char* r0hi_circuit_emit_hip_logup(const uint32_t* blob, size_t n_words, char** source_out) {
+  R0H_GUARD_BEGIN
+  R0H_REQUIRE(blob && source_out, "r0hi_circuit_emit_hip_logup: NULL argument");
+  r0h_circuit c;
+  R0H_TRY(parse_blob(&c, blob, n_words));
+  R0H_REQUIRE(!c.logup.accs.empty(), "r0hi_circuit_emit_hip_logup: the circuit has no LOGUP section");
+  std::string src = emit_logup_source(&c);
+  char* out = (char*)malloc(src.size() + 1);
+  R0H_REQUIRE(out, "r0hi_circuit_emit_hip_logup: out of memory");
+  memcpy(out, src.c_str(), src.size() + 1);
+  *source_out = out;
+  return nullptr;
+  R0H_GUARD_END
+}
+
 }
 namespace r0h {
+uint32_t logup_reads(const r0h_circuit* c, uint32_t a0, uint32_t a1) {
+  uint32_t reads = 0;
+  auto form = [&](const Lf& lf) {
+    for (const LfTerm& t : lf.terms) {
+      if (t.global) reads |= 2u;
+      if (t.col && ((t.col - 1) >> 28) == R0H_GROUP_CODE) reads |= 1u;
+    }
+  };
+  for (uint32_t j = a0; j < a1; j++)
+    for (const LogupFraction& f : c->logup.accs[j].fr) {
+      form(f.num);
+      for (const LogupPart& q : f.parts) {
+        form(q.lf);
+        if (q.ch_kind) reads |= q.ch_kind == 1 ? 4u : 2u;
+      }
+    }
+  return reads;
+}
+
+const char* logup_kernels(const r0h_circuit* c, const hipFunction_t** fn_out) {
+  std::lock_guard<std::mutex> lk(c->logup_mu);
+  *fn_out = c->logup_fn;
+  if (c->logup_module) return nullptr;
+  R0H_REQUIRE(c->n_global + c->n_mix + 2 <= LOGUP_PUB_MAX_WORDS, "the log-derivative kernels take the public inputs and the mix as arguments: %u + %u words are more than %u",
+              c->n_global, c->n_mix, LOGUP_PUB_MAX_WORDS);
+  R0H_TRY_HIP(hipSetDevice(c->ctx->device));
+  std::string suffix;
+  const std::string src = emit_logup_source(c, &suffix);
+  const std::string names[3] = {"logup_count" + suffix, "logup_terms_chain" + suffix, "logup_terms_own" + suffix};
+  const bool have[3] = {c->logup.tables.size() >= 1 && c->logup.tables.size() <= 2, true, c->logup.accs.size() > c->logup.n_chain};
+  hipModule_t module = nullptr;
+  hipFunction_t fn[3] = {nullptr, nullptr, nullptr};
+  auto load = [&](const char* image) -> bool {
+    if (hipModuleLoadData(&module, image) != hipSuccess) { (void)hipGetLastError(); module = nullptr; return false; }
+    for (int k = 0; k < 3; k++)
+      if (have[k] && hipModuleGetFunction(&fn[k], module, names[k].c_str()) != hipSuccess) {
+        (void)hipGetLastError();
+        (void)hipModuleUnload(module);
+        module = nullptr;
+        return false;
+      }
+    return true;
+  };
+  static const std::string EC = ".evalcheck.hsaco";
+  const std::string& ec_path = c->code_object_path;
+  if (ec_path.size() > EC.size() && !ec_path.compare(ec_path.size() - EC.size(), EC.size(), EC)) {
+    const std::string path = ec_path.substr(0, ec_path.size() - EC.size()) + ".logup.hsaco";
+    std::vector<char> image;
+    if (FILE* f = fopen(path.c_str(), "rb")) {
+      fclose(f);
+      if (!read_code_object("the log-derivative kernels", path.c_str(), image)) (void)load(image.data());
+    }
+  }
+  if (!module) {
+    static std::mutex cache_mu;
+    static std::map<std::string, std::shared_ptr<const std::vector<char>>> cache;
+    std::shared_ptr<const std::vector<char>> code;
+    {
+      std::lock_guard<std::mutex> ck(cache_mu);
+      auto it = cache.find(src);
+      if (it == cache.end()) {
+        std::vector<char> fresh;
+        R0H_TRY(compile_in_process(src, fresh));
+        it = cache.emplace(src, std::make_shared<const std::vector<char>>(std::move(fresh))).first;
+      }
+      code = it->second;
+    }
+    R0H_REQUIRE(load(code->data()), "the log-derivative kernels: the compiled text does not load, or lacks one of its kernels");
+  }
+  for (int k = 0; k < 3; k++) c->logup_fn[k] = fn[k];
+  c->logup_module = module;
+  return nullptr;
+}
+
 const char* sponge_plant(r0h_ctx* ctx, const r0h_circuit* c, uint32_t po2, const uint32_t* words, size_t n_words, r0h_buf* data) {
   R0H_REQUIRE(ctx && c && data && c->has_sponge && (words || !n_words), "sponge_plant: NULL argument, or a circuit without the sponge component");
   const size_t n = (size_t)1 << po2, n_perm = n_words ? (n_words + P2_RATE - 1) / P2_RATE : 1, rows = n_perm * R0H_SPONGE_PERIOD;
diff --git a/hyperfridge-r0_amd/csrc/circuit.hpp b/hyperfridge-r0_amd/csrc/circuit.hpp
--- a/hyperfridge-r0_amd/csrc/circuit.hpp
+++ b/hyperfridge-r0_amd/csrc/circuit.hpp
@@ -89,6 +89,10 @@
   mutable std::mutex check_mu;
   mutable hipModule_t check_module = nullptr;
   mutable std::vector<hipFunction_t> check_kernels;
+  std::string code_object_path;
+  mutable std::mutex logup_mu;
+  mutable hipModule_t logup_module = nullptr;
+  mutable hipFunction_t logup_fn[3] = {nullptr, nullptr, nullptr};
 };
 
 namespace r0h {
@@ -96,5 +100,23 @@
 const char* sponge_plant(r0h_ctx* ctx, const r0h_circuit* c, uint32_t po2, const uint32_t* words, size_t n_words, r0h_buf* data);
 const char* require_witness(const char* caller, r0h_ctx* ctx, const r0h_circuit* c, uint32_t po2, const r0h_buf* accum, const r0h_buf* code, const r0h_buf* data,
                             const uint32_t* global, const uint32_t* mix);
-const char* logup_accum(r0h_ctx* ctx, const r0h_circuit* c, uint32_t po2, const r0h_buf* code, const r0h_buf* data, const uint32_t* global, const uint32_t* mix, r0h_buf* accum);
+enum LogupKernel { LOGUP_COUNT = 0, LOGUP_CHAIN = 1, LOGUP_OWN = 2 };
+constexpr uint32_t LOGUP_PUB_MAX_WORDS = 960;
+const char* logup_kernels(const r0h_circuit* c, const hipFunction_t** fn_out);
+uint32_t logup_reads(const r0h_circuit* c, uint32_t a0, uint32_t a1);
+
+struct LogupTerms {
+  DevBuf buf;
+  const r0h_circuit* c = nullptr;
+  const void* data = nullptr;
+  uint32_t po2 = 0;
+  std::vector<uint32_t> global;
+};
+const char* logup_totals(r0h_ctx* ctx, const r0h_circuit* c, uint32_t po2, const r0h_buf* code, const r0h_buf* data, uint32_t* global_io, LogupTerms* terms);
+const char* logup_accum(r0h_ctx* ctx, const r0h_circuit* c, uint32_t po2, const r0h_buf* code, const r0h_buf* data, const uint32_t* global, const uint32_t* mix, r0h_buf* accum,
+                        const LogupTerms* terms = nullptr);
+const char* logup_count_launch(r0h_ctx* ctx, const r0h_circuit* c, uint32_t po2, r0h_buf* data, const uint32_t* global, DevBuf* hist);
+const char* logup_count_verdict(r0h_ctx* ctx, const r0h_circuit* c, const DevBuf& hist);
+const char* prove_segment_with_terms(r0h_ctx* ctx, const r0h_circuit* c, uint32_t po2, const r0h_buf* code, const r0h_buf* data, const uint32_t* global, const LogupTerms* terms,
+                                     uint32_t* seal_out, size_t seal_capacity_words, size_t* seal_words_out);
 }
diff --git a/hyperfridge-r0_amd/csrc/image.cpp b/hyperfridge-r0_amd/csrc/image.cpp
--- a/hyperfridge-r0_amd/csrc/image.cpp
+++ b/hyperfridge-r0_amd/csrc/image.cpp
@@ -107,8 +107,9 @@
   R0H_TRY_HIP(hipMemsetAsync(first_flag, 0, 4 * n * 4, ctx->stream));
   for (size_t j = 0; j < 4; j++)
     R0H_TRY_HIP(hipMemcpy2DAsync(first_flag + j * n, (size_t)R0H_SPONGE_PERIOD * 4, flags.data() + j * n_blocks, 4, 4, n_blocks, hipMemcpyHostToDevice, ctx->stream));
-  R0H_TRY(r0h_logup_totals(ctx, c, po2, code.get(), data.get(), global.data()));
-  return r0h_prove_segment(ctx, c, po2, code.get(), data.get(), global.data(), seal_out, seal_capacity_words, seal_words_out);
+  LogupTerms terms;
+  R0H_TRY(logup_totals(ctx, c, po2, code.get(), data.get(), global.data(), &terms));
+  return prove_segment_with_terms(ctx, c, po2, code.get(), data.get(), global.data(), &terms, seal_out, seal_capacity_words, seal_words_out);
   R0H_GUARD_END
 }
 
diff --git a/hyperfridge-r0_amd/csrc/logup.hip b/hyperfridge-r0_amd/csrc/logup.hip
--- a/hyperfridge-r0_amd/csrc/logup.hip
+++ b/hyperfridge-r0_amd/csrc/logup.hip
@@ -1,5 +1,5 @@
 #include <algorithm>
-#include <map>
+#include <set>
 
 #include "../../include/r0hip_circuit.h"
 #include "circuit.hpp"
@@ -7,203 +7,12 @@
 namespace r0h {
 
 namespace {
-struct Tape {
-  std::vector<uint32_t> words;
-  std::vector<const uint32_t*> cols;
-  std::vector<Fp4> ch;
-  std::vector<uint32_t> acc_begin;
-};
-
-const char* build_tape(const r0h_circuit* c, uint32_t po2, const r0h_buf* code, const r0h_buf* data, const uint32_t* global, const uint32_t* mix, Tape* t, bool lookups_only = false) {
-  std::map<uint32_t, uint32_t> col_index;
-  std::map<uint64_t, uint32_t> ch_index;
-  t->ch.push_back(fp4_one());
-  auto form = [&](const Lf& lf) -> const char* {
-    t->words.push_back((uint32_t)lf.terms.size());
-    for (const LfTerm& term : lf.terms) {
-      uint32_t coef = enc(term.coef);
-      if (term.global) {
-        R0H_REQUIRE(global, "log-derivative accumulation: a form reads a public input and none were given");
-        coef = mul(coef, global[term.global - 1]);
-      }
-      uint32_t col = 0;
-      if (term.col) {
-        const uint32_t ref = term.col - 1;
-        auto it = col_index.find(ref);
-        if (it == col_index.end()) {
-          const r0h_buf* src = (ref >> 28) == R0H_GROUP_CODE ? code : data;
-          R0H_REQUIRE(src, "log-derivative accumulation: a form reads the %s group and none was given", (ref >> 28) == R0H_GROUP_CODE ? "CODE" : "DATA");
-          it = col_index.emplace(ref, (uint32_t)t->cols.size()).first;
-          t->cols.push_back(u32(src) + ((size_t)(ref & 0xfffffu) << po2));
-        }
-        col = it->second + 1;
-      }
-      t->words.push_back(coef);
-      t->words.push_back(col);
-    }
-    return nullptr;
-  };
-  for (const LogupAcc& a : c->logup.accs) {
-    t->acc_begin.push_back((uint32_t)t->words.size());
-    for (const LogupFraction& f : a.fr) {
-      if (lookups_only && !f.table) continue;
-      t->words.push_back(f.table);
-      R0H_TRY(form(f.num));
-      t->words.push_back((uint32_t)f.parts.size());
-      for (const LogupPart& q : f.parts) {
-        uint32_t idx = 0;
-        if (q.ch_kind) {
-          const uint64_t key = (uint64_t)q.ch_kind << 32 | q.ch_idx;
-          auto it = ch_index.find(key);
-          if (it == ch_index.end()) {
-            const uint32_t* src = q.ch_kind == 1 ? mix + 4 * (size_t)q.ch_idx : global + q.ch_idx;
-            R0H_REQUIRE(q.ch_kind == 1 ? mix != nullptr : global != nullptr, "log-derivative accumulation: a challenge is read from %s and none were given", q.ch_kind == 1 ? "the mix" : "the public inputs");
-            it = ch_index.emplace(key, (uint32_t)t->ch.size()).first;
-            t->ch.push_back(Fp4{{src[0], src[1], src[2], src[3]}});
-          }
-          idx = it->second;
-        }
-        t->words.push_back(idx);
-        R0H_TRY(form(q.lf));
-      }
-    }
-  }
-  t->acc_begin.push_back((uint32_t)t->words.size());
-  return nullptr;
-}
-
-struct DeviceTape {
-  DevBuf buf;
-  const uint32_t* words = nullptr;
-  const uint32_t* const* cols = nullptr;
-  const Fp4* ch = nullptr;
-};
-const char* upload_tape(r0h_ctx* ctx, const Tape& t, DeviceTape* d) {
-  const size_t w_bytes = (t.words.size() * 4 + 15) & ~(size_t)15, c_bytes = (t.cols.size() * sizeof(void*) + 15) & ~(size_t)15, h_bytes = t.ch.size() * 16;
-  R0H_TRY(d->buf.alloc(ctx, w_bytes + c_bytes + h_bytes));
-  char* base = (char*)d->buf->ptr;
-  R0H_TRY(stage_h2d(ctx, base, t.words.data(), t.words.size() * 4));
-  R0H_TRY(stage_h2d(ctx, base + w_bytes, t.cols.data(), t.cols.size() * sizeof(void*)));
-  R0H_TRY(stage_h2d(ctx, base + w_bytes + c_bytes, t.ch.data(), h_bytes));
-  d->words = (const uint32_t*)base;
-  d->cols = (const uint32_t* const*)(base + w_bytes);
-  d->ch = (const Fp4*)(base + w_bytes + c_bytes);
-  return nullptr;
-}
-
-__device__ __forceinline__ uint32_t eval_form(const uint32_t* __restrict__ tape, uint32_t& at, const uint32_t* const* __restrict__ cols, uint32_t r) {
-  const uint32_t n = tape[at++];
-  uint32_t acc = 0;
-  for (uint32_t k = 0; k < n; k++) {
-    const uint32_t coef = tape[at], col = tape[at + 1];
-    at += 2;
-    acc = add(acc, col ? mul(coef, cols[col - 1][r]) : coef);
-  }
-  return acc;
-}
-
-constexpr uint32_t HOT = 4096;
-
-__global__ __launch_bounds__(256) void logup_count_kernel(uint32_t* __restrict__ hist , uint32_t* __restrict__ err, const uint32_t* __restrict__ tape,
-                                                          uint32_t tape_end, const uint32_t* const* __restrict__ cols, uint32_t n, uint32_t n_tables) {
-  __shared__ uint32_t hot[2][HOT];
-  for (uint32_t i = threadIdx.x; i < 2 * HOT; i += 256) (&hot[0][0])[i] = 0;
-  __syncthreads();
+__global__ void logup_mult_kernel(uint32_t* __restrict__ column, const uint32_t* __restrict__ hist, const uint32_t* __restrict__ counted, uint32_t total, uint32_t n) {
   const uint32_t r = blockIdx.x * 256u + threadIdx.x;
-  uint32_t gated[2] = {0, 0};
-  if (r < n) {
-    uint32_t at = 0;
-    while (at < tape_end) {
-      const uint32_t table = tape[at++];
-      const uint32_t num = eval_form(tape, at, cols, r);
-      const uint32_t n_parts = tape[at++];
-      uint32_t value = 0;
-      for (uint32_t q = 0; q < n_parts; q++) {
-        at++;
-        const uint32_t v = eval_form(tape, at, cols, r);
-        if (q == 1) value = v;
-      }
-      if (!table || table > n_tables) continue;
-      if (num != ONE) {
-        if (num) atomicOr(err, 1u);
-        else gated[table - 1]++;
-        continue;
-      }
-      uint32_t v = dec(neg(value));
-      if (table == R0H_TABLE_AND) {
-        v -= R0H_TAG_AND;
-        if (v >> 24 || ((v & 255u) & ((v >> 8) & 255u)) != v >> 16) { atomicOr(err, 2u); continue; }
-        v &= 0xffffu;
-      } else if (v >> 16) {
-        atomicOr(err, 2u);
-        continue;
-      }
-      if (!v) continue;
-      if (v < HOT) atomicAdd(&hot[table - 1][v], 1u);
-      else atomicAdd(&hist[(size_t)(table - 1) * 65536 + v], 1u);
-    }
-  }
-  if (gated[0]) atomicAdd(&hot[0][0], gated[0]);
-  if (gated[1]) atomicAdd(&hot[1][0], gated[1]);
-  __syncthreads();
-  for (uint32_t i = threadIdx.x; i < 2 * HOT; i += 256) {
-    const uint32_t cnt = (&hot[0][0])[i];
-    if (cnt) atomicAdd(&hist[(size_t)(i / HOT) * 65536 + (i % HOT)], cnt);
-  }
-}
-__global__ void logup_mult_kernel(uint32_t* __restrict__ column, const uint32_t* __restrict__ hist, uint32_t total, uint32_t n) {
-  __shared__ uint32_t part[256];
-  const uint32_t r = blockIdx.x * 256u + threadIdx.x;
-  if (blockIdx.x == 0) {
-    uint32_t s = 0;
-    for (uint32_t i = threadIdx.x; i < 65536u; i += 256) s += hist[i];
-    part[threadIdx.x] = s;
-    __syncthreads();
-    for (uint32_t k = 128; k; k >>= 1) {
-      if (threadIdx.x < k) part[threadIdx.x] += part[threadIdx.x + k];
-      __syncthreads();
-    }
-  }
   if (r >= n) return;
   uint32_t v = r < 65536u ? hist[r] : 0u;
-  if (r == 0) v = total - part[0];
+  if (r == 0) v = total - *counted;
   column[r] = enc(v);
-}
-
-__global__ __launch_bounds__(256) void logup_term_kernel(uint32_t* __restrict__ accum, uint32_t* __restrict__ row_total, uint32_t* __restrict__ own_terms,
-                                                         const uint32_t* __restrict__ tape, const uint32_t* const* __restrict__ cols, const Fp4* __restrict__ ch,
-                                                         uint32_t a0, uint32_t a1, uint32_t n_chain, uint32_t po2) {
-  const uint32_t r = blockIdx.x * 256u + threadIdx.x, n = 1u << po2;
-  if (r >= n) return;
-  uint32_t at = 0;
-  Fp4 run = fp4_zero();
-  for (uint32_t j = a0; j < a1; j++) {
-    Fp4 d[4];
-    uint32_t num[4];
-    for (uint32_t f = 0; f < 4; f++) {
-      at++;
-      num[f] = eval_form(tape, at, cols, r);
-      const uint32_t n_parts = tape[at++];
-      Fp4 den = fp4_zero();
-      for (uint32_t q = 0; q < n_parts; q++) {
-        const uint32_t ci = tape[at++];
-        const uint32_t v = eval_form(tape, at, cols, r);
-        if (ci == 0) den.e[0] = add(den.e[0], v);
-        else den = den + scale(ch[ci], v);
-      }
-      d[f] = den;
-    }
-    const Fp4 d01 = d[0] * d[1], d23 = d[2] * d[3];
-    const Fp4 top = (scale(d[1], num[0]) + scale(d[0], num[1])) * d23 + (scale(d[3], num[2]) + scale(d[2], num[3])) * d01;
-    const Fp4 term = top * fp4_inv(d01 * d23);
-    if (j < n_chain) {
-      run = run + term;
-      for (uint32_t i = 0; i < 4; i++) accum[((size_t)(4 * j + i) << po2) + r] = run.e[i];
-    } else {
-      *(uint4*)(own_terms + 4 * ((size_t)(j - n_chain) * n + r)) = make_uint4(term.e[0], term.e[1], term.e[2], term.e[3]);
-    }
-  }
-  if (a0 < n_chain) *(uint4*)(row_total + 4 * (size_t)r) = make_uint4(run.e[0], run.e[1], run.e[2], run.e[3]);
 }
 __global__ void logup_chain_kernel(uint32_t* __restrict__ accum, const uint32_t* __restrict__ scanned, uint32_t n_cols, uint32_t po2) {
   const uint32_t r = blockIdx.x * 256u + threadIdx.x, col = blockIdx.y;
@@ -217,122 +26,213 @@
   const uint4 v = *(const uint4*)(scanned + 4 * (size_t)r);
   cols[r] = v.x; cols[((size_t)1 << po2) + r] = v.y; cols[((size_t)2 << po2) + r] = v.z; cols[((size_t)3 << po2) + r] = v.w;
 }
-}
-
-static const char* own_accumulators(r0h_ctx* ctx, const r0h_circuit* c, uint32_t po2, const Tape& t, const DeviceTape& d, r0h_buf* accum, uint32_t* totals_out) {
-  const uint32_t n = 1u << po2, n_chain = c->logup.n_chain, n_acc = (uint32_t)c->logup.accs.size(), n_own = n_acc - n_chain;
-  if (!n_own) return nullptr;
-  DevBuf terms;
+
+std::vector<uint32_t> pub_words(const r0h_circuit* c, const uint32_t* global, const uint32_t* mix) {
+  const uint32_t ng = std::max(1u, c->n_global), nm = std::max(1u, c->n_mix);
+  std::vector<uint32_t> pub(ng + nm, 0u);
+  if (global) std::copy(global, global + c->n_global, pub.begin());
+  if (mix) std::copy(mix, mix + c->n_mix, pub.begin() + ng);
+  return pub;
+}
+const char* launch_rows(r0h_ctx* ctx, const r0h_circuit* c, LogupKernel which, uint32_t n, void** args, const char* what) {
+  const hipFunction_t* fn = nullptr;
+  R0H_TRY(logup_kernels(c, &fn));
+  R0H_REQUIRE(fn[which], "%s: the circuit has no such kernel", what);
+  hipError_t e = hipModuleLaunchKernel(fn[which], (n + 255) / 256, 1, 1, 256, 1, 1, 0, ctx->stream, args, nullptr);
+  R0H_REQUIRE(e == hipSuccess, "%s: launch failed: %s", what, hipGetErrorString(e));
+  return nullptr;
+}
+size_t columns_read(const r0h_circuit* c, uint32_t a0, uint32_t a1, bool lookups_only) {
+  std::set<uint32_t> cols;
+  auto form = [&](const Lf& lf) {
+    for (const LfTerm& t : lf.terms)
+      if (t.col) cols.insert(t.col);
+  };
+  for (uint32_t j = a0; j < a1; j++)
+    for (const LogupFraction& f : c->logup.accs[j].fr) {
+      if (lookups_only && !f.table) continue;
+      form(f.num);
+      for (size_t q = 0; q < f.parts.size(); q++)
+        if (!lookups_only || q == 1) form(f.parts[q].lf);
+    }
+  return cols.size();
+}
+const char* require_inputs(const char* caller, const r0h_circuit* c, uint32_t a0, uint32_t a1, const r0h_buf* code, const uint32_t* global) {
+  const uint32_t reads = logup_reads(c, a0, a1);
+  R0H_REQUIRE(!(reads & 1u) || code, "%s: a form reads the CODE group and none was given", caller);
+  R0H_REQUIRE(!(reads & 2u) || global, "%s: a form reads a public input and none were given", caller);
+  return nullptr;
+}
+
+const char* unpack_own(r0h_ctx* ctx, const r0h_circuit* c, uint32_t po2, const r0h_buf* scanned, r0h_buf* accum) {
+  const uint32_t n = 1u << po2, n_chain = c->logup.n_chain, n_own = (uint32_t)c->logup.accs.size() - n_chain;
+  for (uint32_t k = 0; k < n_own; k++) {
+    hipLaunchKernelGGL(logup_unpack_kernel, dim3((n + 255) / 256), dim3(256), 0, ctx->stream, u32(accum) + ((size_t)(4 * (n_chain + k)) << po2),
+                       u32(scanned) + 4 * (size_t)k * n, po2);
+    R0H_TRY(launch_ok("logup_unpack_kernel"));
+  }
+  return nullptr;
+}
+const char* own_accumulators(r0h_ctx* ctx, const r0h_circuit* c, uint32_t po2, const r0h_buf* code, const r0h_buf* data, const uint32_t* global, DevBuf& terms,
+                             uint32_t* totals_out) {
+  const uint32_t n = 1u << po2, n_own = (uint32_t)(c->logup.accs.size() - c->logup.n_chain);
   R0H_TRY(terms.alloc(ctx, (size_t)n_own * n * 16));
-  hipLaunchKernelGGL(logup_term_kernel, dim3((n + 255) / 256), dim3(256), 0, ctx->stream, accum ? u32(accum) : nullptr, (uint32_t*)nullptr, u32(terms.get()),
-                     d.words + t.acc_begin[n_chain], d.cols, d.ch, n_chain, n_acc, n_chain, po2);
-  R0H_TRY(launch_ok("logup_term_kernel"));
+  std::vector<uint32_t> pub = pub_words(c, global, nullptr);
+  uint32_t* d_terms = u32(terms.get());
+  const uint32_t* d_code = code ? u32(code) : nullptr;
+  const uint32_t* d_data = u32(data);
+  void* args[] = {&d_terms, &d_code, &d_data, pub.data(), &po2};
+  R0H_TRY(launch_rows(ctx, c, LOGUP_OWN, n, args, "logup_terms_own"));
   for (uint32_t k = 0; k < n_own; k++) {
     r0h_buf view = buf_view(terms.get(), (size_t)k * n * 16, (size_t)n * 16);
     R0H_TRY(r0h_prefix_sums(ctx, &view, n));
-    if (accum) {
-      hipLaunchKernelGGL(logup_unpack_kernel, dim3((n + 255) / 256), dim3(256), 0, ctx->stream, u32(accum) + ((size_t)(4 * (n_chain + k)) << po2), (const uint32_t*)view.ptr, po2);
-      R0H_TRY(launch_ok("logup_unpack_kernel"));
-    }
     if (totals_out) R0H_TRY(r0h_buf_d2h(ctx, &view, (size_t)(n - 1) * 16, totals_out + 4 * k, 16));
   }
   return nullptr;
 }
-
-const char* logup_accum(r0h_ctx* ctx, const r0h_circuit* c, uint32_t po2, const r0h_buf* code, const r0h_buf* data, const uint32_t* global, const uint32_t* mix, r0h_buf* accum) {
+}
+
+const char* logup_accum(r0h_ctx* ctx, const r0h_circuit* c, uint32_t po2, const r0h_buf* code, const r0h_buf* data, const uint32_t* global, const uint32_t* mix, r0h_buf* accum,
+                        const LogupTerms* terms) {
   R0H_GUARD_BEGIN
   R0H_REQUIRE(ctx && c && data && accum, "r0h_accum: NULL argument");
   R0H_REQUIRE(po2 >= 4 && po2 <= R0H_MAX_PO2, "r0h_accum: po2 %u outside [4, %u]", po2, R0H_MAX_PO2);
-  const uint32_t n = 1u << po2, n_chain = c->logup.n_chain;
+  const uint32_t n = 1u << po2, n_chain = c->logup.n_chain, n_acc = (uint32_t)c->logup.accs.size();
   R0H_REQUIRE(((size_t)c->group_size[R0H_GROUP_DATA] << po2) * 4 <= data->bytes && ((size_t)c->group_size[R0H_GROUP_ACCUM] << po2) * 4 <= accum->bytes &&
                   (!code || ((size_t)c->group_size[R0H_GROUP_CODE] << po2) * 4 <= code->bytes),
               "r0h_accum: buffers too small for 2^%u rows", po2);
   for (uint32_t i = 0; i < c->n_mix; i++) R0H_REQUIRE(mix && mix[i] < P, "r0h_accum: mix[%u] missing or not canonical", i);
   for (uint32_t i = 0; i < c->n_global; i++) R0H_REQUIRE(!global || global[i] < P, "r0h_accum: global[%u] not canonical", i);
-  Tape t;
-  R0H_TRY(build_tape(c, po2, code, data, global, mix, &t));
-  DeviceTape d;
-  R0H_TRY(upload_tape(ctx, t, &d));
-  KScope ks(ctx, "logup_accum", ((double)t.cols.size() + 2.0 * c->group_size[R0H_GROUP_ACCUM]) * n * 4);
+  R0H_TRY(require_inputs("log-derivative accumulation", c, 0, n_acc, code, global));
+  if (terms && n_acc > n_chain)
+    R0H_REQUIRE(terms->buf && terms->c == c && terms->po2 == po2 && terms->data == data->ptr && global && terms->global.size() == c->n_global &&
+                    std::equal(terms->global.begin(), terms->global.end(), global),
+                "r0h_accum: the terms handed over were computed for another circuit, size, witness or set of public inputs (the challenge is one of them)");
+  KScope ks(ctx, "logup_accum", ((double)columns_read(c, 0, n_acc, false) + 2.0 * c->group_size[R0H_GROUP_ACCUM]) * n * 4);
   DevBuf totals;
   R0H_TRY(totals.alloc(ctx, (size_t)n * 16));
-  hipLaunchKernelGGL(logup_term_kernel, dim3((n + 255) / 256), dim3(256), 0, ctx->stream, u32(accum), u32(totals.get()), (uint32_t*)nullptr, d.words, d.cols, d.ch, 0u, n_chain, n_chain, po2);
-  R0H_TRY(launch_ok("logup_term_kernel"));
+  std::vector<uint32_t> pub = pub_words(c, global, mix);
+  uint32_t *d_accum = u32(accum), *d_totals = u32(totals.get());
+  const uint32_t* d_code = code ? u32(code) : nullptr;
+  const uint32_t* d_data = u32(data);
+  void* args[] = {&d_accum, &d_totals, &d_code, &d_data, pub.data(), &po2};
+  R0H_TRY(launch_rows(ctx, c, LOGUP_CHAIN, n, args, "logup_terms_chain"));
   R0H_TRY(r0h_prefix_sums(ctx, totals.get(), n));
   hipLaunchKernelGGL(logup_chain_kernel, dim3((n + 255) / 256, 4 * n_chain), dim3(256), 0, ctx->stream, u32(accum), u32(totals.get()), 4 * n_chain, po2);
   R0H_TRY(launch_ok("logup_chain_kernel"));
-  R0H_TRY(own_accumulators(ctx, c, po2, t, d, accum, nullptr));
-  R0H_TRY_HIP(hipStreamSynchronize(ctx->stream));
-  return nullptr;
-  R0H_GUARD_END
-}
-
-}
-
-using namespace r0h;
-
-extern "C" {
-
-const char* r0h_logup_multiplicities(r0h_ctx* ctx, const r0h_circuit* c, uint32_t po2, r0h_buf* data, const uint32_t* global) {
-  R0H_GUARD_BEGIN
-  R0H_REQUIRE(ctx && c && data, "r0h_logup_multiplicities: NULL argument");
+  if (n_acc == n_chain) return nullptr;
+  if (terms) return unpack_own(ctx, c, po2, terms->buf.get(), accum);
+  DevBuf own;
+  R0H_TRY(own_accumulators(ctx, c, po2, code, data, global, own, nullptr));
+  return unpack_own(ctx, c, po2, own.get(), accum);
+  R0H_GUARD_END
+}
+
+const char* logup_count_launch(r0h_ctx* ctx, const r0h_circuit* c, uint32_t po2, r0h_buf* data, const uint32_t* global, DevBuf* hist) {
+  R0H_GUARD_BEGIN
+  R0H_REQUIRE(ctx && c && data && hist, "r0h_logup_multiplicities: NULL argument");
+  hist->reset();
   if (c->logup.tables.empty()) return nullptr;
   R0H_REQUIRE(po2 >= 16 && po2 <= R0H_MAX_PO2, "r0h_logup_multiplicities: the tables have 2^16 rows: po2 %u outside [16, %u]", po2, R0H_MAX_PO2);
   R0H_REQUIRE(((size_t)c->group_size[R0H_GROUP_DATA] << po2) * 4 <= data->bytes, "r0h_logup_multiplicities: the DATA buffer is too small for 2^%u rows", po2);
   R0H_REQUIRE(c->logup.tables.size() <= 2, "r0h_logup_multiplicities: at most two tables");
-  const uint32_t n = 1u << po2, n_tables = (uint32_t)c->logup.tables.size();
-  Tape t;
-  std::vector<uint32_t> dummy_mix(c->n_mix, 0), dummy_global(c->n_global, 0);
-  R0H_TRY(build_tape(c, po2, nullptr, data, global ? global : dummy_global.data(), dummy_mix.data(), &t, true));
-  DeviceTape d;
-  R0H_TRY(upload_tape(ctx, t, &d));
+  const uint32_t n = 1u << po2, n_tables = (uint32_t)c->logup.tables.size(), n_chain = c->logup.n_chain;
   std::vector<uint64_t> slots(n_tables, 0);
-  for (uint32_t j = 0; j < c->logup.n_chain; j++)
+  for (uint32_t j = 0; j < n_chain; j++)
     for (const LogupFraction& f : c->logup.accs[j].fr)
       if (f.table && f.table <= n_tables) slots[f.table - 1] += n;
   for (uint32_t k = 0; k < n_tables; k++)
     R0H_REQUIRE(slots[k] <= P - 1, "r0h_logup_multiplicities: table %u has %llu lookup slots at 2^%u rows: more than p - 1", k, (unsigned long long)slots[k], po2);
-  DevBuf hist;
   const size_t hist_words = (size_t)n_tables * 65536;
-  R0H_TRY(hist.alloc(ctx, hist_words * 4 + 16));
-  R0H_TRY_HIP(hipMemsetAsync(hist->ptr, 0, hist_words * 4 + 16, ctx->stream));
-  KScope ks(ctx, "logup_multiplicities", (double)t.cols.size() * n * 4);
-  hipLaunchKernelGGL(logup_count_kernel, dim3((n + 255) / 256), dim3(256), 0, ctx->stream, u32(hist.get()), u32(hist.get()) + hist_words, d.words, (uint32_t)t.words.size(), d.cols, n, n_tables);
-  R0H_TRY(launch_ok("logup_count_kernel"));
+  R0H_TRY(hist->alloc(ctx, hist_words * 4 + 16));
+  R0H_TRY_HIP(hipMemsetAsync((*hist)->ptr, 0, hist_words * 4 + 16, ctx->stream));
+  KScope ks(ctx, "logup_multiplicities", (double)columns_read(c, 0, n_chain, true) * n * 4);
+  std::vector<uint32_t> pub = pub_words(c, global, nullptr);
+  uint32_t *d_hist = u32(hist->get()), *d_err = d_hist + hist_words;
+  const uint32_t* d_data = u32(data);
+  void* args[] = {&d_hist, &d_err, &d_data, pub.data(), &po2};
+  R0H_TRY(launch_rows(ctx, c, LOGUP_COUNT, n, args, "logup_count"));
   for (uint32_t k = 0; k < n_tables; k++) {
     const LogupTable& tb = c->logup.tables[k];
-    hipLaunchKernelGGL(logup_mult_kernel, dim3((n + 255) / 256), dim3(256), 0, ctx->stream, u32(data) + ((size_t)tb.data_col << po2), u32(hist.get()) + (size_t)k * 65536,
-                       (uint32_t)slots[k], n);
+    hipLaunchKernelGGL(logup_mult_kernel, dim3((n + 255) / 256), dim3(256), 0, ctx->stream, u32(data) + ((size_t)tb.data_col << po2), d_hist + (size_t)k * 65536, d_err + 1 + k, (uint32_t)slots[k], n);
     R0H_TRY(launch_ok("logup_mult_kernel"));
   }
-  R0H_TRY_HIP(hipStreamSynchronize(ctx->stream));
+  return nullptr;
+  R0H_GUARD_END
+}
+
+const char* logup_count_verdict(r0h_ctx* ctx, const r0h_circuit* c, const DevBuf& hist) {
+  if (!hist) return nullptr;
   uint32_t err = 0;
-  R0H_TRY(r0h_buf_d2h(ctx, hist.get(), hist_words * 4, &err, 4));
+  R0H_TRY(r0h_buf_d2h(ctx, hist.get(), c->logup.tables.size() * 65536 * 4, &err, 4));
   R0H_REQUIRE(!(err & 1u), "r0h_logup_multiplicities: a lookup's numerator is neither 0 nor 1");
   R0H_REQUIRE(!(err & 2u), "r0h_logup_multiplicities: a row whose numerator is 1 looks up a value that is not in its table");
   return nullptr;
-  R0H_GUARD_END
-}
-
-const char* r0h_logup_totals(r0h_ctx* ctx, const r0h_circuit* c, uint32_t po2, const r0h_buf* code, const r0h_buf* data, uint32_t* global_io) {
+}
+
+const char* logup_totals(r0h_ctx* ctx, const r0h_circuit* c, uint32_t po2, const r0h_buf* code, const r0h_buf* data, uint32_t* global_io, LogupTerms* terms) {
   R0H_GUARD_BEGIN
   R0H_REQUIRE(ctx && c && data && global_io, "r0h_logup_totals: NULL argument");
   R0H_REQUIRE(po2 >= 4 && po2 <= R0H_MAX_PO2, "r0h_logup_totals: po2 %u outside [4, %u]", po2, R0H_MAX_PO2);
   const uint32_t n_chain = c->logup.n_chain, n_acc = (uint32_t)c->logup.accs.size();
+  if (terms) *terms = LogupTerms();
   if (n_acc == n_chain) return nullptr;
+  R0H_REQUIRE(((size_t)c->group_size[R0H_GROUP_DATA] << po2) * 4 <= data->bytes && (!code || ((size_t)c->group_size[R0H_GROUP_CODE] << po2) * 4 <= code->bytes),
+              "r0h_logup_totals: buffers too small for 2^%u rows", po2);
   for (uint32_t j = n_chain; j < n_acc; j++)
     for (const LogupFraction& f : c->logup.accs[j].fr)
       for (const LogupPart& q : f.parts) R0H_REQUIRE(q.ch_kind != 1, "r0h_logup_totals: accumulator %u takes a challenge from the mix", j);
-  Tape t;
-  std::vector<uint32_t> dummy_mix(c->n_mix, 0);
-  R0H_TRY(build_tape(c, po2, code ? code : data, data, global_io, dummy_mix.data(), &t));
-  DeviceTape d;
-  R0H_TRY(upload_tape(ctx, t, &d));
+  R0H_TRY(require_inputs("r0h_logup_totals", c, n_chain, n_acc, code, global_io));
+  DevBuf own;
   std::vector<uint32_t> totals(4 * (size_t)(n_acc - n_chain));
-  R0H_TRY(own_accumulators(ctx, c, po2, t, d, nullptr, totals.data()));
+  R0H_TRY(own_accumulators(ctx, c, po2, code, data, global_io, own, totals.data()));
   for (uint32_t j = n_chain; j < n_acc; j++) memcpy(global_io + c->logup.accs[j].final_global, totals.data() + 4 * (size_t)(j - n_chain), 16);
-  return nullptr;
-  R0H_GUARD_END
-}
-
-}
+  if (terms) {
+    terms->buf = std::move(own);
+    terms->c = c;
+    terms->data = data->ptr;
+    terms->po2 = po2;
+    terms->global.assign(global_io, global_io + c->n_global);
+  }
+  return nullptr;
+  R0H_GUARD_END
+}
+
+}
+
+using namespace r0h;
+
+extern "C" {
+
+const char* r0h_logup_multiplicities(r0h_ctx* ctx, const r0h_circuit* c, uint32_t po2, r0h_buf* data, const uint32_t* global) {
+  DevBuf hist;
+  R0H_TRY(logup_count_launch(ctx, c, po2, data, global, &hist));
+  return logup_count_verdict(ctx, c, hist);
+}
+
+const char* r0h_logup_totals(r0h_ctx* ctx, const r0h_circuit* c, uint32_t po2, const r0h_buf* code, const r0h_buf* data, uint32_t* global_io) {
+  return logup_totals(ctx, c, po2, code, data, global_io, nullptr);
+}
+
+const char* r0hi_logup_totals_terms(r0h_ctx* ctx, const r0h_circuit* c, uint32_t po2, const r0h_buf* code, const r0h_buf* data, uint32_t* global_io, void** terms_out) {
+  R0H_GUARD_BEGIN
+  R0H_REQUIRE(terms_out, "r0hi_logup_totals_terms: NULL argument");
+  std::unique_ptr<LogupTerms> terms(new LogupTerms());
+  R0H_TRY(logup_totals(ctx, c, po2, code, data, global_io, terms.get()));
+  *terms_out = terms.release();
+  return nullptr;
+  R0H_GUARD_END
+}
+const char* r0hi_accum_public_terms(r0h_ctx* ctx, const r0h_circuit* c, uint32_t po2, const r0h_buf* code, const r0h_buf* data, const uint32_t* global, const uint32_t* mix,
+                                    r0h_buf* accum, const void* terms) {
+  R0H_REQUIRE(c && terms && !c->logup.accs.empty(), "r0hi_accum_public_terms: NULL argument, or a circuit without a log-derivative argument");
+  return logup_accum(ctx, c, po2, code, data, global, mix, accum, (const LogupTerms*)terms);
+}
+void r0hi_logup_terms_free(void* terms) { delete (LogupTerms*)terms; }
+const char* r0hi_logup_count_later(r0h_ctx* ctx, const r0h_circuit* c, uint32_t po2, r0h_buf* data, const uint32_t* global) {
+  DevBuf hist;
+  R0H_TRY(logup_count_launch(ctx, c, po2, data, global, &hist));
+  return logup_count_verdict(ctx, c, hist);
+}
+
+}
diff --git a/hyperfridge-r0_amd/csrc/prover.hip b/hyperfridge-r0_amd/csrc/prover.hip
--- a/hyperfridge-r0_amd/csrc/prover.hip
+++ b/hyperfridge-r0_amd/csrc/prover.hip
@@ -482,7 +482,8 @@
 extern "C" {
 
 static const char* prove_segment_impl(r0h_ctx* ctx, const r0h_circuit* c, uint32_t po2, const r0h_buf* code, const r0h_code_commit* cc,
-                                      const r0h_buf* data, const uint32_t* global, uint32_t* seal_out, size_t seal_cap, size_t* seal_words_out) {
+                                      const r0h_buf* data, const uint32_t* global, uint32_t* seal_out, size_t seal_cap, size_t* seal_words_out,
+                                      const LogupTerms* terms = nullptr) {
   R0H_GUARD_BEGIN
   R0H_REQUIRE(ctx && c && (code || cc) && data && seal_words_out, "r0h_prove_segment: NULL argument");
   R0H_REQUIRE(global || r0h_circuit_n_global(c) == 0, "r0h_prove_segment: global is NULL");
@@ -501,7 +502,8 @@
     const r0h_buf* code_cols = code;
     r0h_buf code_view;
     if (!code_cols && cc && cc->witness) { code_view = *cc->witness; code_cols = &code_view; }
-    R0H_TRY(r0h_accum_public(ctx, c, po2, code_cols, data, st.global.data(), st.mix.data(), accum));
+    if (terms) R0H_TRY(logup_accum(ctx, c, po2, code_cols, data, st.global.data(), st.mix.data(), accum, terms));
+    else R0H_TRY(r0h_accum_public(ctx, c, po2, code_cols, data, st.global.data(), st.mix.data(), accum));
     R0H_TRY(proof_finish(st, accum, seal));
   }
   *seal_words_out = seal.size();
@@ -528,6 +530,14 @@
   return nullptr;
   R0H_GUARD_END
 }
+
+}
+const char* r0h::prove_segment_with_terms(r0h_ctx* ctx, const r0h_circuit* c, uint32_t po2, const r0h_buf* code, const r0h_buf* data, const uint32_t* global, const LogupTerms* terms,
+                                          uint32_t* seal_out, size_t seal_capacity_words, size_t* seal_words_out) {
+  R0H_REQUIRE(code && terms && c && !c->logup.accs.empty(), "prove_segment_with_terms: NULL argument, or a circuit without a log-derivative argument");
+  return prove_segment_impl(ctx, c, po2, code, nullptr, data, global, seal_out, seal_capacity_words, seal_words_out, terms);
+}
+extern "C" {
 
 const char* r0h_prove_segment(r0h_ctx* ctx, const r0h_circuit* c, uint32_t po2, const r0h_buf* code, const r0h_buf* data,
                               const uint32_t* global, uint32_t* seal_out, size_t seal_cap, size_t* seal_words_out) {
diff --git a/hyperfridge-r0_amd/csrc/session.cpp b/hyperfridge-r0_amd/csrc/session.cpp
--- a/hyperfridge-r0_amd/csrc/session.cpp
+++ b/hyperfridge-r0_amd/csrc/session.cpp
@@ -336,12 +336,15 @@
   rows.pin(seg.rows.data(), seg.rows.capacity() * sizeof(r0h_preflight_row));
   const r0h_trace_segment ts = {seg.info.index + 1, seg.info.closing, seg.info.pre.pc, 0};
   R0H_TRY(r0h_trace_witgen(pend.lctx, seg.rows.data(), seg.rows.size(), seg.bounds.data(), seg.bounds.size(), pend.po2, &ts, data.get(), global.data()));
-  R0H_TRY(r0h_logup_multiplicities(pend.lctx, c, pend.po2, data.get(), global.data()));
+  DevBuf counts;
+  R0H_TRY(logup_count_launch(pend.lctx, c, pend.po2, data.get(), global.data(), &counts));
   const Clock::time_point t1 = Clock::now();
   r0h_proof* proof = nullptr;
   R0H_TRY(r0h_proof_begin_committed(pend.lctx, c, pend.po2, pend.cc, data.get(), global.data(), nullptr, &proof));
   pend.proof.reset(proof);
   R0H_TRY(r0h_proof_data_root(proof, pend.root));
+  R0H_TRY(logup_count_verdict(pend.lctx, c, counts));
+  counts.reset();
   {
     const uint64_t evaluations = ((uint64_t)c->group_size[R0H_GROUP_DATA] << pend.po2) * 16;
     std::unique_lock<std::mutex> lk(ses->result_mu);
@@ -523,11 +526,12 @@
   memcpy(p.global.data() + R0H_TRACE_GAMMA, challenge, 64);
   const r0h_buf* code_cols = nullptr;
   R0H_TRY(r0h_code_commit_columns(p.cc, &code_cols));
-  R0H_TRY(r0h_logup_totals(p.lctx, c, p.po2, code_cols, data.get(), p.global.data()));
+  LogupTerms terms;
+  R0H_TRY(logup_totals(p.lctx, c, p.po2, code_cols, data.get(), p.global.data(), &terms));
   R0H_TRY(r0h_proof_late(p.proof.get(), p.global.data() + (R0H_TRACE_GLOBALS - R0H_TRACE_LATE_GLOBALS), mix.data()));
   DevBuf accum;
   R0H_TRY(accum.alloc(p.lctx, ((size_t)c->group_size[R0H_GROUP_ACCUM] << p.po2) * 4));
-  R0H_TRY(r0h_accum_public(p.lctx, c, p.po2, code_cols, data.get(), p.global.data(), mix.data(), accum.get()));
+  R0H_TRY(logup_accum(p.lctx, c, p.po2, code_cols, data.get(), p.global.data(), mix.data(), accum.get(), &terms));
   return r0h_proof_finish(p.proof.release(), accum.get(), seal.data(), seal.size(), words);
 }
 }
```
